# IBM/VillanDiffusion

Hardware: AMD Instinct MI355X
Metric: train imgs/sec + 1000-step DDPM sample imgs/sec, CIFAR10 bs128 (higher is better)
Workload: dtype bf16x3/f32

## Files before the change

### include/villan_hip.h

```cpp
#ifndef VILLAN_HIP_H
#define VILLAN_HIP_H

#include <stdint.h>

#ifdef __cplusplus
extern "C" {
#endif

#define VD_ABI_VERSION 12
#define VD_EINVAL (-22)
#define VD_ETIMEDOUT (-110)

int vd_abi_version(void);
const char* vd_last_error(void);
int vd_device_ok(void);
int vd_async_errors(int clear);

enum vd_a_mode { VD_A_ROW = 0,
                 VD_A_COL = 1 };
enum vd_b_mode { VD_B_PLAIN = 0,
                 VD_B_KCONTIG = 1,
                 VD_B_CONV3 = 2,
                 VD_B_CONV3_T = 3,
                 VD_B_CONV3_S2 = 4,
// ... 70 lines not shown
int vd_conv_wgrad_kernel_name(const vd_wgrad_desc* desc, char* name, int name_len);

int vd_presplit_pack(const float* x, void* y, int B, int C, int HW, int64_t x_bstride, int64_t y_bstride, void* stream);
int vd_presplit_unpack(const void* y, float* x, int B, int C, int HW, int64_t y_bstride, int64_t x_bstride, void* stream);
int vd_groupnorm_fwd_presplit_ok(int C, int HW, int G);
int vd_groupnorm_fwd_presplit(const float* x, const float* gamma, const float* beta, void* y, float* mean, float* rstd, int B, int C, int HW, int G,
                              float eps, int apply_silu, int64_t x_bstride, int64_t y_bstride, void* stream);
int vd_groupnorm_bwd_presplit(const float* dy, const float* x, const float* mean, const float* rstd, const float* gamma, const float* beta,
                              const float* extra, const float* extra2, float* dx, void* dx_ps, float* dgamma_ws, float* dbeta_ws, float* rowsum,
                              int B, int C, int HW, int G, int apply_silu, int64_t dy_bstride, int64_t x_bstride, int64_t extra_bstride,
                              int64_t extra2_bstride, int64_t dx_bstride, int64_t ps_bstride, int64_t rowsum_ld, void* stream);

int vd_conv_wgrad_group_class(const vd_wgrad_desc* desc);
int64_t vd_conv_wgrad_group_job_bytes(void);
int vd_conv_wgrad_group_variant(int cls);
int vd_conv_wgrad_group_plan(const vd_wgrad_desc* descs, int n, void* table_out, int64_t* ws_floats, int* blocks, int* rblocks);
int vd_conv_wgrad_group_rebase(void* dev_table, int n, float* ws, void* stream);
int vd_conv_wgrad_group_launch(const void* dev_table, int n, int cls, int blocks, int rblocks, void* stream);
int vd_conv_wgrad_group_kernel_name(int cls, char* name, int name_len);

int64_t vd_conv3_packed_bytes(int M, int C, int taps);
int vd_conv3_pack_weights(const float* W, void* packed, int M, int C, int taps, int64_t row_stride, int64_t chan_stride, void* stream);
int vd_conv3_pack_weights_multi(const int64_t* table, int n_jobs, int64_t total_blocks, void* stream);
int vd_conv3_pack_weights_f16_multi(const int64_t* table, int n_jobs, int64_t total_blocks, void* stream);

int vd_weight_transpose(const float* W, float* Wt, int M, int C, int T, void* stream);
int vd_sumpool2x2(const float* dU, float* dX, int B, int C, int H, int W, int64_t du_bstride, int64_t dx_bstride,
                  int accumulate, void* stream);
int vd_col2im_s2(const float* G, float* dX, int B, int C, int H, int W, int OH, int OW, int pad, int64_t g_bstride,
                 int64_t dx_bstride, void* stream);
int vd_rowsum(const float* X, float* ws, int B, int M, int P, int64_t x_bstride, int64_t ws_ld, void* stream);
int vd_colsum(const float* ws, float* out, int B, int C, int64_t ld, int accumulate, void* stream);
int vd_colsum_segmented(const int64_t* table, int n_jobs, int B, void* stream);

int64_t vd_groupnorm_ws_floats(int B, int C, int HW, int G);
int vd_groupnorm_fwd(const float* x, const float* gamma, const float* beta, float* y, float* mean, float* rstd,
                     int B, int C, int HW, int G, float eps, int apply_silu, int64_t x_bstride, int64_t y_bstride,
                     float* ws, void* stream);
int vd_groupnorm_stats(const float* x, const float* gamma, const float* beta, float* ss, float* mean, float* rstd,
                       int B, int C, int HW, int G, float eps, int64_t x_bstride, void* stream);
int vd_groupnorm_stats_from_partials(const float* part, int tiles, const float* gamma, const float* beta, float* ss, float* mean,
                                     float* rstd, int B, int C, int HW, int G, float eps, void* stream);
int vd_groupnorm_bwd(const float* dy, const float* x, const float* mean, const float* rstd, const float* gamma,
                     const float* beta, const float* extra, float* dx, float* dgamma_ws, float* dbeta_ws,
                     int B, int C, int HW, int G, int apply_silu, int64_t dy_bstride, int64_t x_bstride,
                     int64_t extra_bstride, int64_t dx_bstride, float* ws, void* stream);
int vd_groupnorm_bwd_fused(const float* dy, const float* x, const float* mean, const float* rstd, const float* gamma,
                           const float* beta, const float* extra, const float* extra2, float* dx, float* dgamma_ws,
                           float* dbeta_ws, float* rowsum, int B, int C, int HW, int G, int apply_silu,
                           int64_t dy_bstride, int64_t x_bstride, int64_t extra_bstride, int64_t extra2_bstride,
                           int64_t dx_bstride, int64_t rowsum_ld, float* ws, void* stream);
int vd_groupnorm_plan(int which, int B, int C, int HW, int G, int aligned, int has_ws, void* stream, char* name, int name_len);

int vd_softmax_col_fwd(float* S, int nb, int N, void* stream);
int vd_softmax_col_bwd(const float* P, float* dP, int nb, int N, float scale, void* stream);
int vd_attn_small_fwd(const float* qkv, float* out, float* P, int B, int C, int N, float scale,
                      int64_t qkv_bstride, int64_t out_bstride, void* stream);
int vd_attn_small_bwd(const float* qkv, const float* P, const float* dout, float* dqkv, int B, int C, int N,
                      float scale, int64_t qkv_bstride, int64_t dout_bstride, int64_t dqkv_bstride, void* stream);

int vd_attn_core_fwd(const float* qkv, float* out, float* P, int B, int heads, int head_dim, int N, float scale, void* stream);
int vd_attn_core_bwd(const float* qkv, const float* P, const float* out, const float* dout, float* dS, float* dqkv, int B, int heads,
                     int head_dim, int N, float scale, void* stream);

int vd_attn_flash_fwd(const float* qkv, float* out, float* lse, int B, int heads, int head_dim, int N, float scale, int64_t qkv_bstride,
                      int64_t out_bstride, void* stream);
int vd_attn_flash_bwd(const float* qkv, const float* out, const float* dout, const float* lse, float* delta, float* dqkv, int B, int heads,
                      int head_dim, int N, float scale, int64_t qkv_bstride, int64_t out_bstride, int64_t dout_bstride,
                      int64_t dqkv_bstride, void* stream);

int vd_timestep_embedding(const float* t, const float* freqs, float* emb, int B, int half, int flip_sin_to_cos,
                          void* stream);
int vd_silu_fwd(const float* x, float* y, int64_t n, void* stream);
int vd_silu_bwd(const float* dy, const float* x, float* dx, int64_t n, int accumulate, void* stream);
int vd_add_strided(float* dst, const float* src, int B, int64_t inner, int64_t dst_bstride, int64_t src_bstride,
                   int accumulate, void* stream);
int vd_scale(float* x, int64_t n, float alpha, void* stream);
int vd_lincomb(float* out, const float* const* srcs, const float* coefs, int n_src, int64_t n, void* stream);

int vd_qsample_backdoor(const float* x0, const float* R, const float* eps, const int64_t* t,
                        const float* tab_a, const float* tab_s, const float* tab_step, const float* tab_coef,
                        float* x_t, float* y, int B, int64_t chw, void* stream);
int vd_mse_fwd_bwd(const float* pred, const float* y, const float* pscale, float* dpred, float* loss,
                   float* partial, int B, int64_t chw, float gscale, void* stream);
#define VD_LOSS_L2 0
#define VD_LOSS_L1 1
#define VD_LOSS_HUBER 2
int vd_loss_fwd_bwd(const float* pred, const float* y, const float* pscale, float* dpred, float* loss,
                    float* partial, int B, int64_t chw, float gscale, int kind, void* stream);
int vd_loss_sample_fwd_bwd(const float* pred, const float* y, const float* pscale, const float* weight, const float* wtab, const int64_t* t,
                           int T, const uint8_t* flags, float poison_weight, float* dpred, float* loss, float* sample_loss, float* stats,
                           float* ws, int B, int64_t chw, float gscale, int kind, void* stream);
int64_t vd_loss_sample_ws_floats(int B, int64_t chw);
int vd_loss_sample_plan(int B, int64_t chw, int* segments, int* blocks);
int vd_trigger_inv_objective(const float* e, const float* tau, float lambda, float* loss, float* dout, float* dtau, float* partial,
                             int B, int64_t chw, int64_t e_bstride, void* stream);
int vd_removal_loss(const float* pred, const float* ref, float w_clean, float w_shift, float gscale, float* dpred, float* terms,
                    float* partial, int B, int64_t chw, int64_t pred_bstride, void* stream);
int vd_image_set_stats(const float* x, int N, int C, int H, int W, int64_t x_bstride, float mul, float add, float lo, float hi,
                       float* mean_img, float* stats, float* partial, void* stream);
int vd_score_inv_objective(const float* s, const float* tau, float sigma, float lambda, float* loss, float* dout, float* dtau,
                           float* partial, int B, int64_t chw, int64_t s_bstride, void* stream);
int vd_image_set_merge(float* mean_a, float* stats_a, int64_t n_a, const float* mean_b, const float* stats_b, int64_t n_b, int64_t chw,
                       float* partial, void* stream);
int vd_neuron_scale(const float* w0, float* w, const int64_t* table, int n_jobs, int64_t total_blocks, const float* mask, const float* delta,
                    const float* xi, void* stream);
// ... 51 lines not shown
```

### villandiffusion_amd/csrc/vd_conv_bx3.inc

```
typedef __bf16 bf16x8 __attribute__((ext_vector_type(8)));
typedef unsigned int u32x4 __attribute__((ext_vector_type(4)));

constexpr int XC = 16;

__device__ __forceinline__ void split_bf16x8(const float (&v)[8], u32x4& hi, u32x4& lo) {
    bf16x8 h, l;
#pragma unroll
    for (int j = 0; j < 8; ++j) {
        const __bf16 t = (__bf16)v[j];
        h[j] = t;
        l[j] = (__bf16)(v[j] - (float)t);
    }
    hi = __builtin_bit_cast(u32x4, h);
    lo = __builtin_bit_cast(u32x4, l);
}

template <int T>
__device__ __forceinline__ void conv3_pack_one(const float* __restrict__ src, u32x4* __restrict__ dst, int M, int C, int Mpad, int64_t rs,
                                               int64_t cs, int local) {
    if (local >= Mpad * (C / XC) * 2) return;
    const int m = local % Mpad;
    const int rest = local / Mpad;
    const int q = rest & 1, cc = rest >> 1;
    float v[8][T];
// ... 754 lines not shown
    if (d.OW != 8 || d.OH != 8 || d.pool2 || d.gn_ss || d.N % 256 != 0) return false;
    if (d.b_mode != VD_B_CONV3 && d.b_mode != VD_B_CONV3_T) return false;
    const int base = vd_cdiv(d.M, 128) * (d.N / 256);
    return base >= 32 && base < 256 && d.C / XC >= 8;
}

static void bx3_plan(const vd_gemm_desc& d, int& splits, int& c_per) {
    const int base = vd_cdiv(d.M, 128) * vd_cdiv(d.N, 128);
    const int nchunks = d.C / XC;
    splits = 1;
    if (bx3_big_split(d)) {
        const int bb = vd_cdiv(d.M, 128) * (d.N / 256);
        static const int tgt = getenv("VD_BX3_BIGSPLIT_TARGET") ? atoi(getenv("VD_BX3_BIGSPLIT_TARGET")) : 256;
        splits = vd_cdiv(tgt, bb);
        if (splits > nchunks / 2) splits = nchunks / 2;
        c_per = vd_cdiv(nchunks, splits);
        splits = vd_cdiv(nchunks, c_per);
        return;
    }
    static const int target = getenv("VD_BX3_SPLIT_TARGET") ? atoi(getenv("VD_BX3_SPLIT_TARGET")) : 512;
    if (base < 256) {
        splits = vd_cdiv(d.OW == 4 ? target / 2 : target, base);
        const int max_splits = nchunks / 2 > 0 ? nchunks / 2 : 1;
        if (splits > max_splits) splits = max_splits;
    }
    c_per = vd_cdiv(nchunks, splits);
    splits = vd_cdiv(nchunks, c_per);
}

static int bx3_big_tile(const vd_gemm_desc& d, int splits) {
    if (splits != 1 || (d.OW != 16 && d.OW != 32) || d.N % 256 != 0) return 0;
    if (d.b_mode != VD_B_CONV3_T && !d.pool2 && d.OW == 32 && d.N % 512 == 0) {
        const int nh = vd_cdiv(d.M, 128) * (d.N / 512);
        if (nh >= 256 && (nh % 256 == 0 || nh % 256 >= 192)) return 2;
    }
    const int nb = vd_cdiv(d.M, 128) * (d.N / 256);
    return (nb >= 256 && (nb % 256 == 0 || nb % 256 >= 192)) ? 1 : 0;
}

static bool k32p_pick(const vd_gemm_desc& d) {
    if (d.b_mode != VD_B_CONV3 && d.b_mode != VD_B_CONV3_T && d.b_mode != VD_B_CONV3_UP) return false;
    if (!vd_conv3_k32p_eligible(d) || d.N % 256 != 0) return false;
    const int nt = vd_cdiv(d.M, 128) * (d.N / 256);
    const int rounds = vd_cdiv(nt, 256);
    return nt >= 192 && 4 * nt >= 3 * rounds * 256;
}

static bool pool2_ok(const vd_gemm_desc& d) {
    if (!d.a_packed || d.b_mode != VD_B_CONV3_T || d.bias || d.rowadd || d.residual || d.accumulate) return false;
    if (k32p_pick(d)) return true;
    return d.OH == d.OW && (d.OW == 16 || d.OW == 32) && vd_cdiv(d.M, 128) * vd_cdiv(d.N, 128) >= 256;
}

static int launch_bx3(const vd_gemm_desc& d, int tile, hipStream_t st, char* name) {
    const int mode = d.b_mode == VD_B_CONV3 ? (d.gn_ss ? 3 : 0) : (d.b_mode == VD_B_CONV3_T ? 1 : (d.b_mode == VD_B_CONV3_S2 ? 4 : 2));
    if (tile == 18) {
        if (vd_launch_conv3_k32p(d, mode, st, name) != 0) return VD_EINVAL;
        if (name && d.OW > 32) {
            char at[16];
            snprintf(at, sizeof(at), "@%d", d.OW);
            vd_name_append(name, at);
        }
        return 0;
    }
    int splits, c_per;
    bx3_plan(d, splits, c_per);
    if (!name && splits > 1 && d.ws == nullptr) {
        vd_set_error("vd_gemm: split-K workspace required (%d splits): query vd_gemm_ws_floats()", splits);
        return VD_EINVAL;
    }
    if (tile == 16) {
        dim3 grids(vd_cdiv(d.M, 128) * (d.N / 256), splits);
        if (mode == 0) VD_LAUNCH_OR_NAME(name, (conv3_bx3_kernel<8, 0, 2, 512, 2>), grids, dim3(512), 0, st, d, c_per);
        else VD_LAUNCH_OR_NAME(name, (conv3_bx3_kernel<8, 1, 2, 512, 2>), grids, dim3(512), 0, st, d, c_per);
        if (!name && splits > 1) launch_splitk_epilogue(d, splits, st);
        return 0;
    }
    if (tile == 15) {
        dim3 gridh(vd_cdiv(d.M, 128) * (d.N / 512), 1);
        switch (mode) {
        case 0: VD_LAUNCH_OR_NAME(name, (conv3_bx3_kernel<32, 0, 4, 512, 2>), gridh, dim3(512), 0, st, d, c_per); break;
        case 1: VD_LAUNCH_OR_NAME(name, (conv3_bx3_kernel<32, 1, 4, 512, 2>), gridh, dim3(512), 0, st, d, c_per); break;
        case 2: VD_LAUNCH_OR_NAME(name, (conv3_bx3_kernel<32, 2, 4, 512, 2>), gridh, dim3(512), 0, st, d, c_per); break;
        default: VD_LAUNCH_OR_NAME(name, (conv3_bx3_kernel<32, 3, 4, 512, 2>), gridh, dim3(512), 0, st, d, c_per); break;
        }
        return 0;
    }
    bool done = false;
    if (tile == 12) {
        dim3 gridb(vd_cdiv(d.M, 128) * (d.N / 256), 1);
#define BX3_BIG(WW, MD)                                                                                   \
    if (!done && d.OW == WW && mode == MD) {                                                              \
        VD_LAUNCH_OR_NAME(name, (conv3_bx3_kernel<WW, MD, 2, 512, 2>), gridb, dim3(512), 0, st, d, c_per); \
        done = true;                                                                                      \
    }
        BX3_BIG(32, 0) BX3_BIG(32, 1) BX3_BIG(32, 2) BX3_BIG(32, 3)
        BX3_BIG(16, 0) BX3_BIG(16, 1) BX3_BIG(16, 2) BX3_BIG(16, 3)
#undef BX3_BIG
        return done ? 0 : VD_EINVAL;
    }
    dim3 grid(vd_cdiv(d.M, 128) * vd_cdiv(d.N, 128), splits);
    const int tw = d.OW >= 128 && d.OW % 128 == 0 ? 128 : d.OW;
#define BX3_CASE(WW, MD)                                                                      \
    if (!done && tw == WW && mode == MD) {                                                    \
        VD_LAUNCH_OR_NAME(name, (conv3_bx3_kernel<WW, MD, 2, 256, 2>), grid, dim3(NT), 0, st, d, c_per); \
        done = true;                                                                          \
    }
    BX3_CASE(32, 0) BX3_CASE(32, 1) BX3_CASE(32, 2) BX3_CASE(32, 3)
    BX3_CASE(16, 0) BX3_CASE(16, 1) BX3_CASE(16, 2) BX3_CASE(16, 3)
    BX3_CASE(8, 0) BX3_CASE(8, 1) BX3_CASE(8, 2)
    BX3_CASE(4, 0) BX3_CASE(4, 1)
    BX3_CASE(32, 4) BX3_CASE(16, 4) BX3_CASE(8, 4) BX3_CASE(4, 4)
    BX3_CASE(64, 0) BX3_CASE(64, 1) BX3_CASE(64, 2)
    BX3_CASE(128, 0) BX3_CASE(128, 1) BX3_CASE(128, 2)
    BX3_CASE(64, 4) BX3_CASE(128, 4)
#undef BX3_CASE
    if (!done) return VD_EINVAL;
    if (!name && splits > 1) launch_splitk_epilogue(d, splits, st);
    return 0;
}
```

### villandiffusion_amd/csrc/vd_gemm.hip

```cpp
#include "vd_common.h"
#include <string.h>
#include <stdlib.h>

bool vd_conv3_k32p_eligible(const vd_gemm_desc& d);
int vd_launch_conv3_k32p(const vd_gemm_desc& d, int mode, hipStream_t st, char* name);
int vd_launch_wgrad_ps_group(const void* jobs, int n, int W, int up, int blocks, hipStream_t st, bool one, char* name);
bool vd_conv3_sm_eligible(const vd_gemm_desc& d);
int vd_launch_conv3_sm(const vd_gemm_desc& d, hipStream_t st, char* name);
bool vd_gemm1x1_k32p_pick(const vd_gemm_desc& d);
int vd_launch_gemm1x1_k32p(const vd_gemm_desc& d, hipStream_t st, char* name);

namespace {

constexpr int NT = 256;
constexpr int BK = 32;
constexpr int KG = BK / 4;

struct Pix {
    int b, oy, ox, p;
    bool valid;
};

__device__ __forceinline__ void kdecomp9(int k, int& c, int& r, int& s) {
    c = k / 9;
    int rs = k - c * 9;
    r = (rs * 11) >> 5;
    s = rs - r * 3;
}

template <int BMODE>
__device__ __forceinline__ float conv_gather(const float* __restrict__ src, const vd_gemm_desc& d, const Pix& px,
                                             int64_t boff, int c, int r, int s, bool& ok) {
    int iy, ix;
    if (BMODE == VD_B_CONV3) {
        iy = px.oy + r - 1;
        ix = px.ox + s - 1;
        ok = (unsigned)iy < (unsigned)d.H && (unsigned)ix < (unsigned)d.W;
    } else if (BMODE == VD_B_CONV3_T) {
        iy = px.oy + 1 - r;
        ix = px.ox + 1 - s;
        ok = (unsigned)iy < (unsigned)d.H && (unsigned)ix < (unsigned)d.W;
    } else if (BMODE == VD_B_CONV3_S2) {
        iy = 2 * px.oy + r - d.pad;
        ix = 2 * px.ox + s - d.pad;
        ok = (unsigned)iy < (unsigned)d.H && (unsigned)ix < (unsigned)d.W;
    } else if (BMODE == VD_B_CONV3_UP) {
        int uy = px.oy + r - 1, ux = px.ox + s - 1;
        ok = (unsigned)uy < (unsigned)(2 * d.H) && (unsigned)ux < (unsigned)(2 * d.W);
        iy = uy >> 1;
        ix = ux >> 1;
    } else if (BMODE == VD_B_CONVG) {
        iy = px.oy * d.conv_stride + r - d.pad_h;
        ix = px.ox * d.conv_stride + s - d.pad_w;
// ... 522 lines not shown
                    acc[mi][ni] = __builtin_amdgcn_mfma_f32_32x32x2f32(a0[mi], b0[ni], acc[mi][ni], 0, 0, 0);
            if (u + 2 < (CKK / 2) * 9) fetch(u + 2, a0, b0);
            __builtin_amdgcn_sched_barrier(0);
#pragma unroll
            for (int mi = 0; mi < WM; ++mi)
#pragma unroll
                for (int ni = 0; ni < WN; ++ni)
                    acc[mi][ni] = __builtin_amdgcn_mfma_f32_32x32x2f32(a1[mi], b1[ni], acc[mi][ni], 0, 0, 0);
        }
        __syncthreads();
        if (more && !(VD_DBG(d) & 8)) store_stage((ks + 1) * CKK);
        __syncthreads();
    }
    if (gridDim.y == 1) {
        gemm_epilogue<WM, WN>(d, acc, m0, n0, wm, wn, lane, h);
        return;
    }
    float* __restrict__ slab = d.ws + (int64_t)blockIdx.y * d.M * d.N;
#pragma unroll
    for (int ni = 0; ni < WN; ++ni) {
        const int n = n0 + wn * 32 * WN + ni * 32 + (lane & 31);
        if (n >= d.N) continue;
#pragma unroll
        for (int mi = 0; mi < WM; ++mi)
#pragma unroll
            for (int v = 0; v < 16; ++v) {
                const int m = m0 + wm * 64 + mi * 32 + (v & 3) + 8 * (v >> 2) + 4 * h;
                if (m < d.M) slab[(int64_t)m * d.N + n] = acc[mi][ni][v];
            }
    }
}

__global__ __launch_bounds__(256) void splitk_epilogue_kernel(const vd_gemm_desc d, int splits) {
    const int64_t total = (int64_t)d.M * d.N;
    for (int64_t i = blockIdx.x * (int64_t)blockDim.x + threadIdx.x; i < total; i += (int64_t)gridDim.x * blockDim.x) {
        const int m = (int)(i / d.N), n = (int)(i - (int64_t)m * d.N);
        float s = d.ws[i];
        for (int z = 1; z < splits; ++z) s += d.ws[(int64_t)z * total + i];
        const int b = n / d.NP, p = n - b * d.NP;
        float val = d.alpha * s;
        if (d.bias) val += d.bias[d.bias_on_n ? n : m];
        if (d.rowadd) val += d.rowadd[(int64_t)b * d.rowadd_bstride + m];
        if (d.residual) val += d.residual[(int64_t)b * d.res_bstride + (int64_t)m * d.ldd + p];
        const int64_t off = (int64_t)b * d.d_bstride + (int64_t)m * d.ldd + p;
        if (d.accumulate) val += d.D[off];
        d.D[off] = val;
    }
}

__global__ __launch_bounds__(256) void splitk_epilogue4_kernel(const vd_gemm_desc d, int splits) {
    const int64_t total4 = ((int64_t)d.M * d.N) >> 2;
    const int64_t total = (int64_t)d.M * d.N;
    for (int64_t i4 = blockIdx.x * (int64_t)blockDim.x + threadIdx.x; i4 < total4; i4 += (int64_t)gridDim.x * blockDim.x) {
        const int64_t i = i4 << 2;
        const int m = (int)(i / d.N), n = (int)(i - (int64_t)m * d.N);
        f32x4 s = *reinterpret_cast<const f32x4*>(d.ws + i);
        for (int z = 1; z < splits; ++z) {
            const f32x4 p = *reinterpret_cast<const f32x4*>(d.ws + (int64_t)z * total + i);
#pragma unroll
            for (int j = 0; j < 4; ++j) s[j] += p[j];
        }
        const int b = n / d.NP, p = n - b * d.NP;
        f32x4 val;
#pragma unroll
        for (int j = 0; j < 4; ++j) {
            val[j] = d.alpha * s[j];
            if (d.bias) val[j] += d.bias[d.bias_on_n ? n + j : m];
        }
        if (d.rowadd) {
            const float ra = d.rowadd[(int64_t)b * d.rowadd_bstride + m];
#pragma unroll
            for (int j = 0; j < 4; ++j) val[j] += ra;
        }
        if (d.residual) {
            const f32x4 r = *reinterpret_cast<const f32x4*>(d.residual + (int64_t)b * d.res_bstride + (int64_t)m * d.ldd + p);
#pragma unroll
            for (int j = 0; j < 4; ++j) val[j] += r[j];
        }
        float* __restrict__ dp = d.D + (int64_t)b * d.d_bstride + (int64_t)m * d.ldd + p;
        if (d.accumulate) {
            const f32x4 o = *reinterpret_cast<const f32x4*>(dp);
#pragma unroll
            for (int j = 0; j < 4; ++j) val[j] += o[j];
        }
        *reinterpret_cast<f32x4*>(dp) = val;
    }
}

static void launch_splitk_epilogue(const vd_gemm_desc& d, int splits, hipStream_t st) {
    const int64_t total = (int64_t)d.M * d.N;
    const bool v4 = (d.N & 3) == 0 && (d.NP & 3) == 0 && (d.ldd & 3) == 0 && (d.d_bstride & 3) == 0 && (d.res_bstride & 3) == 0 &&
                    (((uintptr_t)d.D | (uintptr_t)d.residual | (uintptr_t)d.ws) & 15) == 0;
    if (v4) {
        const int64_t t4 = total >> 2;
        const int g2 = (int)((t4 + 255) / 256 < 2048 ? (t4 + 255) / 256 : 2048);
        hipLaunchKernelGGL(splitk_epilogue4_kernel, dim3(g2), dim3(256), 0, st, d, splits);
    } else {
        const int g2 = (int)((total + 255) / 256 < 2048 ? (total + 255) / 256 : 2048);
        hipLaunchKernelGGL(splitk_epilogue_kernel, dim3(g2), dim3(256), 0, st, d, splits);
    }
}

#include "vd_conv_bx3.inc"

static bool patch_eligible(const vd_gemm_desc& d) {
    if (d.a_mode != VD_A_ROW || d.a_bstride != 0 || d.act) return false;
    if (d.gn_ss && (d.b_mode != VD_B_CONV3 || (d.OW != 16 && d.OW != 32) || d.C > 1024)) return false;
    if (d.b_mode == VD_B_CONV3_S2) {
        if ((d.OW != 4 && d.OW != 8 && d.OW != 16) || d.OH != d.OW || d.H != 2 * d.OH || d.W != 2 * d.OW || d.gn_ss) return false;
    } else if (d.b_mode != VD_B_CONV3 && d.b_mode != VD_B_CONV3_T && d.b_mode != VD_B_CONV3_UP) return false;
    if (d.OW != 4 && d.OW != 8 && d.OW != 16 && d.OW != 32 && d.OW != 64 && d.OW % 128 != 0) return false;
    if (d.OH != d.OW && d.OW < 16) return false;
    if (d.C % CK != 0 || d.OH * d.OW != d.NP || d.d_trans) return false;
    if (d.NP >= 128 ? (d.NP % 128 != 0) : (128 % d.NP != 0)) return false;
    if (d.K != d.C * 9 || (d.lda & 3) != 0 || (((uintptr_t)d.A) & 15) != 0) return false;
    if ((VD_DBG(d) & ~(16 | 1 | 8)) != 0 || (VD_DBG(d) != 0 && !(VD_DBG(d) & 16)) || d.tile != 0) return false;
    if (d.b_mode == VD_B_CONV3_UP && d.OW == 4) return false;
    return d.M >= 64;
}

static void patch_plan(const vd_gemm_desc& d, int& splits, int& ks_per) {
    const int base = vd_cdiv(d.M, 128) * vd_cdiv(d.N, 128);
    const int nsteps = d.C / CK;
    splits = 1;
    if (base < 256) {
        splits = vd_cdiv(512, base);
        const int max_splits = nsteps / 4 > 0 ? nsteps / 4 : 1;
        if (splits > max_splits) splits = max_splits;
    }
    ks_per = vd_cdiv(nsteps, splits);
    splits = vd_cdiv(nsteps, ks_per);
}

static bool patch_wide(const vd_gemm_desc& d) {
    if (d.OW != 32 || d.NP % 256 != 0) return false;
    const int64_t wgs = (int64_t)vd_cdiv(d.M, 128) * (d.N / 256);
    return wgs >= 512 && wgs % 512 == 0;
}

static int launch_patch(const vd_gemm_desc& d, hipStream_t st, char* name) {
    int splits, ks_per;
    patch_plan(d, splits, ks_per);
    const int mode_ = d.b_mode == VD_B_CONV3 ? (d.gn_ss ? 3 : 0) : (d.b_mode == VD_B_CONV3_T ? 1 : (d.b_mode == VD_B_CONV3_S2 ? 4 : 2));
    if (splits == 1 && patch_wide(d)) {
        dim3 grid(vd_cdiv(d.M, 128) * (d.N / 256), 1);
        if (mode_ == 0) VD_LAUNCH_OR_NAME(name, (conv3_patch_kernel<32, 0, 4>), grid, dim3(NT), 0, st, d, ks_per);
        else if (mode_ == 3) VD_LAUNCH_OR_NAME(name, (conv3_patch_kernel<32, 3, 4>), grid, dim3(NT), 0, st, d, ks_per);
        else if (mode_ == 1) VD_LAUNCH_OR_NAME(name, (conv3_patch_kernel<32, 1, 4>), grid, dim3(NT), 0, st, d, ks_per);
        else VD_LAUNCH_OR_NAME(name, (conv3_patch_kernel<32, 2, 4>), grid, dim3(NT), 0, st, d, ks_per);
        return 0;
    }
    if (!name && splits > 1 && d.ws == nullptr) {
        vd_set_error("vd_gemm: split-K workspace required (%d splits): query vd_gemm_ws_floats()", splits);
        return VD_EINVAL;
    }
    dim3 grid(vd_cdiv(d.M, 128) * vd_cdiv(d.N, 128), splits);
    const int mode = mode_;
    bool done = false;
    const int tw = d.OW >= 128 && d.OW % 128 == 0 ? 128 : d.OW;
#define VD_PATCH_CASE(WW, MD)                                                                            \
    if (!done && tw == WW && mode == MD) {                                                               \
        VD_LAUNCH_OR_NAME(name, (conv3_patch_kernel<WW, MD, 2>), grid, dim3(NT), 0, st, d, ks_per);        \
        done = true;                                                                                     \
    }
    VD_PATCH_CASE(64, 0) VD_PATCH_CASE(64, 1) VD_PATCH_CASE(64, 2)
    VD_PATCH_CASE(128, 0) VD_PATCH_CASE(128, 1) VD_PATCH_CASE(128, 2)
    VD_PATCH_CASE(32, 0) VD_PATCH_CASE(32, 1) VD_PATCH_CASE(32, 2) VD_PATCH_CASE(32, 3)
    VD_PATCH_CASE(16, 0) VD_PATCH_CASE(16, 1) VD_PATCH_CASE(16, 2) VD_PATCH_CASE(16, 3)
    VD_PATCH_CASE(8, 0) VD_PATCH_CASE(8, 1) VD_PATCH_CASE(8, 2)
    VD_PATCH_CASE(4, 0) VD_PATCH_CASE(4, 1)
    VD_PATCH_CASE(16, 4) VD_PATCH_CASE(8, 4) VD_PATCH_CASE(4, 4)
#undef VD_PATCH_CASE
    if (!done) return VD_EINVAL;
    if (!name && splits > 1) launch_splitk_epilogue(d, splits, st);
    return 0;
}

template <int TW, int MM>
__global__ __launch_bounds__(256) void conv3_smallm_kernel(const vd_gemm_desc d) {
    constexpr int TH = 256 / TW, PW = TW + 2, PH = TH + 2, CK = 8;
    constexpr int PLn = PH * PW;
    constexpr int P_EL = (CK * PLn + 255) / 256;
    __shared__ float Ps[CK * PLn];
    __shared__ f32x4 Ws[CK * 9];
    const int tid = threadIdx.x;
    const int tiles_x = d.W / TW, tiles_y = d.H / TH;
    int bid = blockIdx.x;
    const int txi = bid % tiles_x;
    bid /= tiles_x;
    const int tyi = bid % tiles_y;
    const int b = bid / tiles_y;
    const int y0 = tyi * TH, x0 = txi * TW;
    const int ty = tid / TW, tx = tid - ty * TW;
    const int HWs = d.H * d.W;
    const float* __restrict__ xb = d.B + (int64_t)b * d.b_bstride;
    const float* __restrict__ Wp = d.A;

    int poff[P_EL];
#pragma unroll
    for (int i = 0; i < P_EL; ++i) {
        const int e = tid + i * 256;
        const int rem = e % PLn;
        const int py = rem / PW, px = rem - py * PW;
        const int iy = y0 + py - 1, ix = x0 + px - 1;
        const bool ok = e < CK * PLn && (unsigned)iy < (unsigned)d.H && (unsigned)ix < (unsigned)d.W;
        poff[i] = ok ? iy * d.W + ix : -1;
    }
    float acc[MM];
#pragma unroll
    for (int m = 0; m < MM; ++m) acc[m] = 0.f;

    for (int c0 = 0; c0 < d.C; c0 += CK) {
        __syncthreads();
#pragma unroll
        for (int i = 0; i < P_EL; ++i) {
            const int e = tid + i * 256;
            if (e < CK * PLn) {
                const int c = c0 + e / PLn;
                const bool ok = poff[i] >= 0 && c < d.C;
                const float v = xb[ok ? (int64_t)c * HWs + poff[i] : 0];
                Ps[e] = ok ? v : 0.f;
            }
        }
        if (tid < CK * 9) {
            const int c = c0 + tid / 9, t = tid - (tid / 9) * 9;
            f32x4 w = {0.f, 0.f, 0.f, 0.f};
#pragma unroll
// ... 1214 lines not shown
    int splits, ks_per;
    patch_plan(*desc, splits, ks_per);
    return splits > 1 ? (int64_t)splits * desc->M * desc->N : 0;
}

extern "C" int vd_gemm_tile(const vd_gemm_desc* desc) {
    if (!desc) return 0;
    const vd_gemm_desc& d = *desc;
    if (d.pool2 && !pool2_ok(d)) return -1;
    if (d.a_packed && d.math == 2) {
        if (bx3_eligible(d) && !bx3_big_split(d) && k32p_pick(d)) return 18;
        if (gemm_bx3_eligible(d) && vd_gemm1x1_k32p_pick(d)) return 19;
        return -1;
    }
    if (d.a_packed && d.math == 3) {
        if (bx3_eligible(d)) {
            if (vd_conv3_sm_eligible(d)) return 20;
            if (!bx3_big_split(d) && k32p_pick(d)) return 18;
            return -1;
        }
        if (gemm_bx3_eligible(d) && vd_gemm1x1_k32p_pick(d)) return 19;
        return -1;
    }
    if (d.a_packed) {
        if (bx3_eligible(d)) {
            if (vd_conv3_sm_eligible(d)) return 20;
            if (bx3_big_split(d)) return 16;
            if (k32p_pick(d)) return 18;
            int splits, c_per;
            bx3_plan(d, splits, c_per);
            const int big = d.b_mode == VD_B_CONV3_S2 ? 0 : bx3_big_tile(d, splits);
            return big == 2 ? 15 : (big == 1 ? 12 : 8);
        }
        if (!gemm_bx3_eligible(d)) return -1;
        if (vd_gemm1x1_k32p_pick(d)) return 19;
        if (gemm_bx3_big_tile(d)) return 13;
        return vd_cdiv(d.M, 128) * (d.N / 128) >= 1024 ? 11 : 9;
    }
    if (d.math == 1) return gemm_bx3_act_eligible(d) ? 10 : -1;
    if (smallm_eligible(d)) return 7;
    if (patch_eligible(d)) {
        int splits, ks_per;
        patch_plan(d, splits, ks_per);
        return (splits == 1 && patch_wide(d)) ? 6 : 4;
    }
    if (plain_eligible(d)) return 5;
    int max_bn = 128;
    if (d.a_bstride != 0 && d.NP % 128 != 0) max_bn = 64;
    int tile = d.tile ? d.tile : pick_tile(d.M, d.N, max_bn);
    if (max_bn < 128 && tile != 3) tile = 3;
    return tile;
}

static int gemm_run(const vd_gemm_desc* desc, hipStream_t st, char* name) {
    VD_REQUIRE(desc != nullptr, "vd_gemm: null desc");
    vd_gemm_desc d = *desc;
    VD_REQUIRE(d.A && d.B && d.D, "vd_gemm: null operand");
    VD_REQUIRE(d.math != 3 || d.a_packed, "vd_gemm: math = 3 (one bf16 product per term) reads the hi plane of a_packed; a_packed is NULL");
#ifndef VD_ABLATION
    VD_REQUIRE(d.debug == 0, "vd_gemm: desc.debug = %d -- timing-only ablation bits exist in `make ABLATION=1` builds only", d.debug);
#endif
    VD_REQUIRE(d.M > 0 && d.N > 0 && d.K > 0 && d.NP > 0 && d.N % d.NP == 0, "vd_gemm: bad dims M=%d N=%d K=%d NP=%d", d.M,
               d.N, d.K, d.NP);
    if (d.b_mode >= VD_B_CONV3) {
        VD_REQUIRE(d.C > 0 && d.H > 0 && d.W > 0 && d.OH * d.OW == d.NP, "vd_gemm: bad conv dims");
        if (d.b_mode == VD_B_CONVG)
            VD_REQUIRE(d.kh > 0 && d.kw > 0 && d.K == d.C * d.kh * d.kw && d.conv_stride >= 1 && d.conv_stride <= 4 && d.pad_h >= 0 && d.pad_w >= 0 &&
                           d.OH == (d.H + 2 * d.pad_h - d.kh) / d.conv_stride + 1 && d.OW == (d.W + 2 * d.pad_w - d.kw) / d.conv_stride + 1 &&
                           !d.a_packed && d.math == 0 && d.a_mode == VD_A_ROW,
                       "vd_gemm: VD_B_CONVG needs kh, kw > 0, K = C*kh*kw, conv_stride 1 .. 4, OH / OW = (H + 2 pad - k) / stride + 1, row-major exact-f32 A");
        else
            VD_REQUIRE(d.K == d.C * 9, "vd_gemm: conv K must be C*9");
    }
    VD_REQUIRE(d.act == 0 || (d.act == 1 && !d.a_packed && d.math == 0), "vd_gemm: act = 1 (ReLU) is honoured by the exact-f32 kernels only");
    if (d.a_bstride != 0) VD_REQUIRE(d.NP % 64 == 0, "vd_gemm: per-batch A needs NP %% 64 == 0 (NP=%d)", d.NP);
    VD_REQUIRE(!(d.d_trans && (d.residual || d.rowadd)), "vd_gemm: d_trans excludes residual/rowadd");
    if (d.nb2 > 1)
        VD_REQUIRE(!d.residual && !d.rowadd && !d.d_trans && d.b_mode <= VD_B_KCONTIG && (d.N / d.NP) % d.nb2 == 0,
                   "vd_gemm: two-level batch (nb2=%d) needs plain operands, no residual/rowadd, nb %% nb2 == 0", d.nb2);
    const int tile = vd_gemm_tile(&d);
    VD_REQUIRE(tile != -1, "vd_gemm: a_packed (split-precision bf16) needs a 3x3 convolution with 8x8 / 16x16 / 32x32 outputs, "
                           "C %% 16 == 0, M >= 64, or a VD_B_PLAIN product with shared A, NP %% 128 == 0, K %% 16 == 0, M >= 64; "
                           "a_packed_mpad = M rounded up to 128; math = 1 needs per-batch A, PLAIN / KCONTIG B, NP %% 128 == 0, K %% 16 == 0, K >= 32, M >= 64; "
                           "math = 2 / 3 need the persistent 16x16x32 kernels (vd_gemm_tile 18 / 19; math = 3 also 20); "
                           "pool2 needs VD_B_CONV3_T with a_packed and a bare epilogue, on the persistent kernel or at 16x16 / 32x32 outputs with >= 256 tiles of 128 x 128");
    VD_REQUIRE(d.b_presplit == 0 || (d.b_presplit == 1 && tile == 18),
               "vd_gemm: a pre-split B operand (b_presplit = %d) is read by the persistent 16x16x32 convolution only (vd_gemm_tile() == 18; this problem: %d)",
               d.b_presplit, tile);
    VD_REQUIRE(!d.gn_ss || tile == 4 || tile == 6 || tile == 8 || tile == 12 || tile == 15 || tile == 18,
               "vd_gemm: gn_ss (GroupNorm folded into the loader) needs the patch-staged 3x3 kernel (OW 16/32, C %% 8 == 0, M >= 64)");
    VD_REQUIRE(!d.pool2 || tile == 8 || tile == 12 || tile == 18, "vd_gemm: pool2 needs the split-precision 3x3 kernel (VD_B_CONV3_T with a_packed)");
    VD_REQUIRE(!d.act_out || (tile == 18 && d.gn_ss), "vd_gemm: act_out is written by the persistent 16x16x32 3x3 convolution with gn_ss only (vd_gemm_tile() == 18)");
    VD_REQUIRE(!d.gn_part || (tile == 18 && !d.pool2),
               "vd_gemm: gn_part is written by the persistent 16x16x32 split-precision 3x3 kernel only (vd_gemm_tile() == 18)");
    int rc = 0;
    switch (tile) {
        case 1: rc = launch_gemm_t<2, 2>(d, st, name); break;
        case 2: rc = launch_gemm_t<1, 2>(d, st, name); break;
        case 3: rc = launch_gemm_t<1, 1>(d, st, name); break;
        case 4:
        case 6: rc = launch_patch(d, st, name); break;
        case 7: rc = launch_smallm(d, st, name); break;
        case 8: case 12: case 15: case 16: case 18: rc = launch_bx3(d, tile, st, name); break;
        case 19: rc = vd_launch_gemm1x1_k32p(d, st, name) == 0 ? 0 : VD_EINVAL; break;
        case 20: rc = vd_launch_conv3_sm(d, st, name) == 0 ? 0 : VD_EINVAL; break;
        case 10: launch_gemm_bx3_act(d, st, name); break;
        case 13: VD_LAUNCH_OR_NAME(name, gemm_bx3_kernel<512>, dim3(vd_cdiv(d.M, 128) * (d.N / 256)), dim3(512), 0, st, d, 1 << 30); break;
        case 9: {
            int splits, st_per;
            gemm_bx3_plan(d, splits, st_per);
            VD_REQUIRE(name || splits == 1 || d.ws, "vd_gemm: split-K 1x1 launch needs the workspace (vd_gemm_ws_floats)");
            VD_LAUNCH_OR_NAME(name, gemm_bx3_kernel<256>, dim3(vd_cdiv(d.M, 128) * (d.N / 128), splits), dim3(NT), 0, st, d, st_per);
            if (!name && splits > 1) launch_splitk_epilogue(d, splits, st);
            break;
        }
        case 11: VD_LAUNCH_OR_NAME(name, gemm_bx3_persist_kernel, dim3(512), dim3(NT), 0, st, d, vd_cdiv(d.M, 128) * (d.N / 128)); break;
        case 5: {
            const int grid = vd_cdiv(d.M, 128) * (d.N / 128);
            if (d.a_mode == VD_A_ROW) VD_LAUNCH_OR_NAME(name, gemm_plain_kernel<0>, dim3(grid), dim3(NT), 0, st, d);
            else VD_LAUNCH_OR_NAME(name, gemm_plain_kernel<1>, dim3(grid), dim3(NT), 0, st, d);
            break;
        }
        default: vd_set_error("vd_gemm: bad tile %d", tile); return VD_EINVAL;
    }
    if (rc || name) return rc ? rc : tile;
    VD_LAUNCH_CHECK("vd_gemm");
    return 0;
}

extern "C" int vd_gemm(const vd_gemm_desc* desc, void* stream) { return gemm_run(desc, (hipStream_t)stream, nullptr); }

static int name_out(int rc, const char* buf, char* name, int name_len) {
    if (!name || name_len <= 0) return VD_EINVAL;
    snprintf(name, name_len, "%s", rc < 0 ? "" : buf);
    return rc < 0 ? VD_EINVAL : rc;
}

extern "C" int vd_gemm_kernel_name(const vd_gemm_desc* desc, char* name, int name_len) {
    char buf[VD_NAME_LEN] = "";
    return name_out(gemm_run(desc, nullptr, buf), buf, name, name_len);
}

extern "C" int64_t vd_conv3_packed_bytes(int M, int C, int taps) {
    if (M <= 0 || C <= 0 || C % XC != 0 || (taps != 9 && taps != 1)) return 0;
    return (int64_t)((M + 127) / 128 * 128) * C * taps * 4;
}

extern "C" int vd_conv3_pack_weights(const float* W, void* packed, int M, int C, int taps, int64_t row_stride, int64_t chan_stride,
                                     void* stream) {
    VD_REQUIRE(W && packed && M > 0 && C > 0 && C % XC == 0 && (taps == 9 || taps == 1),
               "vd_conv3_pack_weights: bad arguments (M=%d C=%d taps=%d; C %% 16 == 0, taps 9 or 1)", M, C, taps);
    VD_REQUIRE((((uintptr_t)packed) & 15) == 0, "vd_conv3_pack_weights: packed must be 16-byte aligned");
    const int Mpad = (M + 127) / 128 * 128;
    const int total = (C / XC) * 2 * Mpad;
    hipLaunchKernelGGL(conv3_pack_kernel, dim3(vd_cdiv(total, 256)), dim3(256), 0, (hipStream_t)stream, W,
                       reinterpret_cast<u32x4*>(packed), M, C, Mpad, row_stride, chan_stride, taps);
    VD_LAUNCH_CHECK("vd_conv3_pack_weights");
    return 0;
}

extern "C" int vd_conv3_pack_weights_multi(const int64_t* table, int n_jobs, int64_t total_blocks, void* stream) {
    VD_REQUIRE(table && n_jobs > 0 && total_blocks > 0 && total_blocks < (1ll << 31), "vd_conv3_pack_weights_multi: bad arguments");
    hipLaunchKernelGGL(conv3_pack_multi_kernel, dim3((unsigned)total_blocks), dim3(256), 0, (hipStream_t)stream, table, n_jobs);
    VD_LAUNCH_CHECK("vd_conv3_pack_weights_multi");
    return 0;
}

static void wgrad_plan(const vd_wgrad_desc& d, int& tile, int& splits, int& kk_per) {
    if (wgrad_small_eligible(d)) {
        tile = 6;
        splits = wgrad_small_parts(d) > 1 ? wgrad_small_parts(d) : 2;
        kk_per = 1;
        return;
    }
    if (wgrad1x1_bx3_eligible(d)) {
        tile = 5;
        wgrad1x1_bx3_plan(d, splits, kk_per);
        return;
    }
    if (wgrad_patch_eligible(d)) {
        tile = 4;
        wgrad_patch_plan(d, splits, kk_per);
        return;
    }
    const int Ncols = d.C * d.T, Ktot = d.nb * d.NP;
    tile = d.tile;
    if (!tile) {
        tile = (d.M > 64 && Ncols > 64) ? 1 : 3;
        if (tile == 1 && vd_cdiv(d.M, 128) * vd_cdiv(Ncols, 128) < 32) tile = 3;
    }
    const int bm = tile == 1 ? 128 : 64, bn = tile == 3 ? 64 : 128;
    const int tiles = vd_cdiv(d.M, bm) * vd_cdiv(Ncols, bn);
    splits = d.splits;
// ... 386 lines not shown
```

### villandiffusion_amd/csrc/vd_norm.hip

```cpp
#include "vd_common.h"
#include <atomic>
#include <stdlib.h>

namespace {

template <int NTH>
__device__ __forceinline__ float block_sum_t(float v, float* red) {
    if (NTH == 256) return block_sum_256(v, red);
    v = wave_sum(v);
    const int w = threadIdx.x >> 6;
    __syncthreads();
    if ((threadIdx.x & 63) == 0) red[w] = v;
    __syncthreads();
    float a = 0.f;
#pragma unroll
    for (int k = 0; k < NTH / 64; ++k) a += red[k];
    return a;
}

template <int NV, int NTH = 256>
__global__ __launch_bounds__(NTH) void gn_fwd_reg_kernel(const float* __restrict__ x, const float* __restrict__ gamma,
                                                         const float* __restrict__ beta, float* __restrict__ y,
                                                         float* __restrict__ mean_out, float* __restrict__ rstd_out, int C,
                                                         int HW, int G, float eps, int apply_silu, int64_t x_bs, int64_t y_bs,
                                                         float* __restrict__ ss_out) {
    __shared__ float red[2 * (NTH / 64 < 4 ? 4 : NTH / 64)];
    const int b = blockIdx.x / G, g = blockIdx.x - b * G;
    const int cpg = C / G;
    const int n4 = (cpg * HW) >> 2;
    const f32x4* __restrict__ x4 = reinterpret_cast<const f32x4*>(x + (int64_t)b * x_bs + (int64_t)g * cpg * HW);
    f32x4* __restrict__ y4 = reinterpret_cast<f32x4*>(y + (int64_t)b * y_bs + (int64_t)g * cpg * HW);
    const int tid = threadIdx.x;
    f32x4 v[NV];
    float s = 0.f;
#pragma unroll
    for (int i = 0; i < NV; ++i) {
        const int idx = tid + i * NTH;
        v[i] = (idx < n4) ? x4[idx] : f32x4{0.f, 0.f, 0.f, 0.f};
        s += (v[i][0] + v[i][1]) + (v[i][2] + v[i][3]);
    }
    const float inv_n = 1.f / (float)(cpg * HW);
    const float mean = block_sum_t<NTH>(s, red) * inv_n;
    float q = 0.f;
#pragma unroll
    for (int i = 0; i < NV; ++i) {
        if (tid + i * NTH < n4) {
            const float a0 = v[i][0] - mean, a1 = v[i][1] - mean, a2 = v[i][2] - mean, a3 = v[i][3] - mean;
            q += (a0 * a0 + a1 * a1) + (a2 * a2 + a3 * a3);
        }
    }
    const float rstd = rsqrtf(block_sum_t<NTH>(q, red + (NTH / 64 < 4 ? 4 : NTH / 64)) * inv_n + eps);
    if (tid == 0) {
        mean_out[blockIdx.x] = mean;
        rstd_out[blockIdx.x] = rstd;
    }
    if (ss_out) {
        if (tid < cpg) {
            const int c = g * cpg + tid;
            const float ga = gamma[c] * rstd, be = beta[c] - mean * ga;
            ss_out[((int64_t)b * C + c) * 2] = ga;
            ss_out[((int64_t)b * C + c) * 2 + 1] = be;
        }
        return;
    }
#pragma unroll
    for (int i = 0; i < NV; ++i) {
        const int idx = tid + i * NTH;
        if (idx < n4) {
            const int c = g * cpg + (idx * 4) / HW;
            const float ga = gamma[c] * rstd, be = beta[c] - mean * ga;
            f32x4 o;
#pragma unroll
            for (int j = 0; j < 4; ++j) {
                const float z = v[i][j] * ga + be;
                o[j] = apply_silu ? z * sigmoidf_(z) : z;
            }
            y4[idx] = o;
        }
    }
}

template <int NV>
__global__ __launch_bounds__(256) void gn_fwd_wave_kernel(const float* __restrict__ x, const float* __restrict__ gamma,
                                                          const float* __restrict__ beta, float* __restrict__ y,
                                                          float* __restrict__ mean_out, float* __restrict__ rstd_out, int C,
                                                          int HW, int G, float eps, int apply_silu, int64_t x_bs, int64_t y_bs,
                                                          float* __restrict__ ss_out, int total) {
    const int lane = threadIdx.x & 63;
    const int gid = blockIdx.x * 4 + (threadIdx.x >> 6);
    if (gid >= total) return;
    const int b = gid / G, g = gid - b * G;
    const int cpg = C / G;
    const int n4 = (cpg * HW) >> 2;
    const f32x4* __restrict__ x4 = reinterpret_cast<const f32x4*>(x + (int64_t)b * x_bs + (int64_t)g * cpg * HW);
    f32x4 v[NV];
    float s = 0.f;
#pragma unroll
    for (int i = 0; i < NV; ++i) {
        const int idx = lane + i * 64;
        v[i] = (idx < n4) ? x4[idx] : f32x4{0.f, 0.f, 0.f, 0.f};
        s += (v[i][0] + v[i][1]) + (v[i][2] + v[i][3]);
    }
    const float inv_n = 1.f / (float)(cpg * HW);
    const float mean = wave_sum(s) * inv_n;
    float q = 0.f;
#pragma unroll
    for (int i = 0; i < NV; ++i) {
        if (lane + i * 64 < n4) {
            const float a0 = v[i][0] - mean, a1 = v[i][1] - mean, a2 = v[i][2] - mean, a3 = v[i][3] - mean;
            q += (a0 * a0 + a1 * a1) + (a2 * a2 + a3 * a3);
        }
    }
    const float rstd = rsqrtf(wave_sum(q) * inv_n + eps);
    if (lane == 0) {
        mean_out[gid] = mean;
        rstd_out[gid] = rstd;
    }
    if (ss_out) {
        for (int cl = lane; cl < cpg; cl += 64) {
            const int c = g * cpg + cl;
            const float ga = gamma[c] * rstd, be = beta[c] - mean * ga;
            ss_out[((int64_t)b * C + c) * 2] = ga;
            ss_out[((int64_t)b * C + c) * 2 + 1] = be;
        }
        return;
    }
    f32x4* __restrict__ y4 = reinterpret_cast<f32x4*>(y + (int64_t)b * y_bs + (int64_t)g * cpg * HW);
#pragma unroll
    for (int i = 0; i < NV; ++i) {
        const int idx = lane + i * 64;
        if (idx < n4) {
            const int c = g * cpg + (idx * 4) / HW;
            const float ga = gamma[c] * rstd, be = beta[c] - mean * ga;
            f32x4 o;
#pragma unroll
            for (int j = 0; j < 4; ++j) {
                const float z = v[i][j] * ga + be;
                o[j] = apply_silu ? z * sigmoidf_(z) : z;
            }
            y4[idx] = o;
        }
    }
}

__global__ __launch_bounds__(256) void gn_fwd_kernel(const float* __restrict__ x, const float* __restrict__ gamma,
                                                     const float* __restrict__ beta, float* __restrict__ y,
                                                     float* __restrict__ mean_out, float* __restrict__ rstd_out, int C, int HW,
                                                     int G, float eps, int apply_silu, int64_t x_bs, int64_t y_bs) {
    __shared__ float red[8];
    const int b = blockIdx.x / G, g = blockIdx.x - b * G;
    const int cpg = C / G;
    const int n = cpg * HW;
    const float* __restrict__ xs = x + (int64_t)b * x_bs + (int64_t)g * n;
    float* __restrict__ ys = y + (int64_t)b * y_bs + (int64_t)g * n;
    const int tid = threadIdx.x;
    const bool vec = ((HW & 3) == 0) && ((((uintptr_t)xs) & 15) == 0) && ((((uintptr_t)ys) & 15) == 0);

    float s = 0.f;
    if (vec) {
        const f32x4* x4 = reinterpret_cast<const f32x4*>(xs);
        for (int i = tid; i < (n >> 2); i += 256) {
            f32x4 v = x4[i];
            s += (v[0] + v[1]) + (v[2] + v[3]);
        }
    } else {
        for (int i = tid; i < n; i += 256) s += xs[i];
    }
    const float mean = block_sum_256(s, red) / (float)n;
    float q = 0.f;
    if (vec) {
        const f32x4* x4 = reinterpret_cast<const f32x4*>(xs);
        for (int i = tid; i < (n >> 2); i += 256) {
            f32x4 v = x4[i];
            const float a0 = v[0] - mean, a1 = v[1] - mean, a2 = v[2] - mean, a3 = v[3] - mean;
            q += (a0 * a0 + a1 * a1) + (a2 * a2 + a3 * a3);
        }
    } else {
        for (int i = tid; i < n; i += 256) {
            const float a = xs[i] - mean;
            q += a * a;
        }
    }
    const float var = block_sum_256(q, red + 4) / (float)n;
    const float rstd = rsqrtf(var + eps);
    if (tid == 0) {
        mean_out[blockIdx.x] = mean;
        rstd_out[blockIdx.x] = rstd;
    }
    if (vec) {
        const f32x4* x4 = reinterpret_cast<const f32x4*>(xs);
        f32x4* y4 = reinterpret_cast<f32x4*>(ys);
        for (int i = tid; i < (n >> 2); i += 256) {
            const int c = g * cpg + (i * 4) / HW;
            const float ga = gamma[c] * rstd, be = beta[c] - mean * ga;
            f32x4 v = x4[i], o;
// ... 213 lines not shown
            if (f4) {
                const f32x4 fv = f4[idx];
#pragma unroll
                for (int j = 0; j < 4; ++j) ev[j] += fv[j];
            }
#pragma unroll
            for (int j = 0; j < 4; ++j) {
                o[j] = rstd * (dz[i][j] * ga - m1 - xh[i][j] * m2) + ev[j];
                s3 += o[j];
            }
            o4[idx] = o;
        }
        if (rs_out) {
            if (L >= 64) {
                s3 = wave_sum(s3);
                if (lane == 0) part3[i * (NTH / 64) + wave] = s3;
            } else {
                for (int off = 1; off < L; off <<= 1) s3 += __shfl_xor(s3, off, 64);
                if (in && (lane & (L - 1)) == 0) ch_s3[idx / L] = s3;
            }
        }
    }
    if (rs_out) {
        __syncthreads();
        if (tid < cpg) {
            float a3;
            if (L >= 64) {
                const int np = L >> 6;
                a3 = 0.f;
                for (int k = 0; k < np; ++k) a3 += part3[tid * np + k];
            } else {
                a3 = ch_s3[tid];
            }
            rs_out[(int64_t)b * rs_ld + g * cpg + tid] = a3;
        }
    }
}

template <int NV>
__global__ __launch_bounds__(256) void gn_bwd_wave_kernel(const float* __restrict__ dy, const float* __restrict__ x,
                                                          const float* __restrict__ mean_in, const float* __restrict__ rstd_in,
                                                          const float* __restrict__ gamma, const float* __restrict__ beta,
                                                          const float* __restrict__ extra, float* __restrict__ dx,
                                                          float* __restrict__ dgamma_ws, float* __restrict__ dbeta_ws, int C,
                                                          int HW, int G, int apply_silu, int64_t dy_bs, int64_t x_bs,
                                                          int64_t ex_bs, int64_t dx_bs, const float* __restrict__ extra2,
                                                          int64_t ex2_bs, float* __restrict__ rs_out, int64_t rs_ld, int total) {
    const int lane = threadIdx.x & 63;
    const int gid = blockIdx.x * 4 + (threadIdx.x >> 6);
    if (gid >= total) return;
    const int b = gid / G, g = gid - b * G;
    const int cpg = C / G;
    const int n4 = (cpg * HW) >> 2;
    const int L = HW >> 2;
    const int64_t goff = (int64_t)g * cpg * HW;
    const f32x4* __restrict__ x4 = reinterpret_cast<const f32x4*>(x + (int64_t)b * x_bs + goff);
    const f32x4* __restrict__ d4 = reinterpret_cast<const f32x4*>(dy + (int64_t)b * dy_bs + goff);
    const f32x4* __restrict__ e4 = extra ? reinterpret_cast<const f32x4*>(extra + (int64_t)b * ex_bs + goff) : nullptr;
    const f32x4* __restrict__ f4 = extra2 ? reinterpret_cast<const f32x4*>(extra2 + (int64_t)b * ex2_bs + goff) : nullptr;
    f32x4* __restrict__ o4 = reinterpret_cast<f32x4*>(dx + (int64_t)b * dx_bs + goff);
    const float mean = mean_in[gid], rstd = rstd_in[gid];

    f32x4 xh[NV], dz[NV];
    float gav[NV];
    float m1 = 0.f, m2 = 0.f;
#pragma unroll
    for (int i = 0; i < NV; ++i) {
        const int idx = lane + i * 64;
        const bool in = idx < n4;
        const f32x4 xv = in ? x4[idx] : f32x4{0.f, 0.f, 0.f, 0.f};
        const f32x4 dv = in ? d4[idx] : f32x4{0.f, 0.f, 0.f, 0.f};
        const int c = g * cpg + (in ? idx / L : 0);
        const float ga = gamma[c], be = beta[c];
        gav[i] = ga;
        float s1 = 0.f, s2 = 0.f;
#pragma unroll
        for (int j = 0; j < 4; ++j) {
            const float h_ = (xv[j] - mean) * rstd;
            float z_ = dv[j];
            if (apply_silu) {
                const float z = h_ * ga + be, sg = sigmoidf_(z);
                z_ *= sg * (1.f + z * (1.f - sg));
            }
            if (!in) z_ = 0.f;
            xh[i][j] = h_;
            dz[i][j] = z_;
            s1 += z_;
            s2 += z_ * h_;
        }
        for (int off = 1; off < L; off <<= 1) {
            s1 += __shfl_xor(s1, off, 64);
            s2 += __shfl_xor(s2, off, 64);
        }
        if (in && (lane & (L - 1)) == 0) {
            dbeta_ws[(int64_t)b * C + c] = s1;
            dgamma_ws[(int64_t)b * C + c] = s2;
            m1 += ga * s1;
            m2 += ga * s2;
        }
    }
    const float inv_n = 1.f / (float)(cpg * HW);
    m1 = wave_sum(m1) * inv_n;
    m2 = wave_sum(m2) * inv_n;
#pragma unroll
    for (int i = 0; i < NV; ++i) {
        const int idx = lane + i * 64;
        const bool in = idx < n4;
        float s3 = 0.f;
        if (in) {
            f32x4 ev = {0.f, 0.f, 0.f, 0.f}, o;
            if (e4) ev = e4[idx];
            if (f4) {
                const f32x4 fv = f4[idx];
#pragma unroll
                for (int j = 0; j < 4; ++j) ev[j] += fv[j];
            }
#pragma unroll
            for (int j = 0; j < 4; ++j) {
                o[j] = rstd * (dz[i][j] * gav[i] - m1 - xh[i][j] * m2) + ev[j];
                s3 += o[j];
            }
            o4[idx] = o;
        }
        if (rs_out) {
            for (int off = 1; off < L; off <<= 1) s3 += __shfl_xor(s3, off, 64);
            if (in && (lane & (L - 1)) == 0) rs_out[(int64_t)b * rs_ld + g * cpg + idx / L] = s3;
        }
    }
}

__device__ __forceinline__ void gn_combine(const float* __restrict__ part, int S, float n_c, float& mean, float& m2) {
    float n = 0.f;
    mean = 0.f;
    m2 = 0.f;
    for (int k = 0; k < S; ++k) {
        const float mk = part[2 * k], qk = part[2 * k + 1];
        const float nn = n + n_c, delta = mk - mean;
        mean += delta * (n_c / nn);
        m2 += qk + delta * delta * (n * n_c / nn);
        n = nn;
    }
}

template <int NV>
__global__ __launch_bounds__(256) void gn_chunk_stats_kernel(const float* __restrict__ x, float* __restrict__ part, int C, int HW,
                                                             int G, int S, int64_t x_bs) {
    __shared__ float red[8];
    const int bg = blockIdx.x / S, sc = blockIdx.x - bg * S;
    const int b = bg / G, g = bg - b * G;
    const int cpg = C / G;
    const int c4 = ((cpg * HW) >> 2) / S;
    const f32x4* __restrict__ x4 = reinterpret_cast<const f32x4*>(x + (int64_t)b * x_bs + (int64_t)g * cpg * HW) + (int64_t)sc * c4;
    const int tid = threadIdx.x;
    f32x4 v[NV];
    float s = 0.f;
#pragma unroll
    for (int i = 0; i < NV; ++i) {
        const int idx = tid + i * 256;
        v[i] = (idx < c4) ? x4[idx] : f32x4{0.f, 0.f, 0.f, 0.f};
        s += (v[i][0] + v[i][1]) + (v[i][2] + v[i][3]);
    }
    const float mean = block_sum_256(s, red) / (float)(c4 * 4);
    float q = 0.f;
#pragma unroll
    for (int i = 0; i < NV; ++i)
        if (tid + i * 256 < c4) {
            const float a0 = v[i][0] - mean, a1 = v[i][1] - mean, a2 = v[i][2] - mean, a3 = v[i][3] - mean;
            q += (a0 * a0 + a1 * a1) + (a2 * a2 + a3 * a3);
        }
    q = block_sum_256(q, red + 4);
    if (tid == 0) {
        part[2 * (int64_t)blockIdx.x] = mean;
        part[2 * (int64_t)blockIdx.x + 1] = q;
    }
}

__global__ __launch_bounds__(256) void gn_chunk_apply_kernel(const float* __restrict__ x, const float* __restrict__ gamma,
                                                             const float* __restrict__ beta, float* __restrict__ y,
                                                             float* __restrict__ mean_out, float* __restrict__ rstd_out,
                                                             const float* __restrict__ part, int C, int HW, int G, int S, float eps,
                                                             int apply_silu, int64_t x_bs, int64_t y_bs) {
// ... 465 lines not shown
    if (slab <= 14 * 1024) return GN_F_REG7_512;
    return GN_F_REG7_1024;
}

static GnFwdKernel gn_fwd_choice(int B, int C, int HW, int G, bool al, bool has_ws, hipStream_t st, int* S_out) {
    const int64_t slab = (int64_t)(C / G) * HW;
    al = al && HW % 4 == 0;
    const int S = (al && has_ws) ? gn_chunks(B, C, HW, G, true) : 0;
    *S_out = S;
    if (S && gn_chunk1_ok(st, S)) return slab / S > 8192 ? GN_F_CHUNK1_16 : GN_F_CHUNK1_8;
    if (S) return slab / S > 8192 ? GN_F_CHUNK2_16 : GN_F_CHUNK2_8;
    if (al && slab <= GN_REG_MAX) return gn_fwd_reg_choice(slab);
    return GN_F_GENERIC;
}

static GnBwdKernel gn_bwd_choice(int B, int C, int HW, int G, bool al, bool has_ws, hipStream_t st, int* S_out) {
    const int64_t slab = (int64_t)(C / G) * HW;
    const int L = HW / 4;
    const int S = (al && has_ws) ? gn_chunks(B, C, HW, G) : 0;
    *S_out = S;
    const bool reg_ok = !S && al && HW % 4 == 0 && slab <= GN_REG_MAX &&
                        ((L >= 64 && L % 64 == 0) || (L < 64 && (L & (L - 1)) == 0 && L > 0));
    if (reg_ok) {
        if (slab <= 1024 && L < 64 && gn_wave_ok()) return slab <= 256 ? GN_B_WAVE1 : slab <= 512 ? GN_B_WAVE2 : GN_B_WAVE4;
        if (slab <= 1024) return GN_B_REG1_256;
        if (slab <= 2048) return GN_B_REG2_256;
        if (slab <= 4096) return GN_B_REG4_256;
        if (slab <= 8192) return GN_B_REG4_512;
        if (slab <= 12 * 1024) return GN_B_REG6_512;
        if (slab <= 14 * 1024) return GN_B_REG7_512;
        return GN_B_REG7_1024;
    }
    if (S && gn_chunk1_ok(st, S)) return slab / S > 8192 ? GN_B_CHUNK1_16 : GN_B_CHUNK1_8;
    if (S) return GN_B_CHUNK2;
    return GN_B_GENERIC;
}

static bool gn_dims_ok(int B, int C, int HW, int G) { return B > 0 && C > 0 && HW > 0 && G > 0 && C % G == 0; }
static bool gn_stats_dims_ok(int B, int C, int HW, int G) { return gn_dims_ok(B, C, HW, G) && C / G <= 256; }
static bool gn_stats_slab_ok(int C, int HW, int G, bool al) { return HW % 4 == 0 && al && (int64_t)(C / G) * HW <= GN_REG_MAX; }
static bool gn_bwd_dims_ok(int B, int C, int HW, int G) { return gn_dims_ok(B, C, HW, G) && C / G <= 64; }

int gn_sticky_impl(const char* who) {
    const unsigned n = gn_flag_read();
    if (n == 0) return 0;
    vd_set_error("%s: %u GroupNorm poll timeout(s) reported by an earlier one-launch chunked kernel (statistics were NaN); "
                 "vd_async_errors(1) clears the flag, VD_GN_CHUNK1_OFF=1 selects the two-launch form", who, n);
    return VD_ETIMEDOUT;
}

}

int vd_gn_sticky(const char* who) { return gn_sticky_impl(who); }

extern "C" int vd_async_errors(int clear) {
    const unsigned n = gn_flag_read();
    if (clear && g_gn_flag_host) *reinterpret_cast<volatile unsigned*>(g_gn_flag_host) = 0u;
    return (int)(n > 0x7fffffffu ? 0x7fffffffu : n);
}

extern "C" int64_t vd_groupnorm_ws_floats(int B, int C, int HW, int G) {
    if (B <= 0 || C <= 0 || HW <= 0 || G <= 0 || C % G) return 0;
    const int S = gn_chunks(B, C, HW, G);
    return S ? 4 * (int64_t)B * G * S + 4 * (int64_t)B * G * S : 0;
}

extern "C" int vd_groupnorm_fwd(const float* x, const float* gamma, const float* beta, float* y, float* mean, float* rstd,
                                int B, int C, int HW, int G, float eps, int apply_silu, int64_t x_bstride, int64_t y_bstride,
                                float* ws, void* stream) {
    VD_REQUIRE(x && gamma && beta && y && mean && rstd, "vd_groupnorm_fwd: null pointer");
    VD_REQUIRE(B > 0 && C > 0 && HW > 0 && G > 0 && C % G == 0, "vd_groupnorm_fwd: bad dims B=%d C=%d HW=%d G=%d", B, C, HW, G);
    const bool al = (x_bstride % 4 == 0) && (y_bstride % 4 == 0) && ((((uintptr_t)x) & 15) == 0) && ((((uintptr_t)y) & 15) == 0);
    if (const int rc = vd_gn_sticky("vd_groupnorm_fwd")) return rc;
    int S = 0;
    const GnFwdKernel k = gn_fwd_choice(B, C, HW, G, al, ws != nullptr, (hipStream_t)stream, &S);
#define VD_GN_CHUNK1(NVV)                                                                                                                           \
    hipLaunchKernelGGL((gn_chunk1_fwd_kernel<NVV>), dim3(B * G * S), dim3(256), 0, (hipStream_t)stream, x, gamma, beta, y, mean, rstd,              \
                       reinterpret_cast<unsigned long long*>(ws + 4 * (int64_t)B * G * S), C, HW, G, S, eps, apply_silu, x_bstride, y_bstride,      \
                       gn_next_epoch(), flag, gn_poll_max())
#define VD_GN_CHUNK2(NVV)                                                                                                                           \
    do {                                                                                                                                            \
        hipLaunchKernelGGL((gn_chunk_stats_kernel<NVV>), dim3(B * G * S), dim3(256), 0, (hipStream_t)stream, x, ws, C, HW, G, S, x_bstride);        \
        hipLaunchKernelGGL(gn_chunk_apply_kernel, dim3(B * G * S), dim3(256), 0, (hipStream_t)stream, x, gamma, beta, y, mean, rstd, ws, C, HW, G,  \
                           S, eps, apply_silu, x_bstride, y_bstride);                                                                               \
    } while (0)
#define VD_GN_FWDW(NVV)                                                                                                                     \
    hipLaunchKernelGGL((gn_fwd_wave_kernel<NVV>), dim3(vd_cdiv(B * G, 4)), dim3(256), 0, (hipStream_t)stream, x, gamma, beta, y, mean, rstd, \
                       C, HW, G, eps, apply_silu, x_bstride, y_bstride, (float*)nullptr, B * G)
#define VD_GN_FWD(NVV, NT)                                                                                                          \
    hipLaunchKernelGGL((gn_fwd_reg_kernel<NVV, NT>), dim3(B * G), dim3(NT), 0, (hipStream_t)stream, x, gamma, beta, y, mean, rstd, \
                       C, HW, G, eps, apply_silu, x_bstride, y_bstride, (float*)nullptr)
    switch (k) {
    case GN_F_CHUNK1_16:
    case GN_F_CHUNK1_8: {
        unsigned* flag = gn_flag_dev();
        if (k == GN_F_CHUNK1_16) VD_GN_CHUNK1(16);
        else VD_GN_CHUNK1(8);
        break;
    }
    case GN_F_CHUNK2_16: VD_GN_CHUNK2(16); break;
    case GN_F_CHUNK2_8: VD_GN_CHUNK2(8); break;
    case GN_F_WAVE1: VD_GN_FWDW(1); break;
    case GN_F_WAVE2: VD_GN_FWDW(2); break;
    case GN_F_WAVE4: VD_GN_FWDW(4); break;
    case GN_F_REG1: VD_GN_FWD(1, 256); break;
    case GN_F_REG2: VD_GN_FWD(2, 256); break;
// ... 204 lines not shown
```

### villandiffusion_amd/lib.py

```python
from __future__ import annotations

import ctypes as C
import os
import subprocess
from typing import Optional

_HERE = os.path.dirname(os.path.abspath(__file__))
LIB_PATH = os.path.join(_HERE, "libvillan_hip.so")
CSRC = os.path.join(_HERE, "csrc")

A_ROW, A_COL = 0, 1
B_PLAIN, B_KCONTIG, B_CONV3, B_CONV3_T, B_CONV3_S2, B_CONV3_UP, B_CONV3_DIL, B_CONVG = range(8)

_i32, _i64, _f32, _vp = C.c_int32, C.c_int64, C.c_float, C.c_void_p


class GemmDesc(C.Structure):
    _fields_ = [("A", _vp), ("B", _vp), ("D", _vp), ("bias", _vp), ("rowadd", _vp), ("residual", _vp),
                ("M", _i32), ("N", _i32), ("K", _i32), ("a_mode", _i32), ("b_mode", _i32), ("NP", _i32),
                ("C", _i32), ("H", _i32), ("W", _i32), ("OH", _i32), ("OW", _i32),
                ("bias_on_n", _i32), ("d_trans", _i32), ("accumulate", _i32), ("tile", _i32), ("debug", _i32), ("alpha", _f32),
                ("lda", _i64), ("a_bstride", _i64), ("ldb", _i64), ("b_bstride", _i64),
                ("ldd", _i64), ("d_bstride", _i64), ("res_bstride", _i64), ("rowadd_bstride", _i64), ("ws", _vp), ("pad", _i32), ("nb2", _i32),
                ("a_b2stride", _i64), ("b_b2stride", _i64), ("d_b2stride", _i64), ("gn_ss", _vp), ("a_packed", _vp), ("a_packed_mpad", _i32), ("math", _i32), ("pool2", _i32),
                ("kh", _i32), ("kw", _i32), ("conv_stride", _i32), ("pad_h", _i32), ("pad_w", _i32), ("act", _i32),
                ("gn_part", _vp), ("act_out", _vp), ("act_bstride", _i64), ("b_presplit", _i32), ("reserved_", _i32)]


class WgradDesc(C.Structure):
    _fields_ = [("dY", _vp), ("X", _vp), ("dW", _vp), ("ws", _vp),
                ("M", _i32), ("C", _i32), ("T", _i32), ("nb", _i32), ("NP", _i32),
                ("H", _i32), ("W", _i32), ("OH", _i32), ("OW", _i32),
                ("mode", _i32), ("splits", _i32), ("accumulate", _i32), ("tile", _i32),
                ("dy_bstride", _i64), ("x_bstride", _i64), ("pad", _i32), ("math", _i32), ("presplit", _i32), ("reserved_", _i32)]


PROTOTYPES = {
    "vd_abi_version": (_i32, []),
    "vd_last_error": (C.c_char_p, []),
    "vd_async_errors": (_i32, [_i32]),
    "vd_device_ok": (_i32, []),
    "vd_gemm": (_i32, [C.POINTER(GemmDesc), _vp]),
    "vd_gemm_tile": (_i32, [C.POINTER(GemmDesc)]),
    "vd_gemm_ws_floats": (_i64, [C.POINTER(GemmDesc)]),
    "vd_gemm_kernel_name": (_i32, [C.POINTER(GemmDesc), C.c_char_p, _i32]),
    "vd_conv_wgrad": (_i32, [C.POINTER(WgradDesc), _vp]),
    "vd_conv_wgrad_plan": (_i32, [C.POINTER(WgradDesc), C.POINTER(_i32), C.POINTER(_i32)]),
    "vd_conv_wgrad_ws_floats": (_i64, [C.POINTER(WgradDesc)]),
    "vd_conv_wgrad_kernel_name": (_i32, [C.POINTER(WgradDesc), C.c_char_p, _i32]),
    "vd_presplit_pack": (_i32, [_vp, _vp, _i32, _i32, _i32, _i64, _i64, _vp]),
    "vd_presplit_unpack": (_i32, [_vp, _vp, _i32, _i32, _i32, _i64, _i64, _vp]),
    "vd_groupnorm_fwd_presplit_ok": (_i32, [_i32, _i32, _i32]),
    "vd_groupnorm_fwd_presplit": (_i32, [_vp, _vp, _vp, _vp, _vp, _vp, _i32, _i32, _i32, _i32, _f32, _i32, _i64, _i64, _vp]),
    "vd_groupnorm_bwd_presplit": (_i32, [_vp] * 12 + [_vp, _i32, _i32, _i32, _i32, _i32] + [_i64] * 7 + [_vp]),
    "vd_conv_wgrad_group_class": (_i32, [C.POINTER(WgradDesc)]),
    "vd_conv_wgrad_group_job_bytes": (_i64, []),
    "vd_conv_wgrad_group_variant": (_i32, [_i32]),
    "vd_conv_wgrad_group_kernel_name": (_i32, [_i32, C.c_char_p, _i32]),
    "vd_conv_wgrad_group_plan": (_i32, [C.POINTER(WgradDesc), _i32, _vp, C.POINTER(_i64), C.POINTER(_i32), C.POINTER(_i32)]),
    "vd_conv_wgrad_group_rebase": (_i32, [_vp, _i32, _vp, _vp]),
    "vd_conv_wgrad_group_launch": (_i32, [_vp, _i32, _i32, _i32, _i32, _vp]),
    "vd_conv3_packed_bytes": (_i64, [_i32, _i32, _i32]),
    "vd_conv3_pack_weights": (_i32, [_vp, _vp, _i32, _i32, _i32, _i64, _i64, _vp]),
    "vd_conv3_pack_weights_multi": (_i32, [_vp, _i32, _i64, _vp]),
    "vd_conv3_pack_weights_f16_multi": (_i32, [_vp, _i32, _i64, _vp]),
    "vd_weight_transpose": (_i32, [_vp, _vp, _i32, _i32, _i32, _vp]),
    "vd_sumpool2x2": (_i32, [_vp, _vp, _i32, _i32, _i32, _i32, _i64, _i64, _i32, _vp]),
    "vd_col2im_s2": (_i32, [_vp, _vp, _i32, _i32, _i32, _i32, _i32, _i32, _i32, _i64, _i64, _vp]),
    "vd_rowsum": (_i32, [_vp, _vp, _i32, _i32, _i32, _i64, _i64, _vp]),
    "vd_colsum": (_i32, [_vp, _vp, _i32, _i32, _i64, _i32, _vp]),
    "vd_colsum_segmented": (_i32, [_vp, _i32, _i32, _vp]),
    "vd_groupnorm_ws_floats": (_i64, [_i32, _i32, _i32, _i32]),
    "vd_groupnorm_stats": (_i32, [_vp, _vp, _vp, _vp, _vp, _vp, _i32, _i32, _i32, _i32, _f32, _i64, _vp]),
    "vd_groupnorm_fwd": (_i32, [_vp, _vp, _vp, _vp, _vp, _vp, _i32, _i32, _i32, _i32, _f32, _i32, _i64, _i64, _vp, _vp]),
    "vd_groupnorm_bwd": (_i32, [_vp] * 10 + [_i32] * 5 + [_i64] * 4 + [_vp, _vp]),
    "vd_groupnorm_stats_from_partials": (_i32, [_vp, _i32, _vp, _vp, _vp, _vp, _vp, _i32, _i32, _i32, _i32, _f32, _vp]),
    "vd_groupnorm_bwd_fused": (_i32, [_vp] * 12 + [_i32] * 5 + [_i64] * 6 + [_vp, _vp]),
    "vd_groupnorm_plan": (_i32, [_i32] * 7 + [_vp, C.c_char_p, _i32]),
    "vd_softmax_col_fwd": (_i32, [_vp, _i32, _i32, _vp]),
    "vd_softmax_col_bwd": (_i32, [_vp, _vp, _i32, _i32, _f32, _vp]),
    "vd_attn_small_fwd": (_i32, [_vp, _vp, _vp, _i32, _i32, _i32, _f32, _i64, _i64, _vp]),
    "vd_attn_small_bwd": (_i32, [_vp, _vp, _vp, _vp, _i32, _i32, _i32, _f32, _i64, _i64, _i64, _vp]),
    "vd_attn_core_fwd": (_i32, [_vp, _vp, _vp, _i32, _i32, _i32, _i32, _f32, _vp]),
    "vd_attn_core_bwd": (_i32, [_vp, _vp, _vp, _vp, _vp, _vp, _i32, _i32, _i32, _i32, _f32, _vp]),
    "vd_attn_flash_fwd": (_i32, [_vp, _vp, _vp, _i32, _i32, _i32, _i32, _f32, _i64, _i64, _vp]),
    "vd_attn_flash_bwd": (_i32, [_vp, _vp, _vp, _vp, _vp, _vp, _i32, _i32, _i32, _i32, _f32, _i64, _i64, _i64, _i64, _vp]),
    "vd_timestep_embedding": (_i32, [_vp, _vp, _vp, _i32, _i32, _i32, _vp]),
    "vd_silu_fwd": (_i32, [_vp, _vp, _i64, _vp]),
    "vd_silu_bwd": (_i32, [_vp, _vp, _vp, _i64, _i32, _vp]),
    "vd_add_strided": (_i32, [_vp, _vp, _i32, _i64, _i64, _i64, _i32, _vp]),
    "vd_scale": (_i32, [_vp, _i64, _f32, _vp]),
    "vd_lincomb": (_i32, [_vp, C.POINTER(_vp), C.POINTER(_f32), _i32, _i64, _vp]),
    "vd_qsample_backdoor": (_i32, [_vp] * 10 + [_i32, _i64, _vp]),
    "vd_mse_fwd_bwd": (_i32, [_vp] * 6 + [_i32, _i64, _f32, _vp]),
    "vd_loss_fwd_bwd": (_i32, [_vp] * 6 + [_i32, _i64, _f32, _i32, _vp]),
    "vd_loss_sample_fwd_bwd": (_i32, [_vp] * 6 + [_i32, _vp, _f32] + [_vp] * 5 + [_i32, _i64, _f32, _i32, _vp]),
    "vd_loss_sample_ws_floats": (_i64, [_i32, _i64]),
    "vd_loss_sample_plan": (_i32, [_i32, _i64, C.POINTER(_i32), C.POINTER(_i32)]),
    "vd_trigger_inv_objective": (_i32, [_vp, _vp, _f32, _vp, _vp, _vp, _vp, _i32, _i64, _i64, _vp]),
    "vd_removal_loss": (_i32, [_vp, _vp, _f32, _f32, _f32, _vp, _vp, _vp, _i32, _i64, _i64, _vp]),
    "vd_score_inv_objective": (_i32, [_vp, _vp, _f32, _f32, _vp, _vp, _vp, _vp, _i32, _i64, _i64, _vp]),
    "vd_image_set_stats": (_i32, [_vp, _i32, _i32, _i32, _i32, _i64, _f32, _f32, _f32, _f32, _vp, _vp, _vp, _vp]),
    "vd_image_set_merge": (_i32, [_vp, _vp, _i64, _vp, _vp, _i64, _i64, _vp, _vp]),
    "vd_neuron_scale": (_i32, [_vp, _vp, _vp, _i32, _i64, _vp, _vp, _vp, _vp]),
    "vd_neuron_grad": (_i32, [_vp, _vp, _vp, _i32, _i64, _vp, _vp, _f32, _i32, _vp]),
    "vd_neuron_step": (_i32, [_vp, _vp, _vp, _i64, _f32, _f32, _f32, _f32, _i32, _vp]),
    "vd_lora_merge": (_i32, [_vp, _vp, _vp, _i32, _i64, _vp, _i32, _f32, _vp]),
    "vd_lora_grad": (_i32, [_vp, _vp, _i32, _i64, _vp, _vp, _i32, _f32, _i32, _vp]),
    "vd_lora_act_grad_ws_floats": (_i64, [_vp, _i32, _i32]),
    "vd_lora_act_grad": (_i32, [_vp, _vp, _i32, _vp, _vp, _i32, _f32, _i32, _vp, _i64, _vp]),
    "vd_l2norm_sq": (_i32, [_vp, _i64, _vp, _vp, _vp]),
    "vd_adam_step": (_i32, [_vp, _vp, _vp, _vp, _i64, _vp, _f32, _f32, _f32, _f32, _f32, _f32, _i32, _vp, _vp]),
    "vd_adam_ema_step": (_i32, [_vp, _vp, _vp, _vp, _vp, _i64, _vp, _f32, _f32, _f32, _f32, _f32, _f32, _i32, _f32, _vp, _vp]),
    "vd_swap": (_i32, [_vp, _vp, _i64, _vp]),
    "vd_sched_step": (_i32, [_vp] * 5 + [_i64] + [_f32] * 7 + [C.c_uint64, C.c_uint64, _vp]),
    "vd_batch_l2norm": (_i32, [_vp, _vp, _i32, _i64, _vp]),
    "vd_postprocess": (_i32, [_vp, _vp, _i32, _i32, _i32, _f32, _f32, _f32, _f32, _i32, _vp]),
    "vd_ssim": (_i32, [_vp, _vp, _vp, _vp, _i32, _i32, _i32, _i32, _i32, _f32, _f32, _vp]),
    "vd_randn": (_i32, [_vp, _i64, C.c_uint64, C.c_uint64, _vp]),
    "vd_fir_resample2": (_i32, [_vp, _vp, _i64, _i32, _i32, _i32, _f32, _i32, _vp]),
    "vd_pyramid_dgrad": (_i32, [_vp, _vp, _vp, _vp, _i32, _i32, _i32, _i32, _i32, _i64, _i32, _vp]),
    "vd_fourier_embedding": (_i32, [_vp, _vp, _vp, _i32, _i32, _vp]),
    "vd_rowscale": (_i32, [_vp, _vp, _vp, _i32, _i64, _i32, _vp]),
    "vd_vq_nearest": (_i32, [_vp, _vp, _vp, _vp, _i32, _i32, _i32, _i32, _i64, _i64, _vp]),
    "vd_poison_batch": (_i32, [_vp] * 8 + [_i32] * 4 + [_f32, _f32, _i32, _vp]),
    "vd_pool3": (_i32, [_vp, _vp, _i32, _i32, _i32, _i32, _i32, _i32, _i32, _i64, _i64, _vp]),
    "vd_resize_bilinear": (_i32, [_vp, _vp, _i64, _i32, _i32, _i32, _i32, _f32, _f32, _vp]),
    "vd_channel_affine": (_i32, [_vp, _vp, _vp, _vp, _i32, _i32, _i32, _vp]),
    "vd_lpips_layer": (_i32, [_vp, _vp, _vp, _vp, _i32, _i32, _i32, _i32, _vp]),
}

# ... 65 lines not shown
```

### villandiffusion_amd/ops.py

```python
from __future__ import annotations

import ctypes as C
import functools
import math
import os
from typing import Optional, Sequence

import torch

from . import lib as L
from .lib import (A_COL, A_ROW, B_CONV3, B_CONV3_DIL, B_CONVG, B_CONV3_S2, B_CONV3_T, B_CONV3_UP, B_KCONTIG, B_PLAIN,
                  GemmDesc, WgradDesc)


def _lib():
    L.require_device()
    return L.load()


_PROF = None


def _kernel_name(query, what) -> str:
    buf = C.create_string_buffer(128)
# ... 183 lines not shown
    e2bs = _img(extra2)[4] if extra2 is not None else 0
    assert dgamma_ws.numel() >= Bn * Cc and dbeta_ws.numel() >= Bn * Cc
    assert (extra is None or extra.shape == x.shape) and (extra2 is None or extra2.shape == x.shape)
    rld = 0
    if rowsum is not None:
        rld = Cc if rowsum_ld is None else rowsum_ld
        assert rld >= Cc
    nbytes = (8.0 + (4.0 if dx is not None else 0.0) + (4.0 if dx_ps is not None else 0.0) + (4.0 if extra is not None else 0.0)
              + (4.0 if extra2 is not None else 0.0)) * x.numel()
    _timed("groupnorm_bwd_presplit (gn_bwd_ps_kernel<*>)", nbytes, "hbm", lambda: L.check(
        _lib().vd_groupnorm_bwd_presplit(_p(dy), _p(x), _p(mean), _p(rstd), _p(gamma), _p(beta), _p(extra), _p(extra2), _p(dx),
                                         _p(dx_ps.t) if dx_ps is not None else None, _p(dgamma_ws), _p(dbeta_ws), _p(rowsum), Bn, Cc, H * W, G,
                                         int(silu), dbs, xbs, ebs, e2bs, dxbs, psbs, rld, _s()), "vd_groupnorm_bwd_presplit"))
    return dx_ps if dx_ps is not None else dx


_GEMM_WS = {}
_WS_SLOT = 0
AUX_WS_SLOT = -1


class ws_slot:

    def __init__(self, slot: int):
        self.slot, self.prev = int(slot), 0

    def __enter__(self):
        global _WS_SLOT
        self.prev, _WS_SLOT = _WS_SLOT, self.slot
        return self

    def __exit__(self, *exc):
        global _WS_SLOT
        _WS_SLOT = self.prev
        return False


def gemm_ws_buffer(device, slot: int = None):
    return _GEMM_WS.get((device, _WS_SLOT if slot is None else slot))


def _gemm_ws(n_floats: int, device):
    key = (device, _WS_SLOT)
    t = _GEMM_WS.get(key)
    if t is None or t.numel() < n_floats:
        t = torch.empty(max(n_floats, 1 << 22), device=device, dtype=torch.float32)
        _GEMM_WS[key] = t
    return t


def gemm(A, B, D, *, M, N, K, a_mode=A_ROW, b_mode=B_PLAIN, NP=None, lda=0, a_bstride=0, ldb=0, b_bstride=0,
         ldd=0, d_bstride=0, bias=None, bias_on_n=False, rowadd=None, rowadd_bstride=0, residual=None,
         res_bstride=0, conv=None, alpha=1.0, d_trans=False, accumulate=False, tile=0, debug=0, pad=0, nb2=0, a_b2stride=0,
         b_b2stride=0, d_b2stride=0, gn_ss=None, a_packed=None, math_mode=0, pool2=False, convg=None, act=0, gn_part=None, b_presplit=False):
    global GN_PART_WRITTEN
    d = GemmDesc()
    d.act = act
    d.b_presplit = int(b_presplit)
    if convg is not None:
        d.kh, d.kw, d.conv_stride, d.pad_h, d.pad_w = convg
    d.pad = pad
    d.pool2 = int(pool2)
    d.math = math_mode
    a_packed16, alt_math = None, 2
    if isinstance(a_packed, tuple):
        a_packed, a_packed16, *rest = a_packed
        alt_math = rest[0] if rest else 2
    if a_packed is not None:
        d.a_packed, d.a_packed_mpad = a_packed.data_ptr(), (M + 127) // 128 * 128
    d.gn_ss = _p(gn_ss)
    d.nb2, d.a_b2stride, d.b_b2stride, d.d_b2stride = nb2, a_b2stride, b_b2stride, d_b2stride
    d.A, d.B, d.D = _p(A), _p(B), _p(D)
    d.bias, d.rowadd, d.residual = _p(bias), _p(rowadd), _p(residual)
    d.M, d.N, d.K = M, N, K
    d.a_mode, d.b_mode = a_mode, b_mode
    d.NP = N if NP is None else NP
    if conv is not None:
        d.C, d.H, d.W, d.OH, d.OW = conv
    d.bias_on_n, d.d_trans, d.accumulate, d.tile = int(bias_on_n), int(d_trans), int(accumulate), tile
    d.alpha = alpha
    d.debug = debug
    d.lda, d.a_bstride, d.ldb, d.b_bstride = lda, a_bstride, ldb, b_bstride
    d.ldd, d.d_bstride, d.res_bstride, d.rowadd_bstride = ldd, d_bstride, res_bstride, rowadd_bstride
    lib = _lib()
    need = lib.vd_gemm_ws_floats(C.byref(d))
    if need > 0:
        d.ws = _gemm_ws(need, D.device).data_ptr()
    elif FORCE_WS is not None:
        d.ws = FORCE_WS.data_ptr()
    global LAST_GEMM_TILE, LAST_GEMM_MATH
    if a_packed16 is not None and (gn_part is None or alt_math == 3):
        d.a_packed, d.math = a_packed16.data_ptr(), alt_math
        if lib.vd_gemm_tile(C.byref(d)) not in ((18, 19) if alt_math == 2 else (18, 19, 20)):
            d.a_packed, d.math = a_packed.data_ptr(), math_mode
    LAST_GEMM_MATH = d.math
    LAST_GEMM_TILE = lib.vd_gemm_tile(C.byref(d))
    GN_PART_WRITTEN = gn_part is not None and not pool2 and LAST_GEMM_TILE == 18
    if GN_PART_WRITTEN:
        assert gn_part.is_contiguous() and gn_part.numel() >= (N // 256) * M * 2
        d.gn_part = gn_part.data_ptr()
    if _PROF is None:
        L.check(lib.vd_gemm(C.byref(d), _s()), "vd_gemm")
        return D
    e0, e1 = torch.cuda.Event(enable_timing=True), torch.cuda.Event(enable_timing=True)
    e0.record()
    L.check(lib.vd_gemm(C.byref(d), _s()), "vd_gemm")
    e1.record()
    flops = 2.0 * M * N * K * (0.25 if b_mode == B_CONV3_DIL else 1.0)
    if conv is not None:
        nb_ = N // d.NP
        b_elems = nb_ * d.C * d.H * d.W
        a_elems = M * K
    else:
        b_elems = K * N
        a_elems = M * K * (N // d.NP if a_bstride else 1)
    d_elems = M * N // (4 if pool2 else 1)
    nbytes = 4.0 * (b_elems + d_elems * (2 if residual is not None else 1) + a_elems)
    name = _kernel_name(lib.vd_gemm_kernel_name, C.byref(d))
    _PROF.append({"name": name, "flops": flops, "bytes": nbytes, "e0": e0, "e1": e1, "kind": "mfma", "shape": (M, K, d.NP, N // d.NP, d.OH, d.OW)})
    return D


_CONV_OUT = {B_CONV3: lambda h, w: (h, w), B_CONV3_T: lambda h, w: (h, w), B_CONV3_S2: lambda h, w: (h // 2, w // 2),
             B_CONV3_UP: lambda h, w: (2 * h, 2 * w), B_CONV3_DIL: lambda h, w: (2 * h, 2 * w)}


def conv3_pack_weights(w2d, M, Cc, transposed=False, out=None, taps=9):
    lib = _lib()
    nbytes = lib.vd_conv3_packed_bytes(M, Cc, taps)
    assert nbytes > 0, (M, Cc, taps)
    if out is None:
        out = torch.empty(nbytes // 4, device=w2d.device, dtype=torch.int32)
    assert out.numel() * out.element_size() >= nbytes and w2d.is_contiguous()
    rs, cs = (taps, M * taps) if transposed else (Cc * taps, taps)
    L.check(lib.vd_conv3_pack_weights(_p(w2d), _p(out), M, Cc, taps, rs, cs, _s()), "vd_conv3_pack_weights")
    return out


def conv3_pack_weights_f16(w2d, M, Cc, transposed=False, taps=9):
    nbytes = _lib().vd_conv3_packed_bytes(M, Cc, taps) // 2
    assert nbytes > 0 and w2d.is_contiguous(), (M, Cc, taps)
    out = torch.empty(nbytes // 4, device=w2d.device, dtype=torch.int32)
    rs, cs = (taps, M * taps) if transposed else (Cc * taps, taps)
    mpad = (M + 127) // 128 * 128
    tab = torch.tensor([[w2d.data_ptr(), out.data_ptr(), M, Cc, rs, cs, 0, taps]], dtype=torch.int64).to(w2d.device)
    conv3_pack_weights_f16_multi(tab, 1, (mpad * (Cc // 16) * 2 + 255) // 256)
    torch.cuda.current_stream(w2d.device).synchronize()
    return out


def conv3_pack_weights_f16_multi(table, n_jobs, total_blocks):
    assert table.dtype == torch.int64 and table.is_contiguous() and table.numel() >= 8 * n_jobs
    L.check(_lib().vd_conv3_pack_weights_f16_multi(_p(table), n_jobs, total_blocks, _s()), "vd_conv3_pack_weights_f16_multi")


def conv3_pack_weights_multi(table, n_jobs, total_blocks):
    assert table.dtype == torch.int64 and table.is_contiguous() and table.numel() >= 8 * n_jobs
    L.check(_lib().vd_conv3_pack_weights_multi(_p(table), n_jobs, total_blocks, _s()), "vd_conv3_pack_weights_multi")


WEIGHTS_EPOCH = 0


@functools.lru_cache(maxsize=None)
def bx3_eligible(M, Cc, OH, OW, mode) -> bool:
    return _gemm_tile(conv_query_desc(M, Cc, OH, OW, mode)) in _BX3_TILES


@functools.lru_cache(maxsize=None)
def bx3_pool2_eligible(M, Cc, OH, OW, nb) -> bool:
    return _gemm_tile(conv_query_desc(M, Cc, OH, OW, B_CONV3_T, nb, pool2=1)) in _BX3_TILES and OW <= 32


GN_PART_WRITTEN = False
LAST_GEMM_TILE = 0
LAST_GEMM_MATH = 0
FORCE_WS = None


def conv3x3(x, w2d, bias, out, mode=B_CONV3, rowadd=None, rowadd_bstride=0, residual=None, accumulate=False, tile=0, debug=0,
            pad=0, gn_ss=None, a_packed=None, pool2=False, gn_part=None):
    x, ps = _unwrap(x)
    Bn, Cc, H, W, xbs = _img(x)
    M = w2d.shape[0]
    assert w2d.shape[1] == Cc * 9 and w2d.is_contiguous()
    OH, OW = _CONV_OUT[mode](H, W)
    Bo, Mo, OHo, OWo, obs = _img(out)
    if pool2:
        assert (Bo, Mo, OHo, OWo) == (Bn, M, OH // 2, OW // 2) and mode == B_CONV3_T and a_packed is not None, (out.shape, (Bn, M, OH, OW))
        assert bias is None and rowadd is None and residual is None and not accumulate
    else:
        assert (Bo, Mo, OHo, OWo) == (Bn, M, OH, OW), (out.shape, (Bn, M, OH, OW))
    rbs = 0
    if residual is not None:
        rbs = _img(residual)[4]
        assert residual.shape == out.shape
    return gemm(w2d, x, out, M=M, N=Bn * OH * OW, K=Cc * 9, b_mode=mode, NP=OH * OW, lda=Cc * 9, b_bstride=xbs,
                ldd=OHo * OWo, d_bstride=obs, bias=bias, rowadd=rowadd, rowadd_bstride=rowadd_bstride,
                residual=residual, res_bstride=rbs, conv=(Cc, H, W, OH, OW), accumulate=accumulate, tile=tile, debug=debug,
                pad=pad, gn_ss=gn_ss, a_packed=a_packed, pool2=pool2, gn_part=gn_part, b_presplit=ps)


def conv2d_general(x, w2d, bias, out, kh, kw, stride=1, pad_h=0, pad_w=0, relu=False):
    Bn, Cc, H, W, xbs = _img(x)
    M = w2d.shape[0]
    assert w2d.shape[1] == Cc * kh * kw and w2d.is_contiguous()
    OH, OW = (H + 2 * pad_h - kh) // stride + 1, (W + 2 * pad_w - kw) // stride + 1
    Bo, Mo, OHo, OWo, obs = _img(out)
    assert (Bo, Mo, OHo, OWo) == (Bn, M, OH, OW), (out.shape, (Bn, M, OH, OW))
    if kh == 1 and kw == 1 and stride == 1 and pad_h == 0 and pad_w == 0:
        return gemm(w2d, x, out, M=M, N=Bn * OH * OW, K=Cc, b_mode=B_PLAIN, NP=OH * OW, lda=Cc, ldb=H * W, b_bstride=xbs, ldd=OH * OW,
                    d_bstride=obs, bias=bias, act=int(relu))
    return gemm(w2d, x, out, M=M, N=Bn * OH * OW, K=Cc * kh * kw, b_mode=B_CONVG, NP=OH * OW, lda=Cc * kh * kw, b_bstride=xbs, ldd=OH * OW,
                d_bstride=obs, bias=bias, conv=(Cc, H, W, OH, OW), convg=(kh, kw, stride, pad_h, pad_w), act=int(relu))


def pool3(x, out, stride=1, pad=0, mode="max"):
    Bn, Cc, H, W, xbs = _img(x)
    OH, OW = (H + 2 * pad - 3) // stride + 1, (W + 2 * pad - 3) // stride + 1
    Bo, Co, OHo, OWo, obs = _img(out)
    assert (Bo, Co, OHo, OWo) == (Bn, Cc, OH, OW), (out.shape, (Bn, Cc, OH, OW))
    return _timed("pool3_kernel", 4.0 * (x.numel() + out.numel()), "hbm",
                  lambda: L.check(_lib().vd_pool3(_p(x), _p(out), Bn, Cc, H, W, stride, pad, 0 if mode == "max" else 1, xbs, obs, _s()), "vd_pool3"))


def resize_bilinear(x, out, mul=1.0, add=0.0):
    assert x.is_contiguous() and out.is_contiguous() and x.shape[:2] == out.shape[:2] and x.dtype == out.dtype == torch.float32
    L.check(_lib().vd_resize_bilinear(_p(x), _p(out), x.shape[0] * x.shape[1], x.shape[2], x.shape[3], out.shape[2], out.shape[3], mul, add, _s()),
            "vd_resize_bilinear")
    return out


def channel_affine(x, mul, add, out):
    B, C, H, W = x.shape
    assert x.is_contiguous() and out.is_contiguous() and out.shape == x.shape and mul.numel() == C and add.numel() == C
    L.check(_lib().vd_channel_affine(_p(x), _p(mul), _p(add), _p(out), B, C, H * W, _s()), "vd_channel_affine")
    return out


def lpips_layer(f0, f1, w, out, accumulate=False):
    N, C, H, W = f0.shape
    assert f0.is_contiguous() and f1.is_contiguous() and f1.shape == f0.shape and w.numel() == C and out.numel() == N
    L.check(_lib().vd_lpips_layer(_p(f0), _p(f1), _p(w), _p(out), N, C, H * W, int(accumulate), _s()), "vd_lpips_layer")
    return out


def attn_core_eligible(heads, head_dim, N) -> bool:
    return N == 256 and heads >= 1 and (head_dim in (32, 64, 128) or (head_dim > 0 and head_dim % 256 == 0))


@functools.lru_cache(maxsize=None)
def gemm_bx3_act_eligible(M, K, NP) -> bool:
    return _gemm_tile(product_query_desc(M, K, NP, a_mode=A_COL, act=True)) == 10
# ... 266 lines not shown
    return buf.value.decode(), S


def groupnorm_fwd(x, gamma, beta, y, mean, rstd, G, eps, silu):
    Bn, Cc, H, W, xbs = _img(x)
    ybs = _img(y)[4]
    assert y.shape == x.shape and mean.numel() >= Bn * G and rstd.numel() >= Bn * G
    _timed("groupnorm_fwd (gn_fwd_reg_kernel<*> / gn_chunk_*)", 8.0 * x.numel(), "hbm", lambda: L.check(
        _lib().vd_groupnorm_fwd(_p(x), _p(gamma), _p(beta), _p(y), _p(mean), _p(rstd), Bn, Cc, H * W, G, eps,
                                int(silu), xbs, ybs, _p(_gn_ws(Bn, Cc, H * W, G, x.device)), _s()), "vd_groupnorm_fwd"))
    return y


def groupnorm_stats(x, gamma, beta, ss, mean, rstd, G, eps):
    Bn, Cc, H, W, xbs = _img(x)
    assert ss.shape == (Bn, Cc, 2) and ss.is_contiguous()
    L.check(_lib().vd_groupnorm_stats(_p(x), _p(gamma), _p(beta), _p(ss), _p(mean), _p(rstd), Bn, Cc, H * W, G, eps, xbs, _s()),
            "vd_groupnorm_stats")
    return ss


def groupnorm_stats_from_partials(part, tiles, gamma, beta, ss, mean, rstd, HW, G, eps):
    Bn, Cc = ss.shape[0], ss.shape[1]
    assert ss.is_contiguous() and part.is_contiguous() and part.numel() >= Bn * tiles * Cc * 2
    L.check(_lib().vd_groupnorm_stats_from_partials(_p(part), tiles, _p(gamma), _p(beta), _p(ss), _p(mean), _p(rstd), Bn, Cc, HW, G, eps, _s()),
            "vd_groupnorm_stats_from_partials")
    return ss


def gn_fusable(x, cout) -> bool:
    Bn, Cc, H, W = x.shape
    return W in (16, 32) and H == W and Cc % 8 == 0 and Cc <= 1024 and cout >= 64


def groupnorm_bwd(dy, x, mean, rstd, gamma, beta, dx, dgamma_ws, dbeta_ws, G, silu, extra=None, extra2=None, rowsum=None, rowsum_ld=None):
    Bn, Cc, H, W, xbs = _img(x)
    dbs, dxbs = _img(dy)[4], _img(dx)[4]
    ebs = _img(extra)[4] if extra is not None else 0
    e2bs = _img(extra2)[4] if extra2 is not None else 0
    assert dgamma_ws.numel() >= Bn * Cc and dbeta_ws.numel() >= Bn * Cc
    assert extra2 is None or extra2.shape == x.shape
    rld = 0
    if rowsum is not None:
        rld = Cc if rowsum_ld is None else rowsum_ld
        assert rld >= Cc
    nbytes = (12.0 + (4.0 if extra is not None else 0.0) + (4.0 if extra2 is not None else 0.0)) * x.numel()
    _timed("groupnorm_bwd (gn_bwd_reg_kernel<*> / gn_chunk_*)", nbytes, "hbm", lambda: L.check(
        _lib().vd_groupnorm_bwd_fused(_p(dy), _p(x), _p(mean), _p(rstd), _p(gamma), _p(beta), _p(extra), _p(extra2), _p(dx),
                                      _p(dgamma_ws), _p(dbeta_ws), _p(rowsum), Bn, Cc, H * W, G, int(silu), dbs, xbs, ebs, e2bs, dxbs, rld,
                                      _p(_gn_ws(Bn, Cc, H * W, G, x.device)), _s()), "vd_groupnorm_bwd"))
    return dx


def softmax_col_fwd(S, nb, N):
    L.check(_lib().vd_softmax_col_fwd(_p(S), nb, N, _s()), "vd_softmax_col_fwd")
    return S


def softmax_col_bwd(P, dP, nb, N, scale):
    L.check(_lib().vd_softmax_col_bwd(_p(P), _p(dP), nb, N, scale, _s()), "vd_softmax_col_bwd")
    return dP


def attn_core_fwd(qkv, out, P, heads, head_dim, N, scale):
    Bn = qkv.shape[0]
    assert qkv.is_contiguous() and out.is_contiguous() and (P is None or P.is_contiguous())
    dt = 8 if head_dim % 256 == 0 else head_dim // 32
    _timed(f"attn_core_kernel<{dt}, false>", 4.0 * Bn * heads * N * N * head_dim, "mfma", lambda: L.check(
        _lib().vd_attn_core_fwd(_p(qkv), _p(out), _p(P), Bn, heads, head_dim, N, scale, _s()), "vd_attn_core_fwd"),
        nbytes=4.0 * (qkv.numel() + out.numel() + (P.numel() if P is not None else 0)))
    return out


def attn_core_bwd(qkv, P, out, dout, dS, dqkv, heads, head_dim, N, scale):
    Bn = qkv.shape[0]
    assert qkv.is_contiguous() and P.is_contiguous() and dout.is_contiguous() and dS.is_contiguous() and dqkv.is_contiguous() and out.is_contiguous()
    dt = 8 if head_dim % 256 == 0 else head_dim // 32
    _timed(f"attn_core_kernel<{dt}, true>", 4.0 * Bn * heads * N * N * head_dim, "mfma", lambda: L.check(
        _lib().vd_attn_core_bwd(_p(qkv), _p(P), _p(out), _p(dout), _p(dS), _p(dqkv), Bn, heads, head_dim, N, scale, _s()), "vd_attn_core_bwd"),
        nbytes=4.0 * (qkv.numel() * 2 // 3 + 2 * dout.numel() + P.numel() + dS.numel() + qkv.numel() // 3))
    return dqkv


def attn_flash_eligible(heads, head_dim, N) -> bool:
    return head_dim == 32 and heads >= 1 and N >= 256 and N % 256 == 0


def attn_flash_fwd(qkv, out, lse, heads, head_dim, N, scale):
    Bn = qkv.shape[0]
    assert qkv.is_contiguous() and out.is_contiguous() and (lse is None or lse.is_contiguous())
    _timed("attn_flash_kernel<0>", 4.0 * Bn * heads * N * N * head_dim, "mfma", lambda: L.check(
        _lib().vd_attn_flash_fwd(_p(qkv), _p(out), _p(lse), Bn, heads, head_dim, N, scale, qkv.stride(0), out.stride(0), _s()), "vd_attn_flash_fwd"),
        nbytes=4.0 * (qkv.numel() + out.numel()))
    return out


def attn_flash_bwd(qkv, out, dout, lse, dqkv, heads, head_dim, N, scale):
    Bn = qkv.shape[0]
    assert qkv.is_contiguous() and out.is_contiguous() and dout.is_contiguous() and lse.is_contiguous() and dqkv.is_contiguous()
    delta = torch.empty_like(lse)
    _timed("attn_flash_kernel<1>+<2>", 10.0 * Bn * heads * N * N * head_dim, "mfma", lambda: L.check(
        _lib().vd_attn_flash_bwd(_p(qkv), _p(out), _p(dout), _p(lse), _p(delta), _p(dqkv), Bn, heads, head_dim, N, scale, qkv.stride(0),
                                 out.stride(0), dout.stride(0), dqkv.stride(0), _s()), "vd_attn_flash_bwd"),
        nbytes=4.0 * (2 * qkv.numel() + 2 * dout.numel()))
    return dqkv

# ... 408 lines not shown
```

### villandiffusion_amd/unet.py

```python
from __future__ import annotations

import math
import os
from types import SimpleNamespace
from typing import Dict, List, Optional, Tuple

import torch

from . import ops
from .flatnet import FlatParamNet
from .lib import B_CONV3, B_CONV3_DIL, B_CONV3_S2, B_CONV3_T, B_CONV3_UP, B_PLAIN, A_COL, A_ROW, B_KCONTIG


CONV_MATH_DEFAULT = os.environ.get("VILLAN_CONV_MATH", "bf16x3")
if CONV_MATH_DEFAULT not in ("bf16x3", "f32", "f16", "bf16"):
    raise ValueError(f"VILLAN_CONV_MATH must be 'bf16x3', 'f32', 'f16' or 'bf16', got {CONV_MATH_DEFAULT!r}")


class _PackedConvWeights:

    def __init__(self, net, f16: bool = False):
        self.net = net
        self.f16 = f16
        self.off = {False: {}, True: {}}
        self.jobs = {False: [], True: []}
        self.total = 0
        cands = []
        for name, shape, _ in net._layout:
            if name.endswith(".weight") and len(shape) == 4 and shape[2] == shape[3] and shape[2] in (1, 3):
                cands.append((name[:-7], (lambda n=name: net.P[n]), shape[0], shape[1], shape[2] * shape[3]))
        for prefix, ch in getattr(net, "_qkv", []):
            if prefix + "::qkv_w" in getattr(net, "Pq", {}):
                cands.append((prefix + "::qkv", (lambda k=prefix + "::qkv_w": net.Pq[k]), 3 * ch, ch, 1))
            if prefix + ".to_out.0.weight" in net.P:
                cands.append((prefix + ".to_out.0", (lambda n=prefix + ".to_out.0.weight": net.P[n]), ch, ch, 1))
        plan = []
        for key, get, cout, cin, T in cands:
            for bwd, (M, Cc, rs, cs) in ((False, (cout, cin, cin * T, T)), (True, (cin, cout, T, cin * T))):
                plan.append((key, get, bwd, M, Cc, T, rs, cs))
            if T == 9 and ".downsamplers." in key:
                plan.append((key + "::s2g", get, True, cin * 9, cout, 1, 1, cin * 9))
        for key, get, bwd, M, Cc, T, rs, cs in plan:
            if Cc % 16 == 0 and M >= 64:
                n = (M + 127) // 128 * 128 * Cc * T // (2 if f16 else 1)
                self.off[bwd][key] = (self.total, n)
                self.jobs[bwd].append((key, get, M, Cc, T, rs, cs))
                self.total += n
        self.buf: Optional[torch.Tensor] = None
        self.tables = {}
        self.key = {False: None, True: None}

    def view(self, prefix, bwd):
        ent = self.off[bwd].get(prefix)
        if ent is None:
# ... 46 lines not shown
    if not _split(net) or not ops.bx3_eligible(M, Cc, OH, OW, mode):
        return None
    pk = getattr(net, "_packed", None)
    if pk is None:
        pk = net._packed = _PackedConvWeights(net)
    return _with_mixed(net, pk.view(prefix, bwd), prefix, bwd)


def _bx3_packed_1x1(net, key, bwd, M, K, NP, nb=None):
    if not _split(net) or not ops.gemm_bx3_eligible(M, K, NP, nb):
        return None
    pk = getattr(net, "_packed", None)
    if pk is None:
        pk = net._packed = _PackedConvWeights(net)
    return _with_mixed(net, pk.view(key, bwd), key, bwd)


def _conv1x1_dgrad(net, prefix, cout, cin, dout):
    B, _, H, W = dout.shape
    HW = H * W
    dx = torch.empty((B, cin, H, W), device=dout.device, dtype=torch.float32)
    ops.gemm(net.P[prefix + ".weight"].view(cout, cin), dout, dx, M=cin, N=B * HW, K=cout, a_mode=A_COL, b_mode=B_PLAIN, NP=HW, lda=cin, ldb=HW,
             b_bstride=ops._img(dout)[4], ldd=HW, d_bstride=cin * HW, a_packed=_bx3_packed_1x1(net, prefix, True, cin, cout, HW, B))
    return dx


def _amath(net, M, K, NP) -> int:
    return int(_split(net) and ops.gemm_bx3_act_eligible(M, K, NP))


def _wgrad1x1_math(net, dy, x) -> int:
    ok = _split(net) and ops.wgrad_bx3_eligible(dy.shape[1], x.shape[1], dy.shape[2], dy.shape[3], B_PLAIN) \
        and x.stride(0) % 4 == 0 and dy.stride(0) % 4 == 0
    return int(ok)


class _Conv:

    def __init__(self, net, prefix, cin, cout, mode=B_CONV3, pad=0):
        self.net, self.prefix, self.cin, self.cout, self.mode, self.pad = net, prefix, cin, cout, mode, pad
        net._decl(prefix + ".weight", (cout, cin, 3, 3), fan_in=cin * 9)
        net._decl(prefix + ".bias", (cout,), fan_in=cin * 9, is_bias=True)

    def w2d(self):
        return self.net.P[self.prefix + ".weight"].view(self.cout, self.cin * 9)

    def fwd(self, x, out, rowadd=None, rowadd_bstride=0, residual=None, gn_ss=None, gn_part=None):
        pk = _bx3_packed(self.net, self.prefix, False, self.cout, self.cin, out.shape[2], out.shape[3], self.mode)
        if gn_ss is not None and (out.shape[3] not in (16, 32) or self.mode != B_CONV3):
            pk = None
        return ops.conv3x3(x, self.w2d(), self.net.P[self.prefix + ".bias"], out, mode=self.mode, rowadd=rowadd,
                           rowadd_bstride=rowadd_bstride, residual=residual, pad=self.pad, gn_ss=gn_ss, a_packed=pk, gn_part=gn_part)

    def us_input(self, h, save):
        net = self.net
        B, _, H, W = h.shape
        if (self.mode != B_CONV3_UP or not net.us_fwd_presplit or not getattr(net, "presplit", False) or not _pairs(net) or H != W
                or not ops.conv_presplit_ok(B, self.cin, self.cout, 2 * H, 2 * W, B_CONV3_UP)
                or (save and not (net.group_wgrad and ops.wgrad_presplit_ok(B, self.cin, self.cout, 2 * H, B_CONV3_UP)))):
            return h
        return ops.presplit_pack(h)

    def bwd(self, dout, x, dx, bias_ws=None, skip_bias=False, dout_ps=None):
        net = self.net
        dout_f32 = dout
        gw = net.G[self.prefix + ".weight"].view(self.cout, self.cin * 9)
        want = net.wants_wgrad(gw)
        if isinstance(x, ops.PreSplit):
            if want:
                dy_ps = dout_ps if dout_ps is not None else net.pack_later(dout)
                net.wgrad(dy_ps, x, gw, self.mode, pad=self.pad, math_mode=1)
            if dout_ps is not None:
                dout = dout_ps
        elif (self.mode == B_CONV3_UP and getattr(net, "presplit", False) and _pairs(net) and net.group_wgrad
              and dout.shape[2] == dout.shape[3] and ops.wgrad_presplit_ok(dout.shape[0], self.cin, self.cout, dout.shape[3], B_CONV3_UP)):
            if want:
                dy_ps = dout_ps if dout_ps is not None else net.pack_later(dout)
                net.wgrad(dy_ps, net.pack_later(x), gw, self.mode, pad=self.pad, math_mode=1)
        else:
            assert dout is not None
            bx3 = _split(net) and ops.wgrad_bx3_eligible(self.cout, self.cin, dout.shape[2], dout.shape[3],
                                                                                           self.mode) and x.stride(0) % 4 == 0
            if want:
                net.wgrad(dout, x, gw, self.mode, pad=self.pad, math_mode=int(bx3))
        if not skip_bias:
            B = dout.shape[0]
            ws = bias_ws if bias_ws is not None else net.scratch_bc(B, self.cout)
            if bias_ws is None:
                assert dout_f32 is not None
                net.rowsum(dout_f32, ws)
            net.colsum_later(ws, net.G[self.prefix + ".bias"], B, self.cout, ld=(ws.stride(0) if ws.dim() == 2 else self.cout))
        if dx is None:
            return None
        if self.mode == B_CONV3_S2:
            pk = _bx3_packed_1x1(net, self.prefix + "::s2g", True, self.cin * 9, self.cout, dout.shape[2] * dout.shape[3], dout.shape[0])
            return ops.conv3x3_s2_dgrad(dout, self.w2d(), dx, pad=self.pad, a_packed=pk)
        pk = _bx3_packed(net, self.prefix, True, self.cin, self.cout, dout.shape[2], dout.shape[3], B_CONV3_T) \
            if self.mode in (B_CONV3, B_CONV3_UP) else None
        wt = net.wt_view(self.prefix, self.cout, self.cin, 9, fresh=pk is None)
        if self.mode == B_CONV3:
            ops.conv3x3(dout, wt, None, dx, mode=B_CONV3_T, a_packed=pk)
        elif self.mode == B_CONV3_UP:
            B, _, OH, OW = dout.shape
            if pk is not None and ops.bx3_pool2_eligible(self.cin, self.cout, OH, OW, B):
                src = dout_ps if (dout_ps is not None and net.us_dgrad_presplit and ops.conv_presplit_ok(B, self.cout, self.cin, OH, OW, B_CONV3_T)) else dout
                ops.conv3x3(src, wt, None, dx, mode=B_CONV3_T, a_packed=pk, pool2=True)
            else:
                dU = torch.empty((B, self.cin, OH, OW), device=dout.device, dtype=torch.float32)
                ops.conv3x3(dout, wt, None, dU, mode=B_CONV3_T, a_packed=pk)
                ops.sumpool2x2(dU, dx)
        else:
            raise NotImplementedError(self.mode)
        return dx


class _Norm:
    def __init__(self, net, prefix, ch, silu, groups=None):
        self.net, self.prefix, self.ch, self.silu = net, prefix, ch, silu
        self.groups = net.groups if groups is None else groups
        net._decl(prefix + ".weight", (ch,), ones=True)
        net._decl(prefix + ".bias", (ch,), zeros=True)

    def fwd(self, x, y):
        net = self.net
        B = x.shape[0]
        mean = torch.empty(B * self.groups, device=x.device, dtype=torch.float32)
        rstd = torch.empty_like(mean)
        ops.groupnorm_fwd(x, net.P[self.prefix + ".weight"], net.P[self.prefix + ".bias"], y, mean, rstd, self.groups,
                          net.eps, self.silu)
        return mean, rstd

    def fwd_ps(self, x):
        net = self.net
        B = x.shape[0]
        mean = torch.empty(B * self.groups, device=x.device, dtype=torch.float32)
        rstd = torch.empty_like(mean)
        y = ops.presplit_empty(x.shape, x.device)
        ops.groupnorm_fwd_presplit(x, net.P[self.prefix + ".weight"], net.P[self.prefix + ".bias"], y, mean, rstd, self.groups, net.eps, self.silu)
        return y, mean, rstd

    def ps_ok(self, HW: int) -> bool:
        return ops.groupnorm_presplit_ok(self.ch, HW, self.groups)

    def stats(self, x):
        net = self.net
        B = x.shape[0]
        ss = torch.empty((B, self.ch, 2), device=x.device, dtype=torch.float32)
        mean = torch.empty(B * self.groups, device=x.device, dtype=torch.float32)
        rstd = torch.empty_like(mean)
        ops.groupnorm_stats(x, net.P[self.prefix + ".weight"], net.P[self.prefix + ".bias"], ss, mean, rstd, self.groups, net.eps)
        return ss

    def stats_from_partials(self, part, tiles, B, HW):
        net = self.net
        ss = torch.empty((B, self.ch, 2), device=part.device, dtype=torch.float32)
        mean = torch.empty(B * self.groups, device=part.device, dtype=torch.float32)
        rstd = torch.empty_like(mean)
        ops.groupnorm_stats_from_partials(part, tiles, net.P[self.prefix + ".weight"], net.P[self.prefix + ".bias"], ss, mean, rstd, HW,
                                          self.groups, net.eps)
        return ss

    def bwd(self, dy, x, mean, rstd, dx, extra=None, extra2=None, rowsum=None, dx_ps=None):
        net = self.net
        B = x.shape[0]
        wg, wb = net.scratch_bc(B, self.ch, 1), net.scratch_bc(B, self.ch, 2)
        if dx_ps is not None:
            ops.groupnorm_bwd_presplit(dy, x, mean, rstd, net.P[self.prefix + ".weight"], net.P[self.prefix + ".bias"], dx, dx_ps, wg, wb,
                                       self.groups, self.silu, extra=extra, extra2=extra2, rowsum=rowsum,
                                       rowsum_ld=(rowsum.stride(0) if rowsum is not None else None))
        else:
            ops.groupnorm_bwd(dy, x, mean, rstd, net.P[self.prefix + ".weight"], net.P[self.prefix + ".bias"], dx, wg, wb,
                              self.groups, self.silu, extra=extra, extra2=extra2, rowsum=rowsum,
                              rowsum_ld=(rowsum.stride(0) if rowsum is not None else None))
        net.colsum_later(wg, net.G[self.prefix + ".weight"], B, self.ch)
        net.colsum_later(wb, net.G[self.prefix + ".bias"], B, self.ch)
        return dx


class _Resnet:

    def __init__(self, net, prefix, cin, cout):
        self.net, self.prefix, self.cin, self.cout = net, prefix, cin, cout
        self.norm1 = _Norm(net, prefix + ".norm1", cin, True)
        self.conv1 = _Conv(net, prefix + ".conv1", cin, cout)
        self.temb_off = net._decl_temb(prefix + ".time_emb_proj", cout)
        self.norm2 = _Norm(net, prefix + ".norm2", cout, True)
        self.conv2 = _Conv(net, prefix + ".conv2", cout, cout)
        self.has_sc = cin != cout
        self._ps_cache = {}
        if self.has_sc:
            net._decl(prefix + ".conv_shortcut.weight", (cout, cin, 1, 1), fan_in=cin)
            net._decl(prefix + ".conv_shortcut.bias", (cout,), fan_in=cin, is_bias=True)

    def _sc_dgrad(self, dout):
        return _conv1x1_dgrad(self.net, self.prefix + ".conv_shortcut", self.cout, self.cin, dout)

    def ps_plan(self, B, H, W) -> bool:
        net = self.net
        if not getattr(net, "presplit", False) or not _pairs(net) or not net.group_wgrad or H != W:
            return False
        key = (B, H, W)
        ok = self._ps_cache.get(key)
        if ok is None:
            ci, co = self.cin, self.cout
            ok = (self.norm1.ps_ok(H * W) and self.norm2.ps_ok(H * W)
                  and ops.conv_presplit_ok(B, ci, co, H, W, B_CONV3) and ops.conv_presplit_ok(B, co, co, H, W, B_CONV3)
                  and ops.conv_presplit_ok(B, co, ci, H, W, B_CONV3_T) and ops.conv_presplit_ok(B, co, co, H, W, B_CONV3_T)
                  and ops.wgrad_presplit_ok(B, ci, co, H) and ops.wgrad_presplit_ok(B, co, co, H))
            self._ps_cache[key] = ok
        return ok

    def fwd(self, x, out, st, save):
        net = self.net
        B, _, H, W = x.shape
        dev = x.device
        fuse = net.fuse_gn_inference if net.fuse_gn_inference is not None else _split(net)
        ps_ng = not save and net.nograd_presplit and self.cout > 128 and self.ps_plan(B, H, W)
        if not save and not ps_ng and fuse and ops.gn_fusable(x, self.cout) and self.cin * H * W // net.groups <= 12288 \
                and self.cout * H * W // net.groups <= 12288:
            h1 = torch.empty((B, self.cout, H, W), device=dev, dtype=torch.float32)
            tiles = (H * W) // 256
            part = torch.empty((B, tiles, self.cout, 2), device=dev, dtype=torch.float32) if (getattr(net, "gn_stats_in_epilogue", False) and tiles > 0) else None
            self.conv1.fwd(x, h1, rowadd=st.temb_all[:, self.temb_off:], rowadd_bstride=st.temb_all.stride(0), gn_ss=self.norm1.stats(x),
                           gn_part=part)
            if part is not None and ops.GN_PART_WRITTEN:
                ss2 = self.norm2.stats_from_partials(part, tiles, B, H * W)
            else:
                ss2 = self.norm2.stats(h1)
            if self.has_sc:
                ops.conv1x1(x, net.P[self.prefix + ".conv_shortcut.weight"].view(self.cout, self.cin),
                            net.P[self.prefix + ".conv_shortcut.bias"], out,
                            a_packed=_bx3_packed_1x1(net, self.prefix + ".conv_shortcut", False, self.cout, self.cin, H * W, B))
                self.conv2.fwd(h1, out, residual=out, gn_ss=ss2)
            else:
                self.conv2.fwd(h1, out, residual=x, gn_ss=ss2)
            return None
        ps = (save and self.ps_plan(B, H, W)) or ps_ng
        sc_aux = self.has_sc and save and net.aux_fork()
        if sc_aux:
            with net.aux_scope():
                ops.conv1x1(x, net.P[self.prefix + ".conv_shortcut.weight"].view(self.cout, self.cin),
                            net.P[self.prefix + ".conv_shortcut.bias"], out,
                            a_packed=_bx3_packed_1x1(net, self.prefix + ".conv_shortcut", False, self.cout, self.cin, H * W, B))
        if ps:
            a1, m1, r1 = self.norm1.fwd_ps(x)
        else:
            a1 = torch.empty((B, self.cin, H, W), device=dev, dtype=torch.float32)
            m1, r1 = self.norm1.fwd(x, a1)
        h1 = torch.empty((B, self.cout, H, W), device=dev, dtype=torch.float32)
        self.conv1.fwd(a1, h1, rowadd=st.temb_all[:, self.temb_off:], rowadd_bstride=st.temb_all.stride(0))
        if ps:
            a2, m2, r2 = self.norm2.fwd_ps(h1)
        else:
            a2 = torch.empty_like(h1)
            m2, r2 = self.norm2.fwd(h1, a2)
        if self.has_sc:
            if sc_aux:
                net.aux_join()
            else:
                ops.conv1x1(x, net.P[self.prefix + ".conv_shortcut.weight"].view(self.cout, self.cin),
                            net.P[self.prefix + ".conv_shortcut.bias"], out,
                            a_packed=_bx3_packed_1x1(net, self.prefix + ".conv_shortcut", False, self.cout, self.cin, H * W, B))
            self.conv2.fwd(a2, out, residual=out)
        else:
            self.conv2.fwd(a2, out, residual=x)
        if save:
            return (x, a1, m1, r1, h1, a2, m2, r2)
        return None

    def bwd(self, saved, dout, dx, st, dout_rs=None, extra2=None, dx_rs=None, dout_ps=None, dx_ps=None):
        net = self.net
        x, a1, m1, r1, h1, a2, m2, r2 = saved
        B, _, H, W = x.shape
        dev = x.device
        if isinstance(a2, ops.PreSplit):
            return self._bwd_ps(saved, dout, dx, st, dout_rs, extra2, dx_rs, dout_ps, dx_ps)
        if dout_rs is None:
            bias_ws = net.scratch_bc(B, self.cout).view(B, self.cout)
            net.rowsum(dout, bias_ws)
        else:
            bias_ws = dout_rs
        dsc = None
        if self.has_sc and net.aux_fork():
            with net.aux_scope():
                dsc = self._sc_dgrad(dout)
        da2 = torch.empty((B, self.cout, H, W), device=dev, dtype=torch.float32)
        self.conv2.bwd(dout, a2, da2, bias_ws=bias_ws)
        dh1 = torch.empty_like(da2)
        dt = st.d_temb_all[:, self.temb_off:self.temb_off + self.cout]
        if getattr(net, "fuse_gn_bwd", False):
            self.norm2.bwd(da2, h1, m2, r2, dh1, rowsum=dt)
        else:
            self.norm2.bwd(da2, h1, m2, r2, dh1)
            net.rowsum(dh1, dt, ws_ld=st.d_temb_all.stride(0))
        da1 = da2 if self.cin == self.cout else torch.empty((B, self.cin, H, W), device=dev, dtype=torch.float32)
        self.conv1.bwd(dh1, a1, da1, bias_ws=dt)
        if self.has_sc:
            net.wgrad(dout, x, net.G[self.prefix + ".conv_shortcut.weight"].view(self.cout, self.cin), B_PLAIN,
                      math_mode=_wgrad1x1_math(net, dout, x))
            net.colsum_later(bias_ws, net.G[self.prefix + ".conv_shortcut.bias"], B, self.cout, ld=bias_ws.stride(0))
            if dsc is None:
                dsc = self._sc_dgrad(dout)
            else:
                net.aux_join()
            self.norm1.bwd(da1, x, m1, r1, dx, extra=dsc, extra2=extra2, rowsum=dx_rs, dx_ps=dx_ps)
        else:
            self.norm1.bwd(da1, x, m1, r1, dx, extra=dout, extra2=extra2, rowsum=dx_rs, dx_ps=dx_ps)
        return dx

    def _bwd_ps(self, saved, dout, dx, st, dout_rs, extra2, dx_rs, dout_ps, dx_ps):
        net = self.net
        x, a1, m1, r1, h1, a2, m2, r2 = saved
        B, _, H, W = x.shape
        dev = x.device
        if dout_rs is None:
            bias_ws = net.scratch_bc(B, self.cout).view(B, self.cout)
            net.rowsum(dout, bias_ws)
        else:
            bias_ws = dout_rs
        dsc = None
        if self.has_sc and net.aux_fork():
            with net.aux_scope():
                dsc = self._sc_dgrad(dout)
        da2 = torch.empty((B, self.cout, H, W), device=dev, dtype=torch.float32)
        self.conv2.bwd(dout, a2, da2, bias_ws=bias_ws, dout_ps=dout_ps)
        dh1 = ops.presplit_empty((B, self.cout, H, W), dev)
        dt = st.d_temb_all[:, self.temb_off:self.temb_off + self.cout]
        self.norm2.bwd(da2, h1, m2, r2, None, rowsum=dt, dx_ps=dh1)
        da1 = da2 if self.cin == self.cout else torch.empty((B, self.cin, H, W), device=dev, dtype=torch.float32)
        self.conv1.bwd(None, a1, da1, bias_ws=dt, dout_ps=dh1)
        if self.has_sc:
            net.wgrad(dout, x, net.G[self.prefix + ".conv_shortcut.weight"].view(self.cout, self.cin), B_PLAIN,
                      math_mode=_wgrad1x1_math(net, dout, x))
            net.colsum_later(bias_ws, net.G[self.prefix + ".conv_shortcut.bias"], B, self.cout, ld=bias_ws.stride(0))
            if dsc is None:
                dsc = self._sc_dgrad(dout)
            else:
                net.aux_join()
            self.norm1.bwd(da1, x, m1, r1, dx, extra=dsc, extra2=extra2, rowsum=dx_rs, dx_ps=dx_ps)
        else:
            self.norm1.bwd(da1, x, m1, r1, dx, extra=dout, extra2=extra2, rowsum=dx_rs, dx_ps=dx_ps)
        return dx


class _Attn:

    def __init__(self, net, prefix, ch, head_dim=None, groups=None):
        self.net, self.prefix, self.ch = net, prefix, ch
        self.heads = 1 if head_dim is None else ch // head_dim
        if ch % self.heads:
            raise ValueError(f"{prefix}: {ch} channels do not split into heads of {head_dim}")
        self.norm = _Norm(net, prefix + ".group_norm", ch, False, groups)
        self.qkv_w, self.qkv_b = net._decl_qkv(prefix, ch)
        net._decl(prefix + ".to_out.0.weight", (ch, ch), fan_in=ch)
        net._decl(prefix + ".to_out.0.bias", (ch,), fan_in=ch, is_bias=True)
        self.scale = 1.0 / math.sqrt(ch // self.heads)

    def fwd(self, x, out, st, save):
        net, Cc = self.net, self.ch
        B, _, H, W = x.shape
# ... 234 lines not shown
        super()._materialise(head, grads=True)
        layout, offs, total, dev = self._layout, self._offs, self.flat_numel, self._dev
        n_t = sum(c for _, c in self._temb)
        o0 = offs[self._temb[0][0] + ".weight"][0]
        ob = offs[self._temb[0][0] + ".bias"][0]
        self.temb_total = n_t
        self.Wt_all = self.flat_param[o0:o0 + n_t * self.temb_dim].view(n_t, self.temb_dim)
        self.bt_all = self.flat_param[ob:ob + n_t]
        self.gWt_all = self.flat_grad[o0:o0 + n_t * self.temb_dim].view(n_t, self.temb_dim)
        self.gbt_all = self.flat_grad[ob:ob + n_t]
        self._wt_offs, wt_total = {}, 0
        for name, shape, _ in layout:
            if name.endswith(".weight") and len(shape) == 4 and shape[2] == 3 and name != "conv_in.weight":
                self._wt_offs[name[:-7]] = wt_total
                wt_total += int(math.prod(shape))
        self._wt_offs["conv_in"] = wt_total
        wt_total += int(math.prod(offs["conv_in.weight"][2]))
        self._wt_total = wt_total
        self._wt_buf: Optional[torch.Tensor] = None
        self.wgrad_ws: Optional[torch.Tensor] = None
        self._cs_pool: Optional[torch.Tensor] = None
        self._cs_tables: Dict[tuple, torch.Tensor] = {}
        self._cs_cols_hint = 4 * sum(int(math.prod(sh)) for _, sh, _ in layout if len(sh) == 1) + 4096
        self._cs_off, self._cs_jobs, self._cs_B, self._cs_retired = 0, [], 0, []
        self._d_temb: Dict[int, torch.Tensor] = {}
        half = self.time_dim0 // 2
        exponent = -math.log(10000) * torch.arange(0, half, dtype=torch.float32)
        exponent = exponent / (half - self.config.freq_shift)
        self.freqs = torch.exp(exponent).to(dev)
        self._anchor = torch.zeros(1, device=dev, requires_grad=True)
        def _late(k):
            return ".time_emb_proj." in k or ".to_q." in k or ".to_k." in k or ".to_v." in k
        o_in = offs["conv_in.weight"][0]
        o_mid = min(v[0] for k, v in offs.items() if k.startswith("mid_block.") and not _late(k))
        o_up = min(v[0] for k, v in offs.items() if k.startswith("up_blocks.") and not _late(k))
        self.grad_buckets = [(o_up, total), (o_mid, o_up), (o_in, o_mid), (0, o_in)]
        self.bucket_ready_hook = None
        self.fuse_gn_inference = None
        self.fused_attention = os.environ.get("VILLAN_FUSED_ATTENTION", "1") != "0"
        self.sampler_graph = os.environ.get("VILLAN_SAMPLER_GRAPH", "1") != "0"
        self.group_wgrad = os.environ.get("VILLAN_GROUP_WGRAD", "1") != "0"
        self._wg_jobs: Dict[int, list] = {}
        self.wgrad_stream = os.environ.get("VILLAN_WGRAD_STREAM", "1") != "0"
        self.wgrad_flush_jobs = int(os.environ.get("VILLAN_WGRAD_FLUSH_JOBS", "24"))
        self._wg_side, self._wg_keep, self._rs_jobs = None, [], []
        self.fuse_gn_bwd = os.environ.get("VILLAN_FUSE_GN_BWD", "1") != "0"
        self.presplit = os.environ.get("VILLAN_PRESPLIT", "1") != "0"
        self.nograd_presplit = os.environ.get("VILLAN_NOGRAD_PRESPLIT", "1") != "0"
        self.us_dgrad_presplit = os.environ.get("VILLAN_US_DGRAD_PRESPLIT", "1") != "0"
        self.us_fwd_presplit = os.environ.get("VILLAN_US_FWD_PRESPLIT", "1") != "0"
        self.sc_stream = os.environ.get("VILLAN_SC_STREAM", "1") != "0"
        self._aux_stream = None
        self.gn_stats_in_epilogue = os.environ.get("VILLAN_GN_STATS_IN_EPILOGUE", "1") != "0"
        self._pk_jobs = []
        self.conv_math = CONV_MATH_DEFAULT
        self._packed: Optional[_PackedConvWeights] = None
        self._packed16: Optional[_PackedConvWeights] = None
        self._wt_fresh = set()

    def zero_grad(self, set_to_none: bool = False):
        ops.scale_(self.flat_grad, 0.0)

    def refresh_packed(self, bwd: bool):
        for pk in (self._packed, self._packed16):
            if pk is not None:
                pk.refresh(bwd)

    def weights_changed(self):
        for pk in (self._packed, self._packed16):
            if pk is not None:
                pk.key = {False: None, True: None}

    def _cs_begin(self, B):
        need = B * self._cs_cols_hint
        if self._cs_pool is None or self._cs_pool.numel() < need:
            self._cs_pool = torch.empty(need, device=self._dev, dtype=torch.float32)
            self._cs_tables = {}
        self._cs_off, self._cs_jobs, self._cs_B = 0, [], B
        self._cs_retired = []

    def scratch_bc(self, B, Cc, slot=0):
        n = (B * Cc + 3) // 4 * 4
        if self._cs_off + n > self._cs_pool.numel():
            self._cs_flush()
            self._cs_retired.append(self._cs_pool)
            self._cs_cols_hint *= 2
            self._cs_pool = torch.empty(B * self._cs_cols_hint, device=self._dev, dtype=torch.float32)
            self._cs_tables, self._cs_off = {}, 0
        t = self._cs_pool[self._cs_off:self._cs_off + B * Cc]
        self._cs_off += n
        return t

    def colsum_later(self, ws, out, B, Cc, ld=None):
        if self._dx_only or self.lora_route is not None:
            return
        ld = Cc if ld is None else ld
        wp, op = ws.data_ptr(), out.data_ptr()
        for c0 in range(0, Cc, 64):
            self._cs_jobs.append((wp + 4 * c0, op + 4 * c0, min(64, Cc - c0), ld))

    def wants_wgrad(self, dw2d) -> bool:
        if self._dx_only:
            return False
        return self.lora_route is None or self.lora_route.wants(self, dw2d)

    def wgrad(self, dy, x, dw2d, mode, pad=0, math_mode=0):
# ... 476 lines not shown
```

Before: 7535.

## Fuse GroupNorm forward/backward into split-K conv epilogue reduction

Adds vd_gemm_groupnorm_fwd/bwd entry points that, when a conv3x3 runs split-K, replace the split-K reduction epilogue with a kernel that also computes GroupNorm (stats and normalize, or the backward with rowsum). ResBlock forward (conv1→norm2) and backward (conv2 dgrad→norm2 bwd, conv1 dgrad→norm1 bwd) use it by default. This removes a full write and re-read of the conv output and one kernel launch per fused pair; in backward the intermediate dgrad tensor need not be materialized at all. It adds a new code path with eligibility checks and falls back to separate launches when split-K is not planned.

```diff
diff --git a/include/villan_hip.h b/include/villan_hip.h
--- a/include/villan_hip.h
+++ b/include/villan_hip.h
@@ -146,6 +146,31 @@
                            int64_t dx_bstride, int64_t rowsum_ld, float* ws, void* stream);
 int vd_groupnorm_plan(int which, int B, int C, int HW, int G, int aligned, int has_ws, void* stream, char* name, int name_len);
 
+typedef struct vd_gn_args {
+    const float* t;
+    const float* gamma;
+    const float* beta;
+    float* mean;
+    float* rstd;
+    float* y;
+    const float* x;
+    const float* extra;
+    const float* extra2;
+    float* dx;
+    float* dgamma_ws;
+    float* dbeta_ws;
+    float* rowsum;
+    float* ws;
+    void* mid_event;
+    int64_t t_bstride, y_bstride, x_bstride, extra_bstride, extra2_bstride, dx_bstride, rowsum_ld;
+    int32_t C, G, apply_silu, write_d;
+    float eps;
+    int32_t reserved_;
+} vd_gn_args;
+int vd_gemm_groupnorm_fwd(const vd_gemm_desc* desc, const vd_gn_args* gn, int* fused_splits, void* stream);
+int vd_gemm_groupnorm_bwd(const vd_gemm_desc* desc, const vd_gn_args* gn, int* fused_splits, void* stream);
+int vd_gemm_groupnorm_plan(const vd_gemm_desc* desc, const vd_gn_args* gn, int which, char* name, int name_len);
+
 int vd_softmax_col_fwd(float* S, int nb, int N, void* stream);
 int vd_softmax_col_bwd(const float* P, float* dP, int nb, int N, float scale, void* stream);
 int vd_attn_small_fwd(const float* qkv, float* out, float* P, int B, int C, int N, float scale,
diff --git a/villandiffusion_amd/csrc/vd_conv_bx3.inc b/villandiffusion_amd/csrc/vd_conv_bx3.inc
--- a/villandiffusion_amd/csrc/vd_conv_bx3.inc
+++ b/villandiffusion_amd/csrc/vd_conv_bx3.inc
@@ -830,7 +830,7 @@
     return d.OH == d.OW && (d.OW == 16 || d.OW == 32) && vd_cdiv(d.M, 128) * vd_cdiv(d.N, 128) >= 256;
 }
 
-static int launch_bx3(const vd_gemm_desc& d, int tile, hipStream_t st, char* name) {
+static int launch_bx3(const vd_gemm_desc& d, int tile, hipStream_t st, char* name, vd_splitk_gn* fuse = nullptr) {
     const int mode = d.b_mode == VD_B_CONV3 ? (d.gn_ss ? 3 : 0) : (d.b_mode == VD_B_CONV3_T ? 1 : (d.b_mode == VD_B_CONV3_S2 ? 4 : 2));
     if (tile == 18) {
         if (vd_launch_conv3_k32p(d, mode, st, name) != 0) return VD_EINVAL;
@@ -851,7 +851,7 @@
         dim3 grids(vd_cdiv(d.M, 128) * (d.N / 256), splits);
         if (mode == 0) VD_LAUNCH_OR_NAME(name, (conv3_bx3_kernel<8, 0, 2, 512, 2>), grids, dim3(512), 0, st, d, c_per);
         else VD_LAUNCH_OR_NAME(name, (conv3_bx3_kernel<8, 1, 2, 512, 2>), grids, dim3(512), 0, st, d, c_per);
-        if (!name && splits > 1) launch_splitk_epilogue(d, splits, st);
+        if (!name && splits > 1) launch_splitk_epilogue(d, splits, st, fuse);
         return 0;
     }
     if (tile == 15) {
@@ -894,6 +894,6 @@
     BX3_CASE(64, 4) BX3_CASE(128, 4)
 #undef BX3_CASE
     if (!done) return VD_EINVAL;
-    if (!name && splits > 1) launch_splitk_epilogue(d, splits, st);
+    if (!name && splits > 1) launch_splitk_epilogue(d, splits, st, fuse);
     return 0;
 }
diff --git a/villandiffusion_amd/csrc/vd_gemm.hip b/villandiffusion_amd/csrc/vd_gemm.hip
--- a/villandiffusion_amd/csrc/vd_gemm.hip
+++ b/villandiffusion_amd/csrc/vd_gemm.hip
@@ -1,4 +1,5 @@
 #include "vd_common.h"
+#include "vd_splitk_gn.h"
 #include <string.h>
 #include <stdlib.h>
 
@@ -627,45 +628,26 @@
     const int64_t total4 = ((int64_t)d.M * d.N) >> 2;
     const int64_t total = (int64_t)d.M * d.N;
     for (int64_t i4 = blockIdx.x * (int64_t)blockDim.x + threadIdx.x; i4 < total4; i4 += (int64_t)gridDim.x * blockDim.x) {
-        const int64_t i = i4 << 2;
-        const int m = (int)(i / d.N), n = (int)(i - (int64_t)m * d.N);
-        f32x4 s = *reinterpret_cast<const f32x4*>(d.ws + i);
-        for (int z = 1; z < splits; ++z) {
-            const f32x4 p = *reinterpret_cast<const f32x4*>(d.ws + (int64_t)z * total + i);
-#pragma unroll
-            for (int j = 0; j < 4; ++j) s[j] += p[j];
-        }
-        const int b = n / d.NP, p = n - b * d.NP;
-        f32x4 val;
-#pragma unroll
-        for (int j = 0; j < 4; ++j) {
-            val[j] = d.alpha * s[j];
-            if (d.bias) val[j] += d.bias[d.bias_on_n ? n + j : m];
-        }
-        if (d.rowadd) {
-            const float ra = d.rowadd[(int64_t)b * d.rowadd_bstride + m];
-#pragma unroll
-            for (int j = 0; j < 4; ++j) val[j] += ra;
-        }
-        if (d.residual) {
-            const f32x4 r = *reinterpret_cast<const f32x4*>(d.residual + (int64_t)b * d.res_bstride + (int64_t)m * d.ldd + p);
-#pragma unroll
-            for (int j = 0; j < 4; ++j) val[j] += r[j];
-        }
-        float* __restrict__ dp = d.D + (int64_t)b * d.d_bstride + (int64_t)m * d.ldd + p;
-        if (d.accumulate) {
-            const f32x4 o = *reinterpret_cast<const f32x4*>(dp);
-#pragma unroll
-            for (int j = 0; j < 4; ++j) val[j] += o[j];
-        }
+        float* dp;
+        const f32x4 val = splitk_item4(d, splits, total, i4 << 2, dp);
         *reinterpret_cast<f32x4*>(dp) = val;
     }
 }
 
-static void launch_splitk_epilogue(const vd_gemm_desc& d, int splits, hipStream_t st) {
+static bool splitk_v4(const vd_gemm_desc& d) {
+    return (d.N & 3) == 0 && (d.NP & 3) == 0 && (d.ldd & 3) == 0 && (d.d_bstride & 3) == 0 && (d.res_bstride & 3) == 0 &&
+           (((uintptr_t)d.D | (uintptr_t)d.residual | (uintptr_t)d.ws) & 15) == 0;
+}
+
+static void launch_splitk_epilogue(const vd_gemm_desc& d, int splits, hipStream_t st, vd_splitk_gn* fuse = nullptr) {
     const int64_t total = (int64_t)d.M * d.N;
-    const bool v4 = (d.N & 3) == 0 && (d.NP & 3) == 0 && (d.ldd & 3) == 0 && (d.d_bstride & 3) == 0 && (d.res_bstride & 3) == 0 &&
-                    (((uintptr_t)d.D | (uintptr_t)d.residual | (uintptr_t)d.ws) & 15) == 0;
+    const bool v4 = splitk_v4(d);
+    if (fuse && vd_splitk_gn_ok(d, *fuse->gn, fuse->which, v4)) {
+        if (fuse->gn->mid_event) (void)hipEventRecord((hipEvent_t)fuse->gn->mid_event, st);
+        vd_splitk_gn_launch(d, splits, *fuse->gn, fuse->which, st);
+        fuse->fused_splits = splits;
+        return;
+    }
     if (v4) {
         const int64_t t4 = total >> 2;
         const int g2 = (int)((t4 + 255) / 256 < 2048 ? (t4 + 255) / 256 : 2048);
@@ -713,7 +695,7 @@
     return wgs >= 512 && wgs % 512 == 0;
 }
 
-static int launch_patch(const vd_gemm_desc& d, hipStream_t st, char* name) {
+static int launch_patch(const vd_gemm_desc& d, hipStream_t st, char* name, vd_splitk_gn* fuse = nullptr) {
     int splits, ks_per;
     patch_plan(d, splits, ks_per);
     const int mode_ = d.b_mode == VD_B_CONV3 ? (d.gn_ss ? 3 : 0) : (d.b_mode == VD_B_CONV3_T ? 1 : (d.b_mode == VD_B_CONV3_S2 ? 4 : 2));
@@ -747,7 +729,7 @@
     VD_PATCH_CASE(16, 4) VD_PATCH_CASE(8, 4) VD_PATCH_CASE(4, 4)
 #undef VD_PATCH_CASE
     if (!done) return VD_EINVAL;
-    if (!name && splits > 1) launch_splitk_epilogue(d, splits, st);
+    if (!name && splits > 1) launch_splitk_epilogue(d, splits, st, fuse);
     return 0;
 }
 
@@ -2068,10 +2050,10 @@
     return tile;
 }
 
-static int gemm_run(const vd_gemm_desc* desc, hipStream_t st, char* name) {
+static int gemm_run(const vd_gemm_desc* desc, hipStream_t st, char* name, vd_splitk_gn* fuse = nullptr, bool d_optional = false) {
     VD_REQUIRE(desc != nullptr, "vd_gemm: null desc");
     vd_gemm_desc d = *desc;
-    VD_REQUIRE(d.A && d.B && d.D, "vd_gemm: null operand");
+    VD_REQUIRE(d.A && d.B && (d.D || d_optional), "vd_gemm: null operand");
     VD_REQUIRE(d.math != 3 || d.a_packed, "vd_gemm: math = 3 (one bf16 product per term) reads the hi plane of a_packed; a_packed is NULL");
 #ifndef VD_ABLATION
     VD_REQUIRE(d.debug == 0, "vd_gemm: desc.debug = %d -- timing-only ablation bits exist in `make ABLATION=1` builds only", d.debug);
@@ -2115,9 +2097,9 @@
         case 2: rc = launch_gemm_t<1, 2>(d, st, name); break;
         case 3: rc = launch_gemm_t<1, 1>(d, st, name); break;
         case 4:
-        case 6: rc = launch_patch(d, st, name); break;
+        case 6: rc = launch_patch(d, st, name, fuse); break;
         case 7: rc = launch_smallm(d, st, name); break;
-        case 8: case 12: case 15: case 16: case 18: rc = launch_bx3(d, tile, st, name); break;
+        case 8: case 12: case 15: case 16: case 18: rc = launch_bx3(d, tile, st, name, fuse); break;
         case 19: rc = vd_launch_gemm1x1_k32p(d, st, name) == 0 ? 0 : VD_EINVAL; break;
         case 20: rc = vd_launch_conv3_sm(d, st, name) == 0 ? 0 : VD_EINVAL; break;
         case 10: launch_gemm_bx3_act(d, st, name); break;
@@ -2127,7 +2109,7 @@
             gemm_bx3_plan(d, splits, st_per);
             VD_REQUIRE(name || splits == 1 || d.ws, "vd_gemm: split-K 1x1 launch needs the workspace (vd_gemm_ws_floats)");
             VD_LAUNCH_OR_NAME(name, gemm_bx3_kernel<256>, dim3(vd_cdiv(d.M, 128) * (d.N / 128), splits), dim3(NT), 0, st, d, st_per);
-            if (!name && splits > 1) launch_splitk_epilogue(d, splits, st);
+            if (!name && splits > 1) launch_splitk_epilogue(d, splits, st, fuse);
             break;
         }
         case 11: VD_LAUNCH_OR_NAME(name, gemm_bx3_persist_kernel, dim3(512), dim3(NT), 0, st, d, vd_cdiv(d.M, 128) * (d.N / 128)); break;
@@ -2155,6 +2137,70 @@
 extern "C" int vd_gemm_kernel_name(const vd_gemm_desc* desc, char* name, int name_len) {
     char buf[VD_NAME_LEN] = "";
     return name_out(gemm_run(desc, nullptr, buf), buf, name, name_len);
+}
+
+static int splitk_gn_plan(const vd_gemm_desc& d, const vd_gn_args& gn, int which) {
+    if (d.N <= 0 || d.NP <= 0 || d.M <= 0 || d.N % d.NP != 0) return 0;
+    const int tile = vd_gemm_tile(&d);
+    int splits = 1, per = 0;
+    if (tile == 4) patch_plan(d, splits, per);
+    else if (tile == 8 || tile == 16) bx3_plan(d, splits, per);
+    else if (tile == 9) gemm_bx3_plan(d, splits, per);
+    if (splits <= 1 || !d.ws) return 0;
+    return vd_splitk_gn_ok(d, gn, which, splitk_v4(d)) ? splits : 0;
+}
+
+extern "C" int vd_groupnorm_fwd(const float* x, const float* gamma, const float* beta, float* y, float* mean, float* rstd, int B, int C, int HW, int G,
+                                float eps, int apply_silu, int64_t x_bstride, int64_t y_bstride, float* ws, void* stream);
+extern "C" int vd_groupnorm_bwd_fused(const float* dy, const float* x, const float* mean, const float* rstd, const float* gamma, const float* beta,
+                                      const float* extra, const float* extra2, float* dx, float* dgamma_ws, float* dbeta_ws, float* rowsum, int B, int C,
+                                      int HW, int G, int apply_silu, int64_t dy_bstride, int64_t x_bstride, int64_t extra_bstride, int64_t extra2_bstride,
+                                      int64_t dx_bstride, int64_t rowsum_ld, float* ws, void* stream);
+
+static int gemm_groupnorm(const vd_gemm_desc* desc, const vd_gn_args* gn, int which, int* fused_splits, void* stream) {
+    VD_REQUIRE(desc && gn, "vd_gemm_groupnorm: null argument");
+    if (fused_splits) *fused_splits = 0;
+    const vd_gn_args& a = *gn;
+    const bool fwd = which == VD_SPLITK_GN_FWD;
+    VD_REQUIRE(a.gamma && a.beta && a.mean && a.rstd, "vd_gemm_groupnorm: null GroupNorm pointer");
+    if (fwd) VD_REQUIRE(a.t && a.y, "vd_gemm_groupnorm_fwd: null GroupNorm pointer");
+    else VD_REQUIRE(a.x && a.dx && a.dgamma_ws && a.dbeta_ws, "vd_gemm_groupnorm_bwd: null GroupNorm pointer");
+    VD_REQUIRE(a.C > 0 && a.G > 0 && a.C % a.G == 0 && (fwd || a.C / a.G <= 64), "vd_gemm_groupnorm: bad GroupNorm dims C=%d G=%d", a.C, a.G);
+    VD_REQUIRE(fwd || !a.rowsum || a.rowsum_ld >= a.C, "vd_gemm_groupnorm_bwd: rowsum_ld < C");
+    if (const int rc = vd_gn_sticky(fwd ? "vd_gemm_groupnorm_fwd" : "vd_gemm_groupnorm_bwd")) return rc;
+    const int plan = splitk_gn_plan(*desc, a, which);
+    VD_REQUIRE(plan > 1 || (desc->D && a.t), "vd_gemm_groupnorm_bwd: the problem does not take the fused launch (vd_gemm_groupnorm_plan): D is needed");
+    vd_splitk_gn fuse = {gn, which, 0};
+    int rc = gemm_run(desc, (hipStream_t)stream, nullptr, plan > 1 ? &fuse : nullptr, plan > 1 && !fwd);
+    if (rc) return rc;
+    if (plan > 1) VD_REQUIRE(fuse.fused_splits == plan, "vd_gemm_groupnorm: planned %d splits for the fused launch, the launch walk took %d", plan, fuse.fused_splits);
+    if (fused_splits) *fused_splits = fuse.fused_splits;
+    if (fuse.fused_splits) {
+        VD_LAUNCH_CHECK("vd_gemm_groupnorm");
+        return 0;
+    }
+    if (a.mid_event && (rc = (int)hipEventRecord((hipEvent_t)a.mid_event, (hipStream_t)stream)) != 0) return rc;
+    const int B = desc->N / desc->NP, HW = desc->NP;
+    if (fwd)
+        return vd_groupnorm_fwd(a.t, a.gamma, a.beta, a.y, a.mean, a.rstd, B, a.C, HW, a.G, a.eps, a.apply_silu, a.t_bstride, a.y_bstride, a.ws, stream);
+    return vd_groupnorm_bwd_fused(a.t, a.x, a.mean, a.rstd, a.gamma, a.beta, a.extra, a.extra2, a.dx, a.dgamma_ws, a.dbeta_ws, a.rowsum, B, a.C, HW, a.G,
+                                  a.apply_silu, a.t_bstride, a.x_bstride, a.extra_bstride, a.extra2_bstride, a.dx_bstride, a.rowsum_ld, a.ws, stream);
+}
+
+extern "C" int vd_gemm_groupnorm_fwd(const vd_gemm_desc* desc, const vd_gn_args* gn, int* fused_splits, void* stream) {
+    return gemm_groupnorm(desc, gn, VD_SPLITK_GN_FWD, fused_splits, stream);
+}
+
+extern "C" int vd_gemm_groupnorm_bwd(const vd_gemm_desc* desc, const vd_gn_args* gn, int* fused_splits, void* stream) {
+    return gemm_groupnorm(desc, gn, VD_SPLITK_GN_BWD, fused_splits, stream);
+}
+
+extern "C" int vd_gemm_groupnorm_plan(const vd_gemm_desc* desc, const vd_gn_args* gn, int which, char* name, int name_len) {
+    if (name && name_len > 0) name[0] = 0;
+    if (!desc || !gn || (which != VD_SPLITK_GN_FWD && which != VD_SPLITK_GN_BWD)) return VD_EINVAL;
+    const int plan = splitk_gn_plan(*desc, *gn, which);
+    if (plan > 1 && name && name_len > 0) vd_splitk_gn_name(*desc, *gn, which, name, name_len);
+    return plan > 1 ? plan : 0;
 }
 
 extern "C" int64_t vd_conv3_packed_bytes(int M, int C, int taps) {
diff --git a/villandiffusion_amd/csrc/vd_norm.hip b/villandiffusion_amd/csrc/vd_norm.hip
--- a/villandiffusion_amd/csrc/vd_norm.hip
+++ b/villandiffusion_amd/csrc/vd_norm.hip
@@ -1,4 +1,5 @@
 #include "vd_common.h"
+#include "vd_splitk_gn.h"
 #include <atomic>
 #include <stdlib.h>
 
@@ -94,53 +95,12 @@
     const int n4 = (cpg * HW) >> 2;
     const f32x4* __restrict__ x4 = reinterpret_cast<const f32x4*>(x + (int64_t)b * x_bs + (int64_t)g * cpg * HW);
     f32x4 v[NV];
-    float s = 0.f;
 #pragma unroll
     for (int i = 0; i < NV; ++i) {
         const int idx = lane + i * 64;
         v[i] = (idx < n4) ? x4[idx] : f32x4{0.f, 0.f, 0.f, 0.f};
-        s += (v[i][0] + v[i][1]) + (v[i][2] + v[i][3]);
-    }
-    const float inv_n = 1.f / (float)(cpg * HW);
-    const float mean = wave_sum(s) * inv_n;
-    float q = 0.f;
-#pragma unroll
-    for (int i = 0; i < NV; ++i) {
-        if (lane + i * 64 < n4) {
-            const float a0 = v[i][0] - mean, a1 = v[i][1] - mean, a2 = v[i][2] - mean, a3 = v[i][3] - mean;
-            q += (a0 * a0 + a1 * a1) + (a2 * a2 + a3 * a3);
-        }
-    }
-    const float rstd = rsqrtf(wave_sum(q) * inv_n + eps);
-    if (lane == 0) {
-        mean_out[gid] = mean;
-        rstd_out[gid] = rstd;
-    }
-    if (ss_out) {
-        for (int cl = lane; cl < cpg; cl += 64) {
-            const int c = g * cpg + cl;
-            const float ga = gamma[c] * rstd, be = beta[c] - mean * ga;
-            ss_out[((int64_t)b * C + c) * 2] = ga;
-            ss_out[((int64_t)b * C + c) * 2 + 1] = be;
-        }
-        return;
-    }
-    f32x4* __restrict__ y4 = reinterpret_cast<f32x4*>(y + (int64_t)b * y_bs + (int64_t)g * cpg * HW);
-#pragma unroll
-    for (int i = 0; i < NV; ++i) {
-        const int idx = lane + i * 64;
-        if (idx < n4) {
-            const int c = g * cpg + (idx * 4) / HW;
-            const float ga = gamma[c] * rstd, be = beta[c] - mean * ga;
-            f32x4 o;
-#pragma unroll
-            for (int j = 0; j < 4; ++j) {
-                const float z = v[i][j] * ga + be;
-                o[j] = apply_silu ? z * sigmoidf_(z) : z;
-            }
-            y4[idx] = o;
-        }
-    }
+    }
+    gn_fwd_wave_body<NV>(v, lane, gid, b, g, cpg, n4, gamma, beta, y, mean_out, rstd_out, C, HW, eps, apply_silu, y_bs, ss_out);
 }
 
 __global__ __launch_bounds__(256) void gn_fwd_kernel(const float* __restrict__ x, const float* __restrict__ gamma,
@@ -460,7 +420,6 @@
     const int b = gid / G, g = gid - b * G;
     const int cpg = C / G;
     const int n4 = (cpg * HW) >> 2;
-    const int L = HW >> 2;
     const int64_t goff = (int64_t)g * cpg * HW;
     const f32x4* __restrict__ x4 = reinterpret_cast<const f32x4*>(x + (int64_t)b * x_bs + goff);
     const f32x4* __restrict__ d4 = reinterpret_cast<const f32x4*>(dy + (int64_t)b * dy_bs + goff);
@@ -469,72 +428,15 @@
     f32x4* __restrict__ o4 = reinterpret_cast<f32x4*>(dx + (int64_t)b * dx_bs + goff);
     const float mean = mean_in[gid], rstd = rstd_in[gid];
 
-    f32x4 xh[NV], dz[NV];
-    float gav[NV];
-    float m1 = 0.f, m2 = 0.f;
+    f32x4 xv[NV], dv[NV];
 #pragma unroll
     for (int i = 0; i < NV; ++i) {
         const int idx = lane + i * 64;
         const bool in = idx < n4;
-        const f32x4 xv = in ? x4[idx] : f32x4{0.f, 0.f, 0.f, 0.f};
-        const f32x4 dv = in ? d4[idx] : f32x4{0.f, 0.f, 0.f, 0.f};
-        const int c = g * cpg + (in ? idx / L : 0);
-        const float ga = gamma[c], be = beta[c];
-        gav[i] = ga;
-        float s1 = 0.f, s2 = 0.f;
-#pragma unroll
-        for (int j = 0; j < 4; ++j) {
-            const float h_ = (xv[j] - mean) * rstd;
-            float z_ = dv[j];
-            if (apply_silu) {
-                const float z = h_ * ga + be, sg = sigmoidf_(z);
-                z_ *= sg * (1.f + z * (1.f - sg));
-            }
-            if (!in) z_ = 0.f;
-            xh[i][j] = h_;
-            dz[i][j] = z_;
-            s1 += z_;
-            s2 += z_ * h_;
-        }
-        for (int off = 1; off < L; off <<= 1) {
-            s1 += __shfl_xor(s1, off, 64);
-            s2 += __shfl_xor(s2, off, 64);
-        }
-        if (in && (lane & (L - 1)) == 0) {
-            dbeta_ws[(int64_t)b * C + c] = s1;
-            dgamma_ws[(int64_t)b * C + c] = s2;
-            m1 += ga * s1;
-            m2 += ga * s2;
-        }
-    }
-    const float inv_n = 1.f / (float)(cpg * HW);
-    m1 = wave_sum(m1) * inv_n;
-    m2 = wave_sum(m2) * inv_n;
-#pragma unroll
-    for (int i = 0; i < NV; ++i) {
-        const int idx = lane + i * 64;
-        const bool in = idx < n4;
-        float s3 = 0.f;
-        if (in) {
-            f32x4 ev = {0.f, 0.f, 0.f, 0.f}, o;
-            if (e4) ev = e4[idx];
-            if (f4) {
-                const f32x4 fv = f4[idx];
-#pragma unroll
-                for (int j = 0; j < 4; ++j) ev[j] += fv[j];
-            }
-#pragma unroll
-            for (int j = 0; j < 4; ++j) {
-                o[j] = rstd * (dz[i][j] * gav[i] - m1 - xh[i][j] * m2) + ev[j];
-                s3 += o[j];
-            }
-            o4[idx] = o;
-        }
-        if (rs_out) {
-            for (int off = 1; off < L; off <<= 1) s3 += __shfl_xor(s3, off, 64);
-            if (in && (lane & (L - 1)) == 0) rs_out[(int64_t)b * rs_ld + g * cpg + idx / L] = s3;
-        }
-    }
+        xv[i] = in ? x4[idx] : f32x4{0.f, 0.f, 0.f, 0.f};
+        dv[i] = in ? d4[idx] : f32x4{0.f, 0.f, 0.f, 0.f};
+    }
+    gn_bwd_wave_body<NV>(xv, dv, lane, b, g, cpg, n4, mean, rstd, gamma, beta, e4, f4, o4, dgamma_ws, dbeta_ws, C, HW, apply_silu, rs_out, rs_ld);
 }
 
 __device__ __forceinline__ void gn_combine(const float* __restrict__ part, int S, float n_c, float& mean, float& m2) {
@@ -1106,6 +1008,7 @@
 }
 
 int vd_gn_sticky(const char* who) { return gn_sticky_impl(who); }
+bool vd_gn_wave_ok() { return gn_wave_ok(); }
 
 extern "C" int vd_async_errors(int clear) {
     const unsigned n = gn_flag_read();
diff --git a/villandiffusion_amd/csrc/vd_splitk_gn.h b/villandiffusion_amd/csrc/vd_splitk_gn.h
--- /dev/null
+++ b/villandiffusion_amd/csrc/vd_splitk_gn.h
@@ -0,0 +1,171 @@
+#pragma once
+#include "vd_common.h"
+
+__device__ __forceinline__ f32x4 splitk_item4(const vd_gemm_desc& d, int splits, int64_t total, int64_t i, float*& dp_out) {
+    const int m = (int)(i / d.N), n = (int)(i - (int64_t)m * d.N);
+    f32x4 s = *reinterpret_cast<const f32x4*>(d.ws + i);
+    for (int z = 1; z < splits; ++z) {
+        const f32x4 p = *reinterpret_cast<const f32x4*>(d.ws + (int64_t)z * total + i);
+#pragma unroll
+        for (int j = 0; j < 4; ++j) s[j] += p[j];
+    }
+    const int b = n / d.NP, p = n - b * d.NP;
+    f32x4 val;
+#pragma unroll
+    for (int j = 0; j < 4; ++j) {
+        val[j] = d.alpha * s[j];
+        if (d.bias) val[j] += d.bias[d.bias_on_n ? n + j : m];
+    }
+    if (d.rowadd) {
+        const float ra = d.rowadd[(int64_t)b * d.rowadd_bstride + m];
+#pragma unroll
+        for (int j = 0; j < 4; ++j) val[j] += ra;
+    }
+    if (d.residual) {
+        const f32x4 r = *reinterpret_cast<const f32x4*>(d.residual + (int64_t)b * d.res_bstride + (int64_t)m * d.ldd + p);
+#pragma unroll
+        for (int j = 0; j < 4; ++j) val[j] += r[j];
+    }
+    float* dp = d.D + (int64_t)b * d.d_bstride + (int64_t)m * d.ldd + p;
+    if (d.accumulate) {
+        const f32x4 o = *reinterpret_cast<const f32x4*>(dp);
+#pragma unroll
+        for (int j = 0; j < 4; ++j) val[j] += o[j];
+    }
+    dp_out = dp;
+    return val;
+}
+
+template <int NV>
+__device__ __forceinline__ void gn_fwd_wave_body(const f32x4 (&v)[NV], int lane, int gid, int b, int g, int cpg, int n4,
+                                                 const float* __restrict__ gamma, const float* __restrict__ beta, float* __restrict__ y,
+                                                 float* __restrict__ mean_out, float* __restrict__ rstd_out, int C, int HW, float eps,
+                                                 int apply_silu, int64_t y_bs, float* __restrict__ ss_out) {
+    float s = 0.f;
+#pragma unroll
+    for (int i = 0; i < NV; ++i) s += (v[i][0] + v[i][1]) + (v[i][2] + v[i][3]);
+    const float inv_n = 1.f / (float)(cpg * HW);
+    const float mean = wave_sum(s) * inv_n;
+    float q = 0.f;
+#pragma unroll
+    for (int i = 0; i < NV; ++i) {
+        if (lane + i * 64 < n4) {
+            const float a0 = v[i][0] - mean, a1 = v[i][1] - mean, a2 = v[i][2] - mean, a3 = v[i][3] - mean;
+            q += (a0 * a0 + a1 * a1) + (a2 * a2 + a3 * a3);
+        }
+    }
+    const float rstd = rsqrtf(wave_sum(q) * inv_n + eps);
+    if (lane == 0) {
+        mean_out[gid] = mean;
+        rstd_out[gid] = rstd;
+    }
+    if (ss_out) {
+        for (int cl = lane; cl < cpg; cl += 64) {
+            const int c = g * cpg + cl;
+            const float ga = gamma[c] * rstd, be = beta[c] - mean * ga;
+            ss_out[((int64_t)b * C + c) * 2] = ga;
+            ss_out[((int64_t)b * C + c) * 2 + 1] = be;
+        }
+        return;
+    }
+    f32x4* __restrict__ y4 = reinterpret_cast<f32x4*>(y + (int64_t)b * y_bs + (int64_t)g * cpg * HW);
+#pragma unroll
+    for (int i = 0; i < NV; ++i) {
+        const int idx = lane + i * 64;
+        if (idx < n4) {
+            const int c = g * cpg + (idx * 4) / HW;
+            const float ga = gamma[c] * rstd, be = beta[c] - mean * ga;
+            f32x4 o;
+#pragma unroll
+            for (int j = 0; j < 4; ++j) {
+                const float z = v[i][j] * ga + be;
+                o[j] = apply_silu ? z * sigmoidf_(z) : z;
+            }
+            y4[idx] = o;
+        }
+    }
+}
+
+template <int NV>
+__device__ __forceinline__ void gn_bwd_wave_body(const f32x4 (&xv)[NV], const f32x4 (&dv)[NV], int lane, int b, int g, int cpg, int n4, float mean,
+                                                 float rstd, const float* __restrict__ gamma, const float* __restrict__ beta,
+                                                 const f32x4* __restrict__ e4, const f32x4* __restrict__ f4, f32x4* __restrict__ o4,
+                                                 float* __restrict__ dgamma_ws, float* __restrict__ dbeta_ws, int C, int HW, int apply_silu,
+                                                 float* __restrict__ rs_out, int64_t rs_ld) {
+    const int L = HW >> 2;
+    f32x4 xh[NV], dz[NV];
+    float gav[NV];
+    float m1 = 0.f, m2 = 0.f;
+#pragma unroll
+    for (int i = 0; i < NV; ++i) {
+        const int idx = lane + i * 64;
+        const bool in = idx < n4;
+        const int c = g * cpg + (in ? idx / L : 0);
+        const float ga = gamma[c], be = beta[c];
+        gav[i] = ga;
+        float s1 = 0.f, s2 = 0.f;
+#pragma unroll
+        for (int j = 0; j < 4; ++j) {
+            const float h_ = (xv[i][j] - mean) * rstd;
+            float z_ = dv[i][j];
+            if (apply_silu) {
+                const float z = h_ * ga + be, sg = sigmoidf_(z);
+                z_ *= sg * (1.f + z * (1.f - sg));
+            }
+            if (!in) z_ = 0.f;
+            xh[i][j] = h_;
+            dz[i][j] = z_;
+            s1 += z_;
+            s2 += z_ * h_;
+        }
+        for (int off = 1; off < L; off <<= 1) {
+            s1 += __shfl_xor(s1, off, 64);
+            s2 += __shfl_xor(s2, off, 64);
+        }
+        if (in && (lane & (L - 1)) == 0) {
+            dbeta_ws[(int64_t)b * C + c] = s1;
+            dgamma_ws[(int64_t)b * C + c] = s2;
+            m1 += ga * s1;
+            m2 += ga * s2;
+        }
+    }
+    const float inv_n = 1.f / (float)(cpg * HW);
+    m1 = wave_sum(m1) * inv_n;
+    m2 = wave_sum(m2) * inv_n;
+#pragma unroll
+    for (int i = 0; i < NV; ++i) {
+        const int idx = lane + i * 64;
+        const bool in = idx < n4;
+        float s3 = 0.f;
+        if (in) {
+            f32x4 ev = {0.f, 0.f, 0.f, 0.f}, o;
+            if (e4) ev = e4[idx];
+            if (f4) {
+                const f32x4 fv = f4[idx];
+#pragma unroll
+                for (int j = 0; j < 4; ++j) ev[j] += fv[j];
+            }
+#pragma unroll
+            for (int j = 0; j < 4; ++j) {
+                o[j] = rstd * (dz[i][j] * gav[i] - m1 - xh[i][j] * m2) + ev[j];
+                s3 += o[j];
+            }
+            o4[idx] = o;
+        }
+        if (rs_out) {
+            for (int off = 1; off < L; off <<= 1) s3 += __shfl_xor(s3, off, 64);
+            if (in && (lane & (L - 1)) == 0) rs_out[(int64_t)b * rs_ld + g * cpg + idx / L] = s3;
+        }
+    }
+}
+
+enum { VD_SPLITK_GN_FWD = 0, VD_SPLITK_GN_BWD = 1 };
+struct vd_splitk_gn {
+    const vd_gn_args* gn;
+    int which;
+    int fused_splits;
+};
+bool vd_gn_wave_ok();
+bool vd_splitk_gn_ok(const vd_gemm_desc& d, const vd_gn_args& gn, int which, bool v4);
+void vd_splitk_gn_launch(const vd_gemm_desc& d, int splits, const vd_gn_args& gn, int which, hipStream_t st);
+void vd_splitk_gn_name(const vd_gemm_desc& d, const vd_gn_args& gn, int which, char* name, int name_len);
diff --git a/villandiffusion_amd/csrc/vd_splitk_gn.hip b/villandiffusion_amd/csrc/vd_splitk_gn.hip
--- /dev/null
+++ b/villandiffusion_amd/csrc/vd_splitk_gn.hip
@@ -0,0 +1,132 @@
+#include "vd_splitk_gn.h"
+
+namespace {
+
+template <int NV>
+__device__ __forceinline__ void splitk_slab_items(const vd_gemm_desc& d, int splits, int lane, int b, int g, int cpg, int n4, bool write_d,
+                                                  f32x4 (&v)[NV]) {
+    const int64_t total = (int64_t)d.M * d.N;
+#pragma unroll
+    for (int i = 0; i < NV; ++i) {
+        const int idx = lane + i * 64;
+        v[i] = f32x4{0.f, 0.f, 0.f, 0.f};
+        if (idx < n4) {
+            const int e = idx * 4;
+            const int cl = e / d.NP, p = e - cl * d.NP;
+            const int m = g * cpg + cl;
+            float* dp;
+            f32x4 val = splitk_item4(d, splits, total, (int64_t)m * d.N + (int64_t)b * d.NP + p, dp);
+#pragma unroll
+            for (int j = 0; j < 4; ++j) {
+                float t = val[j];
+                asm volatile("" : "+v"(t));
+                val[j] = t;
+            }
+            if (write_d) *reinterpret_cast<f32x4*>(dp) = val;
+            v[i] = val;
+        }
+    }
+}
+
+template <int NV>
+__global__ __launch_bounds__(256) void splitk_gn_fwd_kernel(const vd_gemm_desc d, int splits, const float* __restrict__ gamma,
+                                                            const float* __restrict__ beta, float* __restrict__ y,
+                                                            float* __restrict__ mean_out, float* __restrict__ rstd_out, int G, float eps,
+                                                            int apply_silu, int64_t y_bs, int total) {
+    const int lane = threadIdx.x & 63;
+    const int gid = blockIdx.x * 4 + (threadIdx.x >> 6);
+    if (gid >= total) return;
+    const int b = gid / G, g = gid - b * G;
+    const int C = d.M, HW = d.NP;
+    const int cpg = C / G;
+    const int n4 = (cpg * HW) >> 2;
+    f32x4 v[NV];
+    splitk_slab_items<NV>(d, splits, lane, b, g, cpg, n4, true, v);
+    gn_fwd_wave_body<NV>(v, lane, gid, b, g, cpg, n4, gamma, beta, y, mean_out, rstd_out, C, HW, eps, apply_silu, y_bs, nullptr);
+}
+
+template <int NV>
+__global__ __launch_bounds__(256) void splitk_gn_bwd_kernel(const vd_gemm_desc d, int splits, int write_d, const float* __restrict__ x,
+                                                            const float* __restrict__ mean_in, const float* __restrict__ rstd_in,
+                                                            const float* __restrict__ gamma, const float* __restrict__ beta,
+                                                            const float* __restrict__ extra, float* __restrict__ dx,
+                                                            float* __restrict__ dgamma_ws, float* __restrict__ dbeta_ws, int G, int apply_silu,
+                                                            int64_t x_bs, int64_t ex_bs, int64_t dx_bs, const float* __restrict__ extra2,
+                                                            int64_t ex2_bs, float* __restrict__ rs_out, int64_t rs_ld, int total) {
+    const int lane = threadIdx.x & 63;
+    const int gid = blockIdx.x * 4 + (threadIdx.x >> 6);
+    if (gid >= total) return;
+    const int b = gid / G, g = gid - b * G;
+    const int C = d.M, HW = d.NP;
+    const int cpg = C / G;
+    const int n4 = (cpg * HW) >> 2;
+    const int64_t goff = (int64_t)g * cpg * HW;
+    const f32x4* __restrict__ x4 = reinterpret_cast<const f32x4*>(x + (int64_t)b * x_bs + goff);
+    const f32x4* __restrict__ e4 = extra ? reinterpret_cast<const f32x4*>(extra + (int64_t)b * ex_bs + goff) : nullptr;
+    const f32x4* __restrict__ f4 = extra2 ? reinterpret_cast<const f32x4*>(extra2 + (int64_t)b * ex2_bs + goff) : nullptr;
+    f32x4* __restrict__ o4 = reinterpret_cast<f32x4*>(dx + (int64_t)b * dx_bs + goff);
+    const float mean = mean_in[gid], rstd = rstd_in[gid];
+    f32x4 xv[NV], dv[NV];
+#pragma unroll
+    for (int i = 0; i < NV; ++i) {
+        const int idx = lane + i * 64;
+        xv[i] = idx < n4 ? x4[idx] : f32x4{0.f, 0.f, 0.f, 0.f};
+    }
+    splitk_slab_items<NV>(d, splits, lane, b, g, cpg, n4, write_d != 0, dv);
+    gn_bwd_wave_body<NV>(xv, dv, lane, b, g, cpg, n4, mean, rstd, gamma, beta, e4, f4, o4, dgamma_ws, dbeta_ws, C, HW, apply_silu, rs_out, rs_ld);
+}
+
+bool al16(const void* p) { return (((uintptr_t)p) & 15) == 0; }
+
+}
+
+bool vd_splitk_gn_ok(const vd_gemm_desc& d, const vd_gn_args& gn, int which, bool v4) {
+    if (!v4 || !vd_gn_wave_ok()) return false;
+    if (d.pool2 || d.gn_ss || d.act || d.gn_part || d.act_out || d.d_trans || d.nb2 > 1) return false;
+    if (gn.t != d.D || gn.C != d.M || gn.t_bstride != d.d_bstride || d.ldd != d.NP) return false;
+    if (gn.G <= 0 || gn.C % gn.G != 0 || d.NP % 4 != 0) return false;
+    const int HW = d.NP, L = HW / 4;
+    if ((int64_t)(gn.C / gn.G) * HW > 1024) return false;
+    if ((int64_t)gn.C * HW > d.d_bstride) return false;
+    if (which == VD_SPLITK_GN_FWD) {
+        if (gn.y == d.D || gn.y == nullptr) return false;
+        return al16(gn.y) && gn.y_bstride % 4 == 0;
+    }
+    if (!d.D && (gn.write_d || d.accumulate)) return false;
+    if (L >= 64 || (L & (L - 1)) != 0 || gn.C / gn.G > 64) return false;
+    return al16(gn.x) && al16(gn.dx) && al16(gn.extra) && al16(gn.extra2) &&
+           ((gn.x_bstride | gn.dx_bstride | gn.extra_bstride | gn.extra2_bstride) & 3) == 0;
+}
+
+static int splitk_gn_nv(const vd_gemm_desc& d, const vd_gn_args& gn) {
+    const int64_t slab = (int64_t)(gn.C / gn.G) * d.NP;
+    return slab <= 256 ? 1 : slab <= 512 ? 2 : 4;
+}
+
+void vd_splitk_gn_name(const vd_gemm_desc& d, const vd_gn_args& gn, int which, char* name, int name_len) {
+    snprintf(name, name_len, "splitk_gn_%s_kernel<%d>", which == VD_SPLITK_GN_FWD ? "fwd" : "bwd", splitk_gn_nv(d, gn));
+}
+
+void vd_splitk_gn_launch(const vd_gemm_desc& d, int splits, const vd_gn_args& gn, int which, hipStream_t st) {
+    const int total = (d.N / d.NP) * gn.G;
+    const dim3 grid(vd_cdiv(total, 4)), block(256);
+    const int nv = splitk_gn_nv(d, gn);
+#define VD_SKGN_FWD(NVV)                                                                                                                   \
+    hipLaunchKernelGGL((splitk_gn_fwd_kernel<NVV>), grid, block, 0, st, d, splits, gn.gamma, gn.beta, gn.y, gn.mean, gn.rstd, gn.G, gn.eps, \
+                       gn.apply_silu, gn.y_bstride, total)
+#define VD_SKGN_BWD(NVV)                                                                                                                       \
+    hipLaunchKernelGGL((splitk_gn_bwd_kernel<NVV>), grid, block, 0, st, d, splits, gn.write_d, gn.x, (const float*)gn.mean, (const float*)gn.rstd, \
+                       gn.gamma, gn.beta, gn.extra, gn.dx, gn.dgamma_ws, gn.dbeta_ws, gn.G, gn.apply_silu, gn.x_bstride, gn.extra_bstride,      \
+                       gn.dx_bstride, gn.extra2, gn.extra2_bstride, gn.rowsum, gn.rowsum_ld, total)
+    if (which == VD_SPLITK_GN_FWD) {
+        if (nv == 1) VD_SKGN_FWD(1);
+        else if (nv == 2) VD_SKGN_FWD(2);
+        else VD_SKGN_FWD(4);
+    } else {
+        if (nv == 1) VD_SKGN_BWD(1);
+        else if (nv == 2) VD_SKGN_BWD(2);
+        else VD_SKGN_BWD(4);
+    }
+#undef VD_SKGN_FWD
+#undef VD_SKGN_BWD
+}
diff --git a/villandiffusion_amd/lib.py b/villandiffusion_amd/lib.py
--- a/villandiffusion_amd/lib.py
+++ b/villandiffusion_amd/lib.py
@@ -33,6 +33,14 @@
                 ("H", _i32), ("W", _i32), ("OH", _i32), ("OW", _i32),
                 ("mode", _i32), ("splits", _i32), ("accumulate", _i32), ("tile", _i32),
                 ("dy_bstride", _i64), ("x_bstride", _i64), ("pad", _i32), ("math", _i32), ("presplit", _i32), ("reserved_", _i32)]
+
+
+class GnArgs(C.Structure):
+    _fields_ = [("t", _vp), ("gamma", _vp), ("beta", _vp), ("mean", _vp), ("rstd", _vp), ("y", _vp), ("x", _vp), ("extra", _vp), ("extra2", _vp),
+                ("dx", _vp), ("dgamma_ws", _vp), ("dbeta_ws", _vp), ("rowsum", _vp), ("ws", _vp), ("mid_event", _vp),
+                ("t_bstride", _i64), ("y_bstride", _i64), ("x_bstride", _i64), ("extra_bstride", _i64), ("extra2_bstride", _i64),
+                ("dx_bstride", _i64), ("rowsum_ld", _i64), ("C", _i32), ("G", _i32), ("apply_silu", _i32), ("write_d", _i32), ("eps", _f32),
+                ("reserved_", _i32)]
 
 
 PROTOTYPES = {
@@ -77,6 +85,9 @@
     "vd_groupnorm_stats_from_partials": (_i32, [_vp, _i32, _vp, _vp, _vp, _vp, _vp, _i32, _i32, _i32, _i32, _f32, _vp]),
     "vd_groupnorm_bwd_fused": (_i32, [_vp] * 12 + [_i32] * 5 + [_i64] * 6 + [_vp, _vp]),
     "vd_groupnorm_plan": (_i32, [_i32] * 7 + [_vp, C.c_char_p, _i32]),
+    "vd_gemm_groupnorm_fwd": (_i32, [C.POINTER(GemmDesc), C.POINTER(GnArgs), C.POINTER(_i32), _vp]),
+    "vd_gemm_groupnorm_bwd": (_i32, [C.POINTER(GemmDesc), C.POINTER(GnArgs), C.POINTER(_i32), _vp]),
+    "vd_gemm_groupnorm_plan": (_i32, [C.POINTER(GemmDesc), C.POINTER(GnArgs), _i32, C.c_char_p, _i32]),
     "vd_softmax_col_fwd": (_i32, [_vp, _i32, _i32, _vp]),
     "vd_softmax_col_bwd": (_i32, [_vp, _vp, _i32, _i32, _f32, _vp]),
     "vd_attn_small_fwd": (_i32, [_vp, _vp, _vp, _i32, _i32, _i32, _f32, _i64, _i64, _vp]),
diff --git a/villandiffusion_amd/ops.py b/villandiffusion_amd/ops.py
--- a/villandiffusion_amd/ops.py
+++ b/villandiffusion_amd/ops.py
@@ -259,7 +259,7 @@
 def gemm(A, B, D, *, M, N, K, a_mode=A_ROW, b_mode=B_PLAIN, NP=None, lda=0, a_bstride=0, ldb=0, b_bstride=0,
          ldd=0, d_bstride=0, bias=None, bias_on_n=False, rowadd=None, rowadd_bstride=0, residual=None,
          res_bstride=0, conv=None, alpha=1.0, d_trans=False, accumulate=False, tile=0, debug=0, pad=0, nb2=0, a_b2stride=0,
-         b_b2stride=0, d_b2stride=0, gn_ss=None, a_packed=None, math_mode=0, pool2=False, convg=None, act=0, gn_part=None, b_presplit=False):
+         b_b2stride=0, d_b2stride=0, gn_ss=None, a_packed=None, math_mode=0, pool2=False, convg=None, act=0, gn_part=None, b_presplit=False, gn=None):
     global GN_PART_WRITTEN
     d = GemmDesc()
     d.act = act
@@ -291,8 +291,12 @@
     d.ldd, d.d_bstride, d.res_bstride, d.rowadd_bstride = ldd, d_bstride, res_bstride, rowadd_bstride
     lib = _lib()
     need = lib.vd_gemm_ws_floats(C.byref(d))
-    if need > 0:
-        d.ws = _gemm_ws(need, D.device).data_ptr()
+    if need > 0 or (gn is not None and gn.ws_floats > 0):
+        ws = _gemm_ws(max(need, gn.ws_floats if gn is not None else 0), B.device)
+        if need > 0:
+            d.ws = ws.data_ptr()
+        if gn is not None and gn.ws_floats > 0:
+            gn.args.ws = ws.data_ptr()
     elif FORCE_WS is not None:
         d.ws = FORCE_WS.data_ptr()
     global LAST_GEMM_TILE, LAST_GEMM_MATH
@@ -306,13 +310,36 @@
     if GN_PART_WRITTEN:
         assert gn_part.is_contiguous() and gn_part.numel() >= (N // 256) * M * 2
         d.gn_part = gn_part.data_ptr()
+    launch, fused, gn_name = lib.vd_gemm, C.c_int32(0), None
+    if gn is not None:
+        global LAST_GN_FUSED_SPLITS, GN_FUSED_LAUNCHES
+        buf = C.create_string_buffer(64)
+        planned = lib.vd_gemm_groupnorm_plan(C.byref(d), C.byref(gn.args), gn.which, buf, len(buf))
+        if D is None and planned <= 0:
+            D = gn.alloc_d()
+            d.D = gn.args.t = D.data_ptr()
+        gn_name = buf.value.decode() if planned > 0 else gn.plain_name
+        fn = lib.vd_gemm_groupnorm_bwd if gn.which else lib.vd_gemm_groupnorm_fwd
+        launch = lambda dd, st: fn(dd, C.byref(gn.args), C.byref(fused), st)
     if _PROF is None:
-        L.check(lib.vd_gemm(C.byref(d), _s()), "vd_gemm")
+        L.check(launch(C.byref(d), _s()), "vd_gemm")
+        if gn is not None:
+            LAST_GN_FUSED_SPLITS = fused.value
+            GN_FUSED_LAUNCHES += fused.value > 0
         return D
     e0, e1 = torch.cuda.Event(enable_timing=True), torch.cuda.Event(enable_timing=True)
+    if gn is not None:
+        em = torch.cuda.Event(enable_timing=True)
+        em.record()
+        gn.args.mid_event = em.cuda_event
     e0.record()
-    L.check(lib.vd_gemm(C.byref(d), _s()), "vd_gemm")
+    L.check(launch(C.byref(d), _s()), "vd_gemm")
     e1.record()
+    if gn is not None:
+        LAST_GN_FUSED_SPLITS = fused.value
+        GN_FUSED_LAUNCHES += fused.value > 0
+        _PROF.append({"name": gn_name, "flops": 0.0, "bytes": float(gn.nbytes), "e0": em, "e1": e1, "kind": "hbm"})
+        e1 = em
     flops = 2.0 * M * N * K * (0.25 if b_mode == B_CONV3_DIL else 1.0)
     if conv is not None:
         nb_ = N // d.NP
@@ -323,6 +350,8 @@
         a_elems = M * K * (N // d.NP if a_bstride else 1)
     d_elems = M * N // (4 if pool2 else 1)
     nbytes = 4.0 * (b_elems + d_elems * (2 if residual is not None else 1) + a_elems)
+    if not d.D:
+        d.D = d.B
     name = _kernel_name(lib.vd_gemm_kernel_name, C.byref(d))
     _PROF.append({"name": name, "flops": flops, "bytes": nbytes, "e0": e0, "e1": e1, "kind": "mfma", "shape": (M, K, d.NP, N // d.NP, d.OH, d.OW)})
     return D
@@ -380,19 +409,21 @@
 
 
 GN_PART_WRITTEN = False
+LAST_GN_FUSED_SPLITS = 0
+GN_FUSED_LAUNCHES = 0
 LAST_GEMM_TILE = 0
 LAST_GEMM_MATH = 0
 FORCE_WS = None
 
 
 def conv3x3(x, w2d, bias, out, mode=B_CONV3, rowadd=None, rowadd_bstride=0, residual=None, accumulate=False, tile=0, debug=0,
-            pad=0, gn_ss=None, a_packed=None, pool2=False, gn_part=None):
+            pad=0, gn_ss=None, a_packed=None, pool2=False, gn_part=None, gn=None):
     x, ps = _unwrap(x)
     Bn, Cc, H, W, xbs = _img(x)
     M = w2d.shape[0]
     assert w2d.shape[1] == Cc * 9 and w2d.is_contiguous()
     OH, OW = _CONV_OUT[mode](H, W)
-    Bo, Mo, OHo, OWo, obs = _img(out)
+    Bo, Mo, OHo, OWo, obs = _img(out) if out is not None else (Bn, M, OH, OW, M * OH * OW)
     if pool2:
         assert (Bo, Mo, OHo, OWo) == (Bn, M, OH // 2, OW // 2) and mode == B_CONV3_T and a_packed is not None, (out.shape, (Bn, M, OH, OW))
         assert bias is None and rowadd is None and residual is None and not accumulate
@@ -405,7 +436,7 @@
     return gemm(w2d, x, out, M=M, N=Bn * OH * OW, K=Cc * 9, b_mode=mode, NP=OH * OW, lda=Cc * 9, b_bstride=xbs,
                 ldd=OHo * OWo, d_bstride=obs, bias=bias, rowadd=rowadd, rowadd_bstride=rowadd_bstride,
                 residual=residual, res_bstride=rbs, conv=(Cc, H, W, OH, OW), accumulate=accumulate, tile=tile, debug=debug,
-                pad=pad, gn_ss=gn_ss, a_packed=a_packed, pool2=pool2, gn_part=gn_part, b_presplit=ps)
+                pad=pad, gn_ss=gn_ss, a_packed=a_packed, pool2=pool2, gn_part=gn_part, b_presplit=ps, gn=gn)
 
 
 def conv2d_general(x, w2d, bias, out, kh, kw, stride=1, pad_h=0, pad_w=0, relu=False):
@@ -778,6 +809,46 @@
     return dx
 
 
+class GnCall:
+
+    def __init__(self, which, args, nbytes, plain_name, ws_floats=0, alloc_d=None):
+        self.which, self.args, self.nbytes, self.plain_name, self.ws_floats, self.alloc_d = which, args, nbytes, plain_name, ws_floats, alloc_d
+
+
+def conv3x3_groupnorm_fwd(x, w2d, bias, out, gamma, beta, y, mean, rstd, G, eps, silu, **conv):
+    Bn, Cc, H, W, obs = _img(out)
+    assert y.shape == out.shape and mean.numel() >= Bn * G and rstd.numel() >= Bn * G
+    a = L.GnArgs()
+    a.t, a.gamma, a.beta, a.mean, a.rstd, a.y = _p(out), _p(gamma), _p(beta), _p(mean), _p(rstd), _p(y)
+    a.t_bstride, a.y_bstride, a.C, a.G, a.apply_silu, a.eps = obs, _img(y)[4], Cc, G, int(silu), eps
+    conv3x3(x, w2d, bias, out, gn=GnCall(GN_FWD, a, 8.0 * out.numel(), "groupnorm_fwd (gn_fwd_reg_kernel<*> / gn_chunk_*)",
+                                         _lib().vd_groupnorm_ws_floats(Bn, Cc, H * W, G)), **conv)
+    return y
+
+
+def conv3x3_groupnorm_bwd(dout, wt, x, mean, rstd, gamma, beta, dx, dgamma_ws, dbeta_ws, G, silu, extra=None, extra2=None, rowsum=None,
+                          rowsum_ld=None, a_packed=None, dy=None, write_dy=True, mode=B_CONV3_T, **conv):
+    Bn, Cc, H, W, xbs = _img(x)
+    assert wt.shape[0] == Cc and dgamma_ws.numel() >= Bn * Cc and dbeta_ws.numel() >= Bn * Cc
+    assert extra2 is None or extra2.shape == x.shape
+    a = L.GnArgs()
+    a.t, a.gamma, a.beta, a.mean, a.rstd, a.x, a.dx = _p(dy), _p(gamma), _p(beta), _p(mean), _p(rstd), _p(x), _p(dx)
+    a.extra, a.extra2, a.dgamma_ws, a.dbeta_ws, a.rowsum = _p(extra), _p(extra2), _p(dgamma_ws), _p(dbeta_ws), _p(rowsum)
+    a.t_bstride = _img(dy)[4] if dy is not None else Cc * H * W
+    a.x_bstride, a.dx_bstride = xbs, _img(dx)[4]
+    a.extra_bstride = _img(extra)[4] if extra is not None else 0
+    a.extra2_bstride = _img(extra2)[4] if extra2 is not None else 0
+    if rowsum is not None:
+        a.rowsum_ld = Cc if rowsum_ld is None else rowsum_ld
+        assert a.rowsum_ld >= Cc
+    a.C, a.G, a.apply_silu, a.write_d = Cc, G, int(silu), int(dy is not None and write_dy)
+    nbytes = (12.0 + (4.0 if extra is not None else 0.0) + (4.0 if extra2 is not None else 0.0)) * x.numel()
+    call = GnCall(GN_BWD, a, nbytes, "groupnorm_bwd (gn_bwd_reg_kernel<*> / gn_chunk_*)", _lib().vd_groupnorm_ws_floats(Bn, Cc, H * W, G),
+                  alloc_d=lambda: torch.empty((Bn, Cc, H, W), device=x.device, dtype=torch.float32))
+    conv3x3(dout, wt, None, dy, mode=mode, a_packed=a_packed, gn=call, **conv)
+    return dx
+
+
 def softmax_col_fwd(S, nb, N):
     L.check(_lib().vd_softmax_col_fwd(_p(S), nb, N, _s()), "vd_softmax_col_fwd")
     return S
diff --git a/villandiffusion_amd/unet.py b/villandiffusion_amd/unet.py
--- a/villandiffusion_amd/unet.py
+++ b/villandiffusion_amd/unet.py
@@ -1,5 +1,6 @@
 from __future__ import annotations
 
+import functools
 import math
 import os
 from types import SimpleNamespace
@@ -152,6 +153,16 @@
         return ops.conv3x3(x, self.w2d(), self.net.P[self.prefix + ".bias"], out, mode=self.mode, rowadd=rowadd,
                            rowadd_bstride=rowadd_bstride, residual=residual, pad=self.pad, gn_ss=gn_ss, a_packed=pk, gn_part=gn_part)
 
+    def fwd_norm(self, x, out, norm, y, rowadd=None, rowadd_bstride=0):
+        net = self.net
+        pk = _bx3_packed(net, self.prefix, False, self.cout, self.cin, out.shape[2], out.shape[3], self.mode)
+        mean = torch.empty(x.shape[0] * norm.groups, device=x.device, dtype=torch.float32)
+        rstd = torch.empty_like(mean)
+        ops.conv3x3_groupnorm_fwd(x, self.w2d(), net.P[self.prefix + ".bias"], out, net.P[norm.prefix + ".weight"], net.P[norm.prefix + ".bias"], y,
+                                  mean, rstd, norm.groups, net.eps, norm.silu, mode=self.mode, rowadd=rowadd, rowadd_bstride=rowadd_bstride,
+                                  pad=self.pad, a_packed=pk)
+        return mean, rstd
+
     def us_input(self, h, save):
         net = self.net
         B, _, H, W = h.shape
@@ -161,7 +172,7 @@
             return h
         return ops.presplit_pack(h)
 
-    def bwd(self, dout, x, dx, bias_ws=None, skip_bias=False, dout_ps=None):
+    def bwd(self, dout, x, dx, bias_ws=None, skip_bias=False, dout_ps=None, then_norm=None):
         net = self.net
         dout_f32 = dout
         gw = net.G[self.prefix + ".weight"].view(self.cout, self.cin * 9)
@@ -190,6 +201,9 @@
                 assert dout_f32 is not None
                 net.rowsum(dout_f32, ws)
             net.colsum_later(ws, net.G[self.prefix + ".bias"], B, self.cout, ld=(ws.stride(0) if ws.dim() == 2 else self.cout))
+        if then_norm is not None:
+            assert dx is None
+            return self.dgrad_norm(dout, then_norm)
         if dx is None:
             return None
         if self.mode == B_CONV3_S2:
@@ -214,6 +228,13 @@
         return dx
 
 
+    def dgrad_norm(self, dout, then_norm):
+        assert self.mode == B_CONV3 and not isinstance(dout, ops.PreSplit)
+        net = self.net
+        pk = _bx3_packed(net, self.prefix, True, self.cin, self.cout, dout.shape[2], dout.shape[3], B_CONV3_T)
+        return then_norm(dout, net.wt_view(self.prefix, self.cout, self.cin, 9, fresh=pk is None), pk)
+
+
 class _Norm:
     def __init__(self, net, prefix, ch, silu, groups=None):
         self.net, self.prefix, self.ch, self.silu = net, prefix, ch, silu
@@ -272,6 +293,17 @@
             ops.groupnorm_bwd(dy, x, mean, rstd, net.P[self.prefix + ".weight"], net.P[self.prefix + ".bias"], dx, wg, wb,
                               self.groups, self.silu, extra=extra, extra2=extra2, rowsum=rowsum,
                               rowsum_ld=(rowsum.stride(0) if rowsum is not None else None))
+        net.colsum_later(wg, net.G[self.prefix + ".weight"], B, self.ch)
+        net.colsum_later(wb, net.G[self.prefix + ".bias"], B, self.ch)
+        return dx
+
+    def bwd_conv(self, dout, wt, pk, x, mean, rstd, dx, extra=None, extra2=None, rowsum=None):
+        net = self.net
+        B = x.shape[0]
+        wg, wb = net.scratch_bc(B, self.ch, 1), net.scratch_bc(B, self.ch, 2)
+        ops.conv3x3_groupnorm_bwd(dout, wt, x, mean, rstd, net.P[self.prefix + ".weight"], net.P[self.prefix + ".bias"], dx, wg, wb, self.groups,
+                                  self.silu, extra=extra, extra2=extra2, rowsum=rowsum,
+                                  rowsum_ld=(rowsum.stride(0) if rowsum is not None else None), a_packed=pk)
         net.colsum_later(wg, net.G[self.prefix + ".weight"], B, self.ch)
         net.colsum_later(wb, net.G[self.prefix + ".bias"], B, self.ch)
         return dx
@@ -348,12 +380,16 @@
             a1 = torch.empty((B, self.cin, H, W), device=dev, dtype=torch.float32)
             m1, r1 = self.norm1.fwd(x, a1)
         h1 = torch.empty((B, self.cout, H, W), device=dev, dtype=torch.float32)
-        self.conv1.fwd(a1, h1, rowadd=st.temb_all[:, self.temb_off:], rowadd_bstride=st.temb_all.stride(0))
-        if ps:
-            a2, m2, r2 = self.norm2.fwd_ps(h1)
-        else:
+        if save and not ps and net.gn_in_splitk:
             a2 = torch.empty_like(h1)
-            m2, r2 = self.norm2.fwd(h1, a2)
+            m2, r2 = self.conv1.fwd_norm(a1, h1, self.norm2, a2, rowadd=st.temb_all[:, self.temb_off:], rowadd_bstride=st.temb_all.stride(0))
+        else:
+            self.conv1.fwd(a1, h1, rowadd=st.temb_all[:, self.temb_off:], rowadd_bstride=st.temb_all.stride(0))
+            if ps:
+                a2, m2, r2 = self.norm2.fwd_ps(h1)
+            else:
+                a2 = torch.empty_like(h1)
+                m2, r2 = self.norm2.fwd(h1, a2)
         if self.has_sc:
             if sc_aux:
                 net.aux_join()
@@ -384,17 +420,27 @@
         if self.has_sc and net.aux_fork():
             with net.aux_scope():
                 dsc = self._sc_dgrad(dout)
-        da2 = torch.empty((B, self.cout, H, W), device=dev, dtype=torch.float32)
-        self.conv2.bwd(dout, a2, da2, bias_ws=bias_ws)
-        dh1 = torch.empty_like(da2)
+        pair = getattr(net, "gn_in_splitk", False) and getattr(net, "fuse_gn_bwd", False)
+        dh1 = torch.empty((B, self.cout, H, W), device=dev, dtype=torch.float32)
         dt = st.d_temb_all[:, self.temb_off:self.temb_off + self.cout]
-        if getattr(net, "fuse_gn_bwd", False):
-            self.norm2.bwd(da2, h1, m2, r2, dh1, rowsum=dt)
-        else:
-            self.norm2.bwd(da2, h1, m2, r2, dh1)
-            net.rowsum(dh1, dt, ws_ld=st.d_temb_all.stride(0))
-        da1 = da2 if self.cin == self.cout else torch.empty((B, self.cin, H, W), device=dev, dtype=torch.float32)
-        self.conv1.bwd(dh1, a1, da1, bias_ws=dt)
+        da2 = None
+        if pair:
+            self.conv2.bwd(dout, a2, None, bias_ws=bias_ws,
+                           then_norm=functools.partial(self.norm2.bwd_conv, x=h1, mean=m2, rstd=r2, dx=dh1, rowsum=dt))
+        else:
+            da2 = torch.empty_like(dh1)
+            self.conv2.bwd(dout, a2, da2, bias_ws=bias_ws)
+            if getattr(net, "fuse_gn_bwd", False):
+                self.norm2.bwd(da2, h1, m2, r2, dh1, rowsum=dt)
+            else:
+                self.norm2.bwd(da2, h1, m2, r2, dh1)
+                net.rowsum(dh1, dt, ws_ld=st.d_temb_all.stride(0))
+        if pair and dx_ps is None:
+            self.conv1.bwd(dh1, a1, None, bias_ws=dt)
+            da1 = None
+        else:
+            da1 = da2 if (self.cin == self.cout and da2 is not None) else torch.empty((B, self.cin, H, W), device=dev, dtype=torch.float32)
+            self.conv1.bwd(dh1, a1, da1, bias_ws=dt)
         if self.has_sc:
             net.wgrad(dout, x, net.G[self.prefix + ".conv_shortcut.weight"].view(self.cout, self.cin), B_PLAIN,
                       math_mode=_wgrad1x1_math(net, dout, x))
@@ -403,9 +449,11 @@
                 dsc = self._sc_dgrad(dout)
             else:
                 net.aux_join()
-            self.norm1.bwd(da1, x, m1, r1, dx, extra=dsc, extra2=extra2, rowsum=dx_rs, dx_ps=dx_ps)
-        else:
-            self.norm1.bwd(da1, x, m1, r1, dx, extra=dout, extra2=extra2, rowsum=dx_rs, dx_ps=dx_ps)
+        res = dsc if self.has_sc else dout
+        if da1 is None:
+            self.conv1.dgrad_norm(dh1, functools.partial(self.norm1.bwd_conv, x=x, mean=m1, rstd=r1, dx=dx, extra=res, extra2=extra2, rowsum=dx_rs))
+        else:
+            self.norm1.bwd(da1, x, m1, r1, dx, extra=res, extra2=extra2, rowsum=dx_rs, dx_ps=dx_ps)
         return dx
 
     def _bwd_ps(self, saved, dout, dx, st, dout_rs, extra2, dx_rs, dout_ps, dx_ps):
@@ -746,6 +794,7 @@
         self.sc_stream = os.environ.get("VILLAN_SC_STREAM", "1") != "0"
         self._aux_stream = None
         self.gn_stats_in_epilogue = os.environ.get("VILLAN_GN_STATS_IN_EPILOGUE", "1") != "0"
+        self.gn_in_splitk = os.environ.get("VILLAN_GN_IN_SPLITK", "1") != "0"
         self._pk_jobs = []
         self.conv_math = CONV_MATH_DEFAULT
         self._packed: Optional[_PackedConvWeights] = None
```

After: 7481. About the same (-0.7%).
